# OwshenNetwork/owshen

Hardware: AMD Instinct MI355X
Metric: withdraw proofs/sec (batch=1024) (higher is better)
Workload: dtype u32 (9 x 29-bit-limb Montgomery, 254-bit modular integers)

## Files before the change

include/owshen_gpu.h:

```cpp
#ifndef OWSHEN_GPU_H
#define OWSHEN_GPU_H

#include <stddef.h>
#include <stdint.h>

#ifdef __cplusplus
extern "C" {
#endif

typedef struct og_ctx og_ctx;
typedef struct og_bases og_bases;
typedef struct og_pk og_pk;

#define OG_OK 0
#define OG_ERR_INVALID (-1)
#define OG_ERR_HIP (-2)
#define OG_ERR_NO_DEVICE (-3)
#define OG_ERR_UNSATISFIED (-4)

int og_init(int device, og_ctx** out);
void og_shutdown(og_ctx* ctx);
const char* og_last_error(void);
int og_device_count(void);
int og_sync(og_ctx* ctx);
void* og_stream(og_ctx* ctx);

int og_malloc(og_ctx* ctx, size_t bytes, void** out_d);
int og_free(og_ctx* ctx, void* ptr_d);
int og_memcpy_h2d(og_ctx* ctx, void* dst_d, const void* src, size_t bytes);
int og_memcpy_d2h(og_ctx* ctx, void* dst, const void* src_d, size_t bytes);

int og_field_op_d(og_ctx* ctx, int field, int op, const uint8_t* a_d, const uint8_t* b_d,
                  uint8_t* out_d, size_t n);
int og_field_mulchain_d(og_ctx* ctx, int field, uint8_t* x_d, const uint8_t* y_d, size_t n,
                        int iters, float* ms_out);

int og_field_mulchain_lat_d(og_ctx* ctx, int field, int form, uint8_t* x_d, const uint8_t* y_d, size_t n,
                            int iters, float* ms_out, uint64_t* wave_cycles_out);

int og_ubench(og_ctx* ctx, int kind, int iters, int blocks, float* ms_out);
int og_ubench_cycles(og_ctx* ctx, int kind, int iters, int blocks, float* ms_out, uint64_t* wave_cycles_out);
int og_ubench_coresidency(og_ctx* ctx, int wgs_per_cu, int kind, int iters, int filler_blocks, int filler_threads,
                          int filler_lds, int filler_prio, int filler_work, int delay_us, float out[3]);

int og_mimc7_constants(og_ctx* ctx, uint8_t out[91 * 32]);
int og_mimc7_hash2_d(og_ctx* ctx, const uint8_t* left_d, const uint8_t* right_d, uint8_t* out_d,
                     size_t n);
int og_mimc7_merkle_paths_d(og_ctx* ctx, const uint8_t* leaves_d, const uint64_t* indices_d,
                            const uint8_t* siblings_d, int depth, uint8_t* nodes_out_d, size_t n);
int og_mimc7_tree_build_d(og_ctx* ctx, const uint8_t* leaves_d, size_t n, uint8_t* nodes_out_d);
int og_mimc7_append_d(og_ctx* ctx, int depth, const uint8_t* frontier_in_d, uint64_t next_index, const uint8_t* leaves_d,
                      size_t k, uint8_t* frontier_out_d, uint8_t* root_out_d);

int og_eddsa_verify_batch_d(og_ctx* ctx, const uint8_t* records_d, size_t n, uint32_t* ok_out);

int og_eddsa_pubkey_batch_d(og_ctx* ctx, const uint8_t* sk_d, size_t n, uint8_t* pk_out_d, uint8_t* pkc_out_d, uint32_t* ok_out);
int og_eddsa_decompress_batch_d(og_ctx* ctx, const uint8_t* pkc_d, size_t n, uint8_t* pk_out_d, uint32_t* ok_out);
int og_eddsa_sign_batch_d(og_ctx* ctx, const uint8_t* requests_d, size_t n, uint8_t* records_out_d, uint32_t* ok_out);
int og_eddsa_verify_compressed_batch_d(og_ctx* ctx, const uint8_t* records_d, size_t n, uint32_t* ok_out);

int og_note_seal_batch_d(og_ctx* ctx, const uint8_t* requests_d, size_t n, uint8_t* memos_out_d, uint8_t* notes_out_d, uint32_t* ok_out);
int og_note_scan_batch_d(og_ctx* ctx, const uint8_t sk[32], const uint8_t* memos_d, const uint8_t* leaves_d, size_t n, uint8_t* opened_out_d, uint32_t* hit_out);

int og_ntt_fr_d(og_ctx* ctx, const uint8_t* in_d, uint8_t* out_d, int log_n, int batch, int inverse,
                int coset);
int og_h_poly_d(og_ctx* ctx, const uint8_t* a_d, const uint8_t* b_d, const uint8_t* c_d, int log_d,
                int batch, uint8_t* h_out_d);

int og_bases_create_d(og_ctx* ctx, int group, const uint8_t* points_d, size_t n, int window_bits,
                      int precompute, og_bases** out);
void og_bases_free(og_bases* bases);
int og_msm_d(og_ctx* ctx, const og_bases* bases, const uint8_t* scalars_d, size_t n, int batch,
             size_t stride_bytes, uint8_t* out);

int og_msm_partial_slots(const og_bases* bases);
int og_msm_windows_d(og_ctx* ctx, const og_bases* bases, const uint8_t* scalars_d, size_t n, int win_rank, int win_world,
                     uint8_t* partial_out_d);
int og_msm_combine_d(og_ctx* ctx, const og_bases* bases, const uint8_t* gathered_d, int world, uint8_t* out);

int og_pk_load(og_ctx* ctx, const uint8_t* blob, size_t len, og_pk** out);
void og_pk_free(og_pk* pk);
int og_pk_info(const og_pk* pk, uint64_t info[4]);
int og_pk_density(const og_pk* pk, uint64_t out[4]);
int og_pk_windows(const og_pk* pk, uint64_t out[4]);
int og_pk_load_rows(og_ctx* ctx, const uint8_t* blob, size_t len, const uint8_t* rows, size_t rows_len, og_pk** out);
int og_pk_query_form(const og_pk* pk, uint64_t out[20]);
int og_prove(og_ctx* ctx, const og_pk* pk, const uint8_t* witness, const uint8_t rs[64], uint8_t proof_out[256]);
int og_prove_batch(og_ctx* ctx, const og_pk* pk, const uint8_t* witnesses, size_t n, const uint8_t* rs,
                   uint8_t* proofs_out);
int og_prove_batch_d(og_ctx* ctx, const og_pk* pk, const uint8_t* witnesses_d, size_t n, const uint8_t* rs,
                     uint8_t* proofs_out);

typedef struct og_multi og_multi;
int og_multi_init(int n_devices, og_multi** out);
void og_multi_shutdown(og_multi* m);
int og_multi_size(const og_multi* m);
int og_multi_slice(const og_multi* m, size_t n, int rank, size_t out[2]);
og_ctx* og_multi_ctx(og_multi* m, int rank);
int og_multi_device_info(const og_multi* m, int rank, uint64_t out[4], char pci_out[32]);
int og_multi_pk_load(og_multi* m, const uint8_t* blob, size_t len, og_pk** pks_out);
void og_multi_pk_free(og_multi* m, og_pk** pks);
int og_multi_prove_batch(og_multi* m, og_pk* const* pks, const uint8_t* witnesses, size_t n, const uint8_t* rs,
                         uint8_t* proofs_out);
int og_multi_withdraw_prove_batch(og_multi* m, og_pk* const* pks, int depth, uint64_t n_pad3, uint64_t n_pad2,
                                  const uint8_t* inputs, size_t n, const uint8_t* rs, uint8_t* proofs_out,
                                  uint8_t* public_out);
int og_multi_withdraw_prove_sharded(og_multi* m, og_pk* const* pks, int depth, uint64_t n_pad3, uint64_t n_pad2,
                                    const uint8_t* inputs, size_t n, const uint8_t* rs, uint8_t* proofs_out,
                                    uint8_t* public_out);
int og_multi_prove_sharded(og_multi* m, og_pk* const* pks, const uint8_t* witnesses, size_t n, const uint8_t* rs,
                           uint8_t* proofs_out);
int og_multi_bases_create(og_multi* m, int group, const uint8_t* points, size_t n, int window_bits, int precompute,
                          og_bases** bases_out);
void og_multi_bases_free(og_multi* m, og_bases** bases);
int og_multi_msm(og_multi* m, og_bases* const* bases, const uint8_t* scalars, size_t n, uint8_t* out);

int og_verify(const uint8_t* vk, size_t vk_len, const uint8_t* public_inputs, size_t n_pub,
              const uint8_t proof[256], int* ok_out);

typedef struct og_vk og_vk;
int og_vk_load(og_ctx* ctx, const uint8_t* vk, size_t vk_len, og_vk** out);
void og_vk_free(og_vk* vk);
int og_vk_info(const og_vk* vk, uint64_t info[4]);
int og_verify_batch_d(og_ctx* ctx, const og_vk* vk, const uint8_t* public_inputs_d, const uint8_t* proofs_d, size_t n,
                      uint32_t* ok_out);

int og_withdraw_shape(int depth, uint64_t n_pad3, uint64_t n_pad2, uint64_t shape[3]);
int og_withdraw_witness_d(og_ctx* ctx, int depth, uint64_t n_pad3, uint64_t n_pad2, const uint8_t* inputs_d,
                          size_t n, uint8_t* witness_out_d);
int og_withdraw_prove_batch_d(og_ctx* ctx, const og_pk* pk, int depth, uint64_t n_pad3, uint64_t n_pad2,
                              const uint8_t* inputs_d, size_t n, const uint8_t* rs, uint8_t* proofs_out,
                              uint8_t* public_out);

int og_deposit_shape(uint64_t shape[3]);
int og_deposit_witness_d(og_ctx* ctx, const uint8_t* inputs_d, size_t n, uint8_t* witness_out_d);
int og_deposit_prove_batch_d(og_ctx* ctx, const og_pk* pk, const uint8_t* inputs_d, size_t n, const uint8_t* rs,
                             uint8_t* proofs_out, uint8_t* public_out);

int og_split_shape(int depth, uint64_t shape[3]);
int og_split_witness_d(og_ctx* ctx, int depth, const uint8_t* inputs_d, size_t n, uint8_t* witness_out_d);
int og_split_prove_batch_d(og_ctx* ctx, const og_pk* pk, int depth, const uint8_t* inputs_d, size_t n, const uint8_t* rs,
                           uint8_t* proofs_out, uint8_t* public_out);

int og_join_shape(int depth, uint64_t shape[3]);
int og_join_witness_d(og_ctx* ctx, int depth, const uint8_t* inputs_d, size_t n, uint8_t* witness_out_d);
int og_join_prove_batch_d(og_ctx* ctx, const og_pk* pk, int depth, const uint8_t* inputs_d, size_t n, const uint8_t* rs,
                          uint8_t* proofs_out, uint8_t* public_out);

int og_transfer_shape(int depth, uint64_t shape[3]);
int og_transfer_witness_d(og_ctx* ctx, int depth, const uint8_t* inputs_d, size_t n, uint8_t* witness_out_d);
int og_transfer_prove_batch_d(og_ctx* ctx, const og_pk* pk, int depth, const uint8_t* inputs_d, size_t n, const uint8_t* rs,
                              uint8_t* proofs_out, uint8_t* public_out);

typedef struct og_job og_job;
int og_withdraw_prove_batch_submit_d(og_ctx* ctx, const og_pk* pk, int depth, uint64_t n_pad3, uint64_t n_pad2,
                                     const uint8_t* inputs_d, size_t n, const uint8_t* rs, uint8_t* proofs_out,
                                     uint8_t* public_out, og_job** job_out);
int og_job_wait(og_ctx* ctx, og_job* job);
int og_job_poll(og_ctx* ctx, og_job* job, int* done_out);
int og_job_abandon(og_ctx* ctx, og_job* job);

#define OG_PARTIAL_BYTES 768
int og_withdraw_prove_partials_d(og_ctx* ctx, const og_pk* pk, int depth, uint64_t n_pad3, uint64_t n_pad2,
                                 const uint8_t* inputs_d, size_t n, int win_rank, int win_world, uint8_t* partials_d,
                                 uint8_t* public_out);
int og_prove_partials_d(og_ctx* ctx, const og_pk* pk, const uint8_t* witnesses_d, size_t n, int win_rank, int win_world,
                        uint8_t* partials_d);
int og_prove_from_partials_d(og_ctx* ctx, const og_pk* pk, const uint8_t* gathered_d, int win_world, size_t n,
                             const uint8_t* rs, uint8_t* proofs_out);

typedef struct og_r1cs og_r1cs;
int og_withdraw_r1cs(og_ctx* ctx, int depth, uint64_t n_pad3, uint64_t n_pad2, int dense, og_r1cs** out);
int og_deposit_r1cs(og_ctx* ctx, og_r1cs** out);
int og_split_r1cs(og_ctx* ctx, int depth, og_r1cs** out);
int og_join_r1cs(og_ctx* ctx, int depth, og_r1cs** out);
int og_transfer_r1cs(og_ctx* ctx, int depth, og_r1cs** out);
int og_r1cs_from_csr(uint64_t n_wires, uint64_t n_pub, uint64_t n_constraints, const uint32_t* const ptr[3],
                     const uint32_t* const col[3], const uint8_t* const val[3], og_r1cs** out);
void og_r1cs_free(og_r1cs* r1cs);
int og_r1cs_info(const og_r1cs* r1cs, uint64_t info[6]);
int og_r1cs_export(const og_r1cs* r1cs, int matrix, uint32_t* ptr_out, uint32_t* col_out, uint8_t* val_out);
int og_setup(og_ctx* ctx, const og_r1cs* r1cs, const uint8_t toxic[160], uint8_t** pk_out, size_t* pk_len, uint8_t** vk_out,
             size_t* vk_len);
int og_setup_rows(og_ctx* ctx, const og_r1cs* r1cs, const uint8_t toxic[160], uint8_t** pk_out, size_t* pk_len, uint8_t** vk_out,
                  size_t* vk_len, uint8_t** rows_out, size_t* rows_len);
void og_blob_free(uint8_t* blob);

int og_zkey_import(og_ctx* ctx, const uint8_t* zkey, size_t zkey_len, const og_r1cs* r1cs, uint8_t** pk_out, size_t* pk_len,
                   uint8_t** vk_out, size_t* vk_len);
int og_zkey_export(og_ctx* ctx, const uint8_t* pk, size_t pk_len, const uint8_t* vk, size_t vk_len, uint8_t** zkey_out,
                   size_t* zkey_len);
int og_r1cs_read(const uint8_t* r1cs_file, size_t len, og_r1cs** out);
int og_r1cs_write(const og_r1cs* r1cs, uint8_t** file_out, size_t* file_len);
int og_wtns_read(const uint8_t* wtns, size_t len, uint8_t* values_out, size_t capacity, uint64_t* n_out);
int og_wtns_write(const uint8_t* values, uint64_t n, uint8_t** wtns_out, size_t* wtns_len);

int og_ptau_info(const uint8_t* ptau, size_t len, uint64_t info[4]);
int og_setup_ptau(og_ctx* ctx, const og_r1cs* r1cs, const uint8_t* ptau, size_t len, uint8_t** pk_out, size_t* pk_len,
                  uint8_t** vk_out, size_t* vk_len);
int og_pk_contribute(og_ctx* ctx, const uint8_t* pk, size_t pk_len, const uint8_t* vk, size_t vk_len, const uint8_t d[32],
                     uint8_t** pk_out, size_t* pk_out_len, uint8_t** vk_out, size_t* vk_out_len);
int og_ptau_verify(og_ctx* ctx, const uint8_t* ptau, size_t len, uint32_t* failed_out);
int og_pk_verify(og_ctx* ctx, const og_r1cs* r1cs, const uint8_t* ptau, size_t len, const uint8_t* pk, size_t pk_len,
                 const uint8_t* vk, size_t vk_len, uint32_t* failed_out);

int og_scalar_mul_d(og_ctx* ctx, int group, const uint8_t* base, const uint8_t* scalars_d, size_t n,
                    uint8_t* out_d);
int og_lagrange_evals_d(og_ctx* ctx, int log_d, const uint8_t tau[32], uint8_t* out_d);
int og_spmv_fr_d(og_ctx* ctx, const uint32_t* row_ptr_d, const uint32_t* col_d, const uint8_t* val_d,
                 size_t n_rows, const uint8_t* x_d, uint8_t* out_d);

int og_profile(og_ctx* ctx, int enable);
int og_set_lanes(og_ctx* ctx, int n_lanes);
int og_profile_read(og_ctx* ctx, int kind, double out[3]);
int og_release_scratch(og_ctx* ctx);
int og_set_scratch_budget(og_ctx* ctx, uint64_t bytes);
int og_set_host_chains(og_ctx* ctx, int max_requests);
int og_mem_info(og_ctx* ctx, uint64_t out[4]);
int og_prove_plan(og_ctx* ctx, const og_pk* pk, size_t n, uint32_t* sizes_out, size_t cap, size_t* count_out, int* mode_out);
int og_glv_decompose(const uint8_t k[32], uint8_t out[32]);
int og_pk_bytes(const og_pk* pk, uint64_t* out);

#ifdef __cplusplus
}
#endif
#endif
```

owshen_amd/_abi.py:

```python
import ctypes as C

_vp, _sz, _i, _u8p = C.c_void_p, C.c_size_t, C.c_int, C.c_void_p
_fp = C.POINTER(C.c_float)

SIGNATURES = {
    "og_init": (_i, [_i, C.POINTER(_vp)]),
    "og_shutdown": (None, [_vp]),
    "og_last_error": (C.c_char_p, []),
    "og_device_count": (_i, []),
    "og_sync": (_i, [_vp]),
    "og_stream": (_vp, [_vp]),
    "og_malloc": (_i, [_vp, _sz, C.POINTER(_vp)]),
    "og_free": (_i, [_vp, _vp]),
    "og_memcpy_h2d": (_i, [_vp, _vp, _vp, _sz]),
    "og_memcpy_d2h": (_i, [_vp, _vp, _vp, _sz]),
    "og_field_op_d": (_i, [_vp, _i, _i, _u8p, _u8p, _u8p, _sz]),
    "og_field_mulchain_d": (_i, [_vp, _i, _u8p, _u8p, _sz, _i, _fp]),
    "og_field_mulchain_lat_d": (_i, [_vp, _i, _i, _u8p, _u8p, _sz, _i, _fp, C.POINTER(C.c_uint64)]),
    "og_ubench": (_i, [_vp, _i, _i, _i, _fp]),
    "og_ubench_cycles": (_i, [_vp, _i, _i, _i, _fp, C.POINTER(C.c_uint64)]),
    "og_ubench_coresidency": (_i, [_vp, _i, _i, _i, _i, _i, _i, _i, _i, _i, _fp]),
    "og_mimc7_constants": (_i, [_vp, _vp]),
    "og_mimc7_hash2_d": (_i, [_vp, _u8p, _u8p, _u8p, _sz]),
    "og_mimc7_merkle_paths_d": (_i, [_vp, _u8p, _vp, _u8p, _i, _u8p, _sz]),
    "og_mimc7_tree_build_d": (_i, [_vp, _u8p, _sz, _u8p]),
    "og_mimc7_append_d": (_i, [_vp, _i, _u8p, C.c_uint64, _u8p, _sz, _u8p, _u8p]),
    "og_eddsa_verify_batch_d": (_i, [_vp, _u8p, _sz, _vp]),
    "og_eddsa_pubkey_batch_d": (_i, [_vp, _u8p, _sz, _u8p, _u8p, _vp]),
    "og_eddsa_decompress_batch_d": (_i, [_vp, _u8p, _sz, _u8p, _vp]),
    "og_eddsa_sign_batch_d": (_i, [_vp, _u8p, _sz, _u8p, _vp]),
    "og_eddsa_verify_compressed_batch_d": (_i, [_vp, _u8p, _sz, _vp]),
    "og_note_seal_batch_d": (_i, [_vp, _u8p, _sz, _u8p, _u8p, _vp]),
    "og_note_scan_batch_d": (_i, [_vp, _u8p, _u8p, _u8p, _sz, _u8p, _vp]),
    "og_ntt_fr_d": (_i, [_vp, _u8p, _u8p, _i, _i, _i, _i]),
    "og_h_poly_d": (_i, [_vp, _u8p, _u8p, _u8p, _i, _i, _u8p]),
    "og_bases_create_d": (_i, [_vp, _i, _u8p, _sz, _i, _i, C.POINTER(_vp)]),
    "og_bases_free": (None, [_vp]),
    "og_msm_d": (_i, [_vp, _vp, _u8p, _sz, _i, _sz, _vp]),
    "og_msm_partial_slots": (_i, [_vp]),
    "og_msm_windows_d": (_i, [_vp, _vp, _u8p, _sz, _i, _i, _u8p]),
    "og_msm_combine_d": (_i, [_vp, _vp, _u8p, _i, _vp]),
    "og_multi_init": (_i, [_i, C.POINTER(_vp)]),
    "og_multi_shutdown": (None, [_vp]),
    "og_multi_size": (_i, [_vp]),
    "og_multi_slice": (_i, [_vp, _sz, _i, C.POINTER(_sz)]),
    "og_multi_ctx": (_vp, [_vp, _i]),
    "og_multi_pk_load": (_i, [_vp, _vp, _sz, C.POINTER(_vp)]),
    "og_multi_pk_free": (None, [_vp, C.POINTER(_vp)]),
    "og_multi_prove_batch": (_i, [_vp, C.POINTER(_vp), _vp, _sz, _vp, _vp]),
    "og_multi_withdraw_prove_batch": (_i, [_vp, C.POINTER(_vp), _i, C.c_uint64, C.c_uint64, _vp, _sz, _vp, _vp, _vp]),
    "og_multi_withdraw_prove_sharded": (_i, [_vp, C.POINTER(_vp), _i, C.c_uint64, C.c_uint64, _vp, _sz, _vp, _vp, _vp]),
    "og_multi_prove_sharded": (_i, [_vp, C.POINTER(_vp), _vp, _sz, _vp, _vp]),
    "og_withdraw_prove_partials_d": (_i, [_vp, _vp, _i, C.c_uint64, C.c_uint64, _u8p, _sz, _i, _i, _u8p, _vp]),
    "og_prove_partials_d": (_i, [_vp, _vp, _u8p, _sz, _i, _i, _u8p]),
    "og_prove_from_partials_d": (_i, [_vp, _vp, _u8p, _i, _sz, _vp, _vp]),
    "og_multi_bases_create": (_i, [_vp, _i, _vp, _sz, _i, _i, C.POINTER(_vp)]),
    "og_multi_bases_free": (None, [_vp, C.POINTER(_vp)]),
    "og_multi_msm": (_i, [_vp, C.POINTER(_vp), _vp, _sz, _vp]),
    "og_deposit_shape": (_i, [C.POINTER(C.c_uint64)]),
    "og_deposit_witness_d": (_i, [_vp, _u8p, _sz, _u8p]),
    "og_deposit_prove_batch_d": (_i, [_vp, _vp, _u8p, _sz, _vp, _vp, _vp]),
    "og_deposit_r1cs": (_i, [_vp, C.POINTER(_vp)]),
    "og_split_shape": (_i, [_i, C.POINTER(C.c_uint64)]),
    "og_split_witness_d": (_i, [_vp, _i, _u8p, _sz, _u8p]),
    "og_split_prove_batch_d": (_i, [_vp, _vp, _i, _u8p, _sz, _vp, _vp, _vp]),
    "og_split_r1cs": (_i, [_vp, _i, C.POINTER(_vp)]),
    "og_join_shape": (_i, [_i, C.POINTER(C.c_uint64)]),
    "og_join_witness_d": (_i, [_vp, _i, _u8p, _sz, _u8p]),
    "og_join_prove_batch_d": (_i, [_vp, _vp, _i, _u8p, _sz, _vp, _vp, _vp]),
    "og_join_r1cs": (_i, [_vp, _i, C.POINTER(_vp)]),
    "og_transfer_shape": (_i, [_i, C.POINTER(C.c_uint64)]),
    "og_transfer_witness_d": (_i, [_vp, _i, _u8p, _sz, _u8p]),
    "og_transfer_prove_batch_d": (_i, [_vp, _vp, _i, _u8p, _sz, _vp, _vp, _vp]),
    "og_transfer_r1cs": (_i, [_vp, _i, C.POINTER(_vp)]),
    "og_withdraw_r1cs": (_i, [_vp, _i, C.c_uint64, C.c_uint64, _i, C.POINTER(_vp)]),
    "og_r1cs_from_csr": (_i, [C.c_uint64, C.c_uint64, C.c_uint64, C.POINTER(_vp), C.POINTER(_vp), C.POINTER(_vp), C.POINTER(_vp)]),
    "og_r1cs_free": (None, [_vp]),
    "og_r1cs_info": (_i, [_vp, C.POINTER(C.c_uint64)]),
    "og_r1cs_export": (_i, [_vp, _i, _vp, _vp, _vp]),
    "og_setup": (_i, [_vp, _vp, _vp, C.POINTER(_vp), C.POINTER(_sz), C.POINTER(_vp), C.POINTER(_sz)]),
    "og_setup_rows": (_i, [_vp, _vp, _vp, C.POINTER(_vp), C.POINTER(_sz), C.POINTER(_vp), C.POINTER(_sz), C.POINTER(_vp), C.POINTER(_sz)]),
    "og_blob_free": (None, [_vp]),
    "og_zkey_import": (_i, [_vp, _vp, _sz, _vp, C.POINTER(_vp), C.POINTER(_sz), C.POINTER(_vp), C.POINTER(_sz)]),
    "og_r1cs_read": (_i, [_vp, _sz, C.POINTER(_vp)]),
    "og_r1cs_write": (_i, [_vp, C.POINTER(_vp), C.POINTER(_sz)]),
    "og_zkey_export": (_i, [_vp, _vp, _sz, _vp, _sz, C.POINTER(_vp), C.POINTER(_sz)]),
    "og_wtns_read": (_i, [_vp, _sz, _vp, _sz, C.POINTER(C.c_uint64)]),
    "og_wtns_write": (_i, [_vp, C.c_uint64, C.POINTER(_vp), C.POINTER(_sz)]),
    "og_ptau_info": (_i, [_vp, _sz, C.POINTER(C.c_uint64)]),
    "og_setup_ptau": (_i, [_vp, _vp, _vp, _sz, C.POINTER(_vp), C.POINTER(_sz), C.POINTER(_vp), C.POINTER(_sz)]),
    "og_pk_contribute": (_i, [_vp, _vp, _sz, _vp, _sz, _vp, C.POINTER(_vp), C.POINTER(_sz), C.POINTER(_vp), C.POINTER(_sz)]),
    "og_ptau_verify": (_i, [_vp, _vp, _sz, C.POINTER(C.c_uint32)]),
    "og_pk_verify": (_i, [_vp, _vp, _vp, _sz, _vp, _sz, _vp, _sz, C.POINTER(C.c_uint32)]),
    "og_pk_load": (_i, [_vp, _vp, _sz, C.POINTER(_vp)]),
    "og_pk_load_rows": (_i, [_vp, _vp, _sz, _vp, _sz, C.POINTER(_vp)]),
    "og_pk_query_form": (_i, [_vp, C.POINTER(C.c_uint64)]),
    "og_pk_free": (None, [_vp]),
    "og_pk_info": (_i, [_vp, C.POINTER(C.c_uint64)]),
    "og_pk_density": (_i, [_vp, C.POINTER(C.c_uint64)]),
    "og_pk_windows": (_i, [_vp, C.POINTER(C.c_uint64)]),
    "og_prove": (_i, [_vp, _vp, _vp, _vp, _vp]),
    "og_prove_batch": (_i, [_vp, _vp, _vp, _sz, _vp, _vp]),
    "og_prove_batch_d": (_i, [_vp, _vp, _u8p, _sz, _vp, _vp]),
    "og_verify": (_i, [_vp, _sz, _vp, _sz, _vp, C.POINTER(_i)]),
    "og_vk_load": (_i, [_vp, _vp, _sz, C.POINTER(_vp)]),
    "og_vk_free": (None, [_vp]),
    "og_vk_info": (_i, [_vp, C.POINTER(C.c_uint64)]),
    "og_verify_batch_d": (_i, [_vp, _vp, _u8p, _u8p, _sz, _vp]),
    "og_withdraw_shape": (_i, [_i, C.c_uint64, C.c_uint64, C.POINTER(C.c_uint64)]),
    "og_withdraw_witness_d": (_i, [_vp, _i, C.c_uint64, C.c_uint64, _u8p, _sz, _u8p]),
    "og_profile": (_i, [_vp, _i]),
    "og_set_lanes": (_i, [_vp, _i]),
    "og_profile_read": (_i, [_vp, _i, C.POINTER(C.c_double)]),
    "og_release_scratch": (_i, [_vp]),
    "og_set_scratch_budget": (_i, [_vp, C.c_uint64]),
    "og_set_host_chains": (_i, [_vp, _i]),
    "og_withdraw_prove_batch_d": (_i, [_vp, _vp, _i, C.c_uint64, C.c_uint64, _u8p, _sz, _vp, _vp, _vp]),
    "og_withdraw_prove_batch_submit_d": (_i, [_vp, _vp, _i, C.c_uint64, C.c_uint64, _u8p, _sz, _vp, _vp, _vp, C.POINTER(_vp)]),
    "og_job_wait": (_i, [_vp, _vp]),
    "og_job_abandon": (_i, [_vp, _vp]),
    "og_job_poll": (_i, [_vp, _vp, _vp]),
    "og_multi_device_info": (_i, [_vp, _i, _vp, _vp]),
    "og_mem_info": (_i, [_vp, C.POINTER(C.c_uint64)]),
    "og_pk_bytes": (_i, [_vp, C.POINTER(C.c_uint64)]),
    "og_glv_decompose": (_i, [_vp, _vp]),
    "og_prove_plan": (_i, [_vp, _vp, _sz, C.POINTER(C.c_uint32), _sz, C.POINTER(_sz), C.POINTER(_i)]),
    "og_scalar_mul_d": (_i, [_vp, _i, _vp, _u8p, _sz, _u8p]),
    "og_lagrange_evals_d": (_i, [_vp, _i, _vp, _u8p]),
    "og_spmv_fr_d": (_i, [_vp, _vp, _vp, _u8p, _sz, _u8p, _u8p]),
}


def bind(lib):
    for name, (res, args) in SIGNATURES.items():
        f = getattr(lib, name)
        f.restype = res
        f.argtypes = args
    return lib
```

owshen_amd/csrc/groth16.hip:

```cpp
#include "ctx.h"
#include "statements.h"
#include "msm.hip.h"
#include "prover.h"
#include "field.hip.h"
#include "glv.h"
#include "ec.hip.h"
#include "key_blob.h"
#include <string.h>
#include <algorithm>
#include <iterator>
#include <atomic>
#include <mutex>
#include <thread>

struct og_pk {
  uint64_t m = 0, n_pub = 0, log_d = 0, n_rows = 0;
  size_t d = 0;
  uint64_t nnz[3] = {0, 0, 0};
  uint32_t* ptr[3] = {nullptr, nullptr, nullptr};
  uint32_t* col[3] = {nullptr, nullptr, nullptr};
  uint8_t* val[3] = {nullptr, nullptr, nullptr};
  uint32_t* long_rows[3] = {nullptr, nullptr, nullptr};
  uint32_t n_long[3] = {0, 0, 0};
  og_bases *a = nullptr, *b1 = nullptr, *b2 = nullptr, *l = nullptr, *h = nullptr;
  uint32_t* map[3] = {nullptr, nullptr, nullptr};
  size_t n_dense[3] = {0, 0, 0};
  size_t n_real[3] = {0, 0, 0};
  int sort_src[3] = {0, 1, 2};
  bool row[3] = {false, false, false};
  og_bases *lag1 = nullptr, *lag2 = nullptr;
  uint32_t* rmap = nullptr;
  size_t n_rowpts = 0;
  size_t rows_q[2] = {0, 0};
  int c_wire[3] = {0, 0, 0};
  bool merge_lh = false;
  bool c_is_ab = false;
  uint8_t* consts1 = nullptr;
  uint8_t* consts2 = nullptr;
  uint8_t* fb_delta2 = nullptr;
  int device = 0;
  uint8_t consts1_h[192] = {}, consts2_h[256] = {};
  std::vector<uint8_t> fb_delta2_h;
  mutable std::vector<uint8_t> fb_delta1_h;
  mutable std::once_flag fb_delta1_once;
};

namespace og {

__global__ void __launch_bounds__(256) k_spmv(const uint32_t* __restrict__ ptr, const uint32_t* __restrict__ col,
                                             const uint8_t* __restrict__ val, size_t n_rows, size_t n_out,
                                             const uint8_t* __restrict__ x, size_t x_stride, uint8_t* __restrict__ out,
                                             size_t out_stride, int val_mont, int out_mont, uint32_t long_row,
                                             uint8_t* __restrict__ canon, size_t canon_stride) {
  OG_FILLER_PRIO();
  size_t row = (size_t)blockIdx.x * blockDim.x + threadIdx.x;
  if (row >= n_out) return;
  const int g = blockIdx.y;
  const uint8_t* xg = x + (size_t)g * x_stride;
  Fr acc = Fr::zero();
  if (row < n_rows) {
    if (ptr[row + 1] - ptr[row] > long_row) return;
    for (uint32_t k = ptr[row]; k < ptr[row + 1]; k++) {
      Fr v = fe_load<FrParams>(val + (size_t)k * 32);
      if (!val_mont) v = fe_to_mont(v);
      acc = fe_add(acc, fe_mul(v, fe_load<FrParams>(xg + (size_t)col[k] * 32)));
    }
    if (canon) fe_store(canon + (size_t)g * canon_stride + row * 32, fe_canon(acc));
    acc = out_mont ? fe_to_mont(acc) : fe_canon(acc);
  }
  fe_store(out + (size_t)g * out_stride + row * 32, acc);
}

constexpr uint32_t SPMV_LONG = 2048;
__global__ void __launch_bounds__(256) k_spmv_long(const uint32_t* __restrict__ rows, const uint32_t* __restrict__ ptr,
                                                  const uint32_t* __restrict__ col, const uint8_t* __restrict__ val,
                                                  const uint8_t* __restrict__ x, size_t x_stride, uint8_t* __restrict__ out,
                                                  size_t out_stride, int val_mont, int out_mont, uint8_t* __restrict__ canon,
                                                  size_t canon_stride) {
  OG_FILLER_PRIO();
  __shared__ __align__(16) uint32_t part[256 * 8];
  const uint32_t row = rows[blockIdx.x];
  const int g = blockIdx.y;
  const uint8_t* xg = x + (size_t)g * x_stride;
  Fr acc = Fr::zero();
  for (uint32_t k = ptr[row] + threadIdx.x; k < ptr[row + 1]; k += 256) {
    Fr v = fe_load<FrParams>(val + (size_t)k * 32);
    if (!val_mont) v = fe_to_mont(v);
    acc = fe_add(acc, fe_mul(v, fe_load<FrParams>(xg + (size_t)col[k] * 32)));
  }
  fe_store(&part[threadIdx.x * 8], acc);
  __syncthreads();
  for (int d = 128; d >= 1; d >>= 1) {
    if ((int)threadIdx.x < d)
      fe_store(&part[threadIdx.x * 8], fe_add(fe_load<FrParams>(&part[threadIdx.x * 8]), fe_load<FrParams>(&part[(threadIdx.x + d) * 8])));
    __syncthreads();
  }
  if (threadIdx.x == 0) {
    acc = fe_load<FrParams>(&part[0]);
    if (canon) fe_store(canon + (size_t)g * canon_stride + (size_t)row * 32, fe_canon(acc));
    fe_store(out + (size_t)g * out_stride + (size_t)row * 32, out_mont ? fe_to_mont(acc) : fe_canon(acc));
  }
}

__global__ void __launch_bounds__(256) k_fr_to_mont(const uint8_t* __restrict__ in, uint8_t* __restrict__ out, size_t n) {
  size_t i = (size_t)blockIdx.x * blockDim.x + threadIdx.x;
  if (i >= n) return;
  fe_store(out + i * 32, fe_to_mont(fe_load<FrParams>(in + i * 32)));
}

__global__ void __launch_bounds__(256) k_mul_rows(const uint8_t* __restrict__ a, const uint8_t* __restrict__ b, uint8_t* __restrict__ c, size_t d) {
  OG_FILLER_PRIO();
  const size_t row = (size_t)blockIdx.x * blockDim.x + threadIdx.x;
  if (row >= d) return;
  const size_t o = ((size_t)blockIdx.y * d + row) * 32;
  fe_store(c + o, fe_mul(fe_load<FrParams>(a + o), fe_load<FrParams>(b + o)));
}

__global__ void __launch_bounds__(256) k_check_rows(const uint8_t* __restrict__ a, const uint8_t* __restrict__ b, const uint8_t* __restrict__ c,
                                                   size_t n_rows, size_t d, const uint8_t* __restrict__ z, size_t z_stride,
                                                   uint32_t* __restrict__ flags) {
  OG_FILLER_PRIO();
  size_t row = (size_t)blockIdx.x * blockDim.x + threadIdx.x;
  const int g = blockIdx.y;
  if (row >= n_rows) return;
  const size_t o = ((size_t)g * d + row) * 32;
  bool bad = !fe_sub(fe_mul(fe_load<FrParams>(a + o), fe_load<FrParams>(b + o)), fe_load<FrParams>(c + o)).is_zero();
  if (row == 0) {
    Fr z0 = fe_load<FrParams>(z + (size_t)g * z_stride);
    z0.l[0] ^= 1u;
    uint32_t nz = 0;
#pragma unroll
    for (int i = 0; i < 9; i++) nz |= z0.l[i];
    bad = bad || nz != 0;
  }
  if (bad) atomicOr(&flags[g], 1u);
}

__global__ void __launch_bounds__(256) k_check_canonical(const uint8_t* __restrict__ x, size_t stride, size_t count, uint32_t* __restrict__ bad) {
  OG_FILLER_PRIO();
  const size_t i = (size_t)blockIdx.x * blockDim.x + threadIdx.x;
  if (i >= count) return;
  const int g = blockIdx.y;
  if (!fe_lt_modulus(fe_load<FrParams>(x + (size_t)g * stride + i * 32))) atomicMin(&bad[g], (uint32_t)i);
}

__global__ void __launch_bounds__(256) k_lagrange(const uint8_t* __restrict__ consts, const uint8_t* __restrict__ tau_c, int log_d,
                                                 uint8_t* __restrict__ out) {
  size_t k = (size_t)blockIdx.x * blockDim.x + threadIdx.x;
  const size_t d = (size_t)1 << log_d;
  if (k >= d) return;
  Fr tau = fe_to_mont(fe_load<FrParams>(tau_c));
  Fr zt = tau;
  for (int i = 0; i < log_d; i++) zt = fe_sqr(zt);
  zt = fe_sub(zt, Fr::one());
  Fr b = fe_load<FrParams>(consts + 0 * 32), wk = Fr::one();
  for (size_t e = k; e; e >>= 1) {
    if (e & 1) wk = fe_mul(wk, b);
    b = fe_sqr(b);
  }
  Fr num = fe_mul(fe_mul(zt, fe_load<FrParams>(consts + 4 * 32)), wk);
  Fr den = fe_sub(tau, wk);
  fe_store(out + k * 32, fe_from_mont(fe_mul(num, fe_inv(den))));
}

int spmv_canonical(og_ctx* ctx, const uint32_t* ptr_d, const uint32_t* col_d, const uint8_t* val_d, size_t n_rows,
                   const uint8_t* x_d, uint8_t* out_d) {
  if (n_rows == 0) return OG_OK;
  hipLaunchKernelGGL(k_spmv, dim3(grid_for(n_rows, 256), 1), dim3(256), 0, ctx->stream, ptr_d, col_d, val_d, n_rows, n_rows, x_d,
                     (size_t)0, out_d, (size_t)0, 0, 0, 0xffffffffu, (uint8_t*)nullptr, (size_t)0);
  OG_HIP(hipGetLastError());
  return OG_OK;
}

int lagrange_evals(og_ctx* ctx, int log_d, const uint8_t tau[32], uint8_t* out_d) {
  uint8_t* consts = nullptr;
  OG_TRY(ntt_domain_consts(ctx, log_d, &consts));
  uint8_t* tau_d = nullptr;
  OG_TRY(arena_get(ctx, "g16.tau", 32, (void**)&tau_d));
  OG_HIP(hipMemcpyAsync(tau_d, tau, 32, hipMemcpyHostToDevice, ctx->stream));
  const size_t d = (size_t)1 << log_d;
  hipLaunchKernelGGL(k_lagrange, dim3(grid_for(d, 256)), dim3(256), 0, ctx->stream, consts, tau_d, log_d, out_d);
  OG_HIP(hipGetLastError());
  OG_HIP(hipStreamSynchronize(ctx->stream));
  return OG_OK;
}

int scalar_mul_fixed(og_ctx* ctx, int is_g2, const uint8_t* base_host, const uint8_t* scalars_d, size_t n, uint8_t* out_d) {
  const size_t pb = is_g2 ? 128 : 64;
  const int g = is_g2 ? 1 : 0;
  uint8_t *raw = nullptr, *mont = nullptr;
  OG_TRY(arena_get(ctx, "g16.base.raw", 128, (void**)&raw));
  OG_TRY(arena_get(ctx, "g16.base.mont", 128, (void**)&mont));
  if (!ctx->fb_tab[g]) {
    OG_HIP(hipMalloc((void**)&ctx->fb_tab[g], 64 * 16 * pb));
    ctx->owned.push_back(ctx->fb_tab[g]);
  }
  uint8_t* tab = ctx->fb_tab[g];
  if (!ctx->fb_valid[g] || memcmp(ctx->fb_base[g], base_host, pb) != 0) {
    ctx->fb_valid[g] = false;
    OG_HIP(hipMemcpyAsync(raw, base_host, pb, hipMemcpyHostToDevice, ctx->stream));
    OG_TRY(is_g2 ? import_points_g2(ctx, raw, mont, 1) : import_points_g1(ctx, raw, mont, 1));
    OG_TRY(is_g2 ? fixed_table_g2(ctx, mont, tab) : fixed_table_g1(ctx, mont, tab));
    OG_HIP(hipStreamSynchronize(ctx->stream));
    memcpy(ctx->fb_base[g], base_host, pb);
    ctx->fb_valid[g] = true;
  }
  OG_TRY(is_g2 ? scalar_mul_fixed_g2(ctx, tab, scalars_d, n, out_d) : scalar_mul_fixed_g1(ctx, tab, scalars_d, n, out_d));
  OG_HIP(hipStreamSynchronize(ctx->stream));
  return OG_OK;
}

void pk_destroy(og_pk* pk) {
  if (!pk) return;
  (void)hipSetDevice(pk->device);
  (void)hipDeviceSynchronize();
  for (int k = 0; k < 3; k++) {
    if (pk->ptr[k]) (void)hipFree(pk->ptr[k]);
    if (pk->col[k]) (void)hipFree(pk->col[k]);
    if (pk->val[k]) (void)hipFree(pk->val[k]);
    if (pk->long_rows[k]) (void)hipFree(pk->long_rows[k]);
  }
  for (og_bases* q : {pk->a, pk->b1, pk->b2})
    if (q != pk->lag1 && q != pk->lag2) bases_destroy(q);
  bases_destroy(pk->lag1); bases_destroy(pk->lag2); bases_destroy(pk->l); bases_destroy(pk->h);
  for (int k = 0; k < 3; k++)
    if (pk->map[k] && pk->map[k] != pk->rmap) (void)hipFree(pk->map[k]);
  if (pk->rmap) (void)hipFree(pk->rmap);
  if (pk->consts1) (void)hipFree(pk->consts1);
  if (pk->consts2) (void)hipFree(pk->consts2);
  if (pk->fb_delta2) (void)hipFree(pk->fb_delta2);
  delete pk;
}

bool row_form_pays(size_t rows_q, size_t wires_q) {
  if (rows_q == 0 || wires_q == 0) return false;
  const double row_adds = (double)rows_q * msm_nwin((int)msm_pick_query_c(rows_q));
  const double wire_adds = (double)wires_q * msm_nwin((int)msm_pick_query_c(wires_q));
  return row_adds <= 0.8 * wire_adds;
}

static int rows_check(og_ctx* ctx, const og_pk* pk, const PkView& v, const RowsView& rv, uint8_t* stage, const std::string& who) {
  const size_t m = pk->m, nr = pk->n_rows;
  std::vector<uint8_t> rho(m * 32);
  uint64_t x = rd64(rv.digest) ^ rd64(rv.digest + 8) ^ rd64(rv.digest + 16) ^ rd64(rv.digest + 24);
  for (size_t i = 0; i < m * 4; i++) {
    x += 0x9e3779b97f4a7c15ull;
    uint64_t z = x;
    z = (z ^ (z >> 30)) * 0xbf58476d1ce4e5b9ull;
    z = (z ^ (z >> 27)) * 0x94d049bb133111ebull;
    z ^= z >> 31;
    if ((i & 3) == 3) z &= (1ull << 60) - 1;
    memcpy(&rho[i * 8], &z, 8);
  }
  uint8_t *rho_d, *ev_d, *res_d, *aff_d;
  OG_TRY(arena_get(ctx, "g16.chk.rho", m * 32, (void**)&rho_d));
  OG_TRY(arena_get(ctx, "g16.chk.ev", nr * 32, (void**)&ev_d));
  OG_TRY(arena_get(ctx, "g16.chk.res", 512, (void**)&res_d));
  OG_TRY(arena_get(ctx, "g16.chk.aff", 256, (void**)&aff_d));
  OG_HIP(hipMemcpyAsync(rho_d, rho.data(), m * 32, hipMemcpyHostToDevice, ctx->stream));
  const int cw = (int)msm_pick_c(m);
  struct Pair { int q, src, is_g2; const char* name; };
  const Pair pairs[3] = {{0, 0, 0, "A"}, {1, 1, 0, "B (G1)"}, {1, 2, 1, "B (G2)"}};
  for (const Pair& p : pairs) {
    if (!pk->row[p.q]) continue;
    const size_t pb = p.is_g2 ? 128 : 64;
    hipLaunchKernelGGL(k_spmv, dim3(grid_for(nr, 256), 1), dim3(256), 0, ctx->stream, pk->ptr[p.q], pk->col[p.q], pk->val[p.q], nr, nr, rho_d,
                       (size_t)0, ev_d, (size_t)0, 1, 0, SPMV_LONG, (uint8_t*)nullptr, (size_t)0);
    OG_HIP(hipGetLastError());
    if (pk->n_long[p.q]) {
      hipLaunchKernelGGL(k_spmv_long, dim3(pk->n_long[p.q], 1), dim3(256), 0, ctx->stream, pk->long_rows[p.q], pk->ptr[p.q], pk->col[p.q],
                         pk->val[p.q], rho_d, (size_t)0, ev_d, (size_t)0, 1, 0, (uint8_t*)nullptr, (size_t)0);
      OG_HIP(hipGetLastError());
    }
    OG_HIP(hipMemcpyAsync(stage, v.query[p.src], m * pb, hipMemcpyHostToDevice, ctx->stream));
    og_bases* wb = nullptr;
    OG_TRY(bases_create(ctx, p.is_g2, stage, m, cw, 0, &wb));
    struct Drop { og_bases* b; ~Drop() { bases_destroy(b); } } drop{wb};
    DigitSort dw, dr;
    OG_TRY(msm_digit_sort(ctx, 0, rho_d, m * 32, m, nullptr, 1, cw, 0, &dw));
    OG_TRY(msm_run(ctx, wb, dw, res_d));
    const og_bases* lag = p.is_g2 ? pk->lag2 : pk->lag1;
    OG_TRY(msm_digit_sort(ctx, 1, ev_d, nr * 32, pk->n_rowpts, pk->rmap, 1, lag->c, 1, &dr));
    OG_TRY(msm_run(ctx, lag, dr, res_d + 256));
    OG_TRY(xyzz_to_affine_bytes(ctx, p.is_g2, res_d, aff_d, 1));
    OG_TRY(xyzz_to_affine_bytes(ctx, p.is_g2, res_d + 256, aff_d + 128, 1));
    uint8_t got[256];
    OG_HIP(hipMemcpyAsync(got, aff_d, 256, hipMemcpyDeviceToHost, ctx->stream));
    OG_HIP(hipStreamSynchronize(ctx->stream));
    OG_REQUIRE(memcmp(got, got + 128, pb) == 0,
               who + ": row-basis extension: its points do not reproduce the key's " + p.name + " query (not the Lagrange basis of this key's tau)");
  }
  return OG_OK;
}

static int pk_load_impl(og_ctx* ctx, const uint8_t* blob, size_t len, const uint8_t* rows, size_t rows_len, og_pk* pk) {
  const std::string who = rows ? "og_pk_load_rows" : "og_pk_load";
  PkView v;
  OG_TRY(pk_view(blob, len, who, &v));
  RowsView rv{};
  if (rows) OG_TRY(rows_view(rows, rows_len, v, who, &rv));
  OG_REQUIRE(v.flags <= 1 && v.word9 == 0, who + ": unknown header flags");
  OG_REQUIRE(!(v.flags & 1) || v.nnz[2] == 0, who + ": a key with the C = A o B flag carries no C matrix");
  OG_TRY(pk_csr_check(v, 3, who));
  pk->m = v.m; pk->n_pub = v.l; pk->log_d = v.log_d; pk->n_rows = v.n_rows; pk->d = v.d;
  for (int k = 0; k < 3; k++) pk->nnz[k] = v.nnz[k];
  pk->c_is_ab = (v.flags & 1) != 0;
  const size_t m = pk->m, nl = v.nl, nh = v.nh;
  const uint8_t *c1 = blob + PK_CONSTS1, *c2 = blob + PK_CONSTS2;
  for (int k = 0; k < 3; k++) {
    OG_HIP(hipMalloc((void**)&pk->ptr[k], (pk->n_rows + 1) * 4));
    OG_HIP(hipMalloc((void**)&pk->col[k], pk->nnz[k] * 4 + 4));
    OG_HIP(hipMalloc((void**)&pk->val[k], pk->nnz[k] * 32 + 32));
    OG_HIP(hipMemcpyAsync(pk->ptr[k], v.ptr[k], (pk->n_rows + 1) * 4, hipMemcpyHostToDevice, ctx->stream));
    OG_HIP(hipMemcpyAsync(pk->col[k], v.col[k], pk->nnz[k] * 4, hipMemcpyHostToDevice, ctx->stream));
    OG_HIP(hipMemcpyAsync(pk->val[k], v.val[k], pk->nnz[k] * 32, hipMemcpyHostToDevice, ctx->stream));
    {
      std::vector<uint32_t> lr;
      for (size_t r = 0; r < pk->n_rows; r++)
        if (rd32(v.ptr[k] + (r + 1) * 4) - rd32(v.ptr[k] + r * 4) > SPMV_LONG) lr.push_back((uint32_t)r);
      pk->n_long[k] = (uint32_t)lr.size();
      if (!lr.empty()) {
        OG_HIP(hipMalloc((void**)&pk->long_rows[k], lr.size() * 4));
        OG_HIP(hipMemcpy(pk->long_rows[k], lr.data(), lr.size() * 4, hipMemcpyHostToDevice));
      }
    }
    if (pk->nnz[k]) {
      hipLaunchKernelGGL(k_fr_to_mont, dim3(grid_for(pk->nnz[k], 256)), dim3(256), 0, ctx->stream, pk->val[k], pk->val[k],
                         (size_t)pk->nnz[k]);
      OG_HIP(hipGetLastError());
    }
  }
  uint8_t* stage = nullptr;
  const size_t stage_bytes = std::max<size_t>(std::max<size_t>(std::max<size_t>(512, m * 128), nh * 64), rows ? pk->n_rows * 128 : 0);
  OG_HIP(hipMalloc((void**)&stage, stage_bytes));
  struct Guard { uint8_t* p; ~Guard() { if (p) (void)hipFree(p); } } guard{stage};
  OG_HIP(hipMalloc((void**)&pk->consts1, 256));
  OG_HIP(hipMalloc((void**)&pk->consts2, 256));
  OG_HIP(hipMemcpyAsync(stage, c1, 256, hipMemcpyHostToDevice, ctx->stream));
  OG_TRY(import_points_g1(ctx, stage, pk->consts1, 3));
  OG_HIP(hipStreamSynchronize(ctx->stream));
  OG_HIP(hipMemcpyAsync(stage, c2, 256, hipMemcpyHostToDevice, ctx->stream));
  OG_TRY(import_points_g2(ctx, stage, pk->consts2, 2));
  OG_HIP(hipMalloc((void**)&pk->fb_delta2, 64 * 16 * 128));
  OG_TRY(fixed_table_g2(ctx, pk->consts2 + 128, pk->fb_delta2));
  OG_HIP(hipStreamSynchronize(ctx->stream));
  pk->fb_delta2_h.resize(64 * 16 * 128);
  OG_HIP(hipMemcpy(pk->consts1_h, pk->consts1, 192, hipMemcpyDeviceToHost));
  OG_HIP(hipMemcpy(pk->consts2_h, pk->consts2, 256, hipMemcpyDeviceToHost));
  OG_HIP(hipMemcpy(pk->fb_delta2_h.data(), pk->fb_delta2, pk->fb_delta2_h.size(), hipMemcpyDeviceToHost));
  int ch = (int)msm_pick_query_c(nh);
  std::vector<uint32_t> wire[3];
  for (size_t i = 0; i < m; i++) {
    if (!all_zero(v.query[0] + i * 64, 64)) wire[0].push_back((uint32_t)i);
    if (!all_zero(v.query[1] + i * 64, 64) || !all_zero(v.query[2] + i * 128, 128)) wire[1].push_back((uint32_t)i);
  }
  for (size_t i = 0; i < nl; i++)
    if (!all_zero(v.query[3] + i * 64, 64)) wire[2].push_back((uint32_t)(i + pk->n_pub + 1));
  for (int k = 0; k < 3; k++) pk->n_real[k] = wire[k].size();
  std::vector<uint32_t> rlist;
  if (rows) {
    const long long force = OG_HOOK_INT("OG_ROW_FORM", -1);
    for (int q = 0; q < 2; q++) {
      for (size_t r = 0; r < pk->n_rows; r++) pk->rows_q[q] += rd32(v.ptr[q] + (r + 1) * 4) > rd32(v.ptr[q] + r * 4);
      pk->row[q] = pk->rows_q[q] > 0 && !wire[q].empty() && force != 0 && (force == 1 || row_form_pays(pk->rows_q[q], wire[q].size()));
    }
    for (size_t r = 0; r < pk->n_rows; r++)
      if ((pk->row[0] && rd32(v.ptr[0] + (r + 1) * 4) > rd32(v.ptr[0] + r * 4)) || (pk->row[1] && rd32(v.ptr[1] + (r + 1) * 4) > rd32(v.ptr[1] + r * 4)))
        rlist.push_back((uint32_t)r);
  }
  for (int q = 1; q < 3; q++)
    for (int p0 = 0; p0 < q; p0++) {
      if (pk->row[q] || pk->row[p0]) continue;
      if (pk->sort_src[p0] != p0) continue;
      std::vector<uint32_t> u;
      std::set_union(wire[p0].begin(), wire[p0].end(), wire[q].begin(), wire[q].end(), std::back_inserter(u));
      const size_t least = std::min(wire[p0].size(), wire[q].size());
      if (u.size() - least > 64 || msm_pick_query_c(u.size()) != msm_pick_query_c(least)) continue;
      for (int k = 0; k < q; k++)
        if (pk->sort_src[k] == p0) wire[k] = u;
      wire[q] = u;
      pk->sort_src[q] = p0;
      break;
    }
  pk->n_rowpts = rlist.size();
  if (!rlist.empty()) {
    OG_HIP(hipMalloc((void**)&pk->rmap, rlist.size() * 4 + 4));
    OG_HIP(hipMemcpyAsync(pk->rmap, rlist.data(), rlist.size() * 4, hipMemcpyHostToDevice, ctx->stream));
  }
  for (int k = 0; k < 3; k++) {
    pk->c_wire[k] = (int)msm_pick_query_c(wire[k].size());
    if (pk->row[k]) {
      pk->n_dense[k] = rlist.size();
      pk->map[k] = pk->rmap;
      continue;
    }
    pk->n_dense[k] = wire[k].size();
    OG_HIP(hipMalloc((void**)&pk->map[k], wire[k].size() * 4 + 4));
    OG_HIP(hipMemcpyAsync(pk->map[k], wire[k].data(), wire[k].size() * 4, hipMemcpyHostToDevice, ctx->stream));
  }
  OG_HIP(hipStreamSynchronize(ctx->stream));
  std::vector<uint8_t> host(std::max<size_t>(std::max<size_t>(std::max<size_t>(1, m * 128), nh * 64), rlist.size() * 128));
  if (!rlist.empty()) {
    for (int g2 = 0; g2 < (pk->row[1] ? 2 : 1); g2++) {
      const size_t pb = g2 ? 128 : 64;
      uint32_t flags = 0;
      OG_TRY(points_on_curve(ctx, g2, g2 ? rv.g2 : rv.g1, pk->n_rows, &flags));
      OG_REQUIRE(!(flags & 1), who + ": row-basis extension: a coordinate of a " + (g2 ? "G2" : "G1") + " point is not below the base-field modulus");
      OG_REQUIRE(!(flags & 2), who + ": row-basis extension: a " + (g2 ? "G2" : "G1") + " point is not on its curve");
      for (size_t k = 0; k < rlist.size(); k++) memcpy(host.data() + k * pb, (g2 ? rv.g2 : rv.g1) + (size_t)rlist[k] * pb, pb);
      OG_HIP(hipMemcpyAsync(stage, host.data(), rlist.size() * pb, hipMemcpyHostToDevice, ctx->stream));
      OG_TRY(bases_create(ctx, g2, stage, rlist.size(), (int)msm_pick_query_c(rlist.size()), 1, g2 ? &pk->lag2 : &pk->lag1));
    }
    if (pk->row[0]) pk->a = pk->lag1;
    if (pk->row[1]) { pk->b1 = pk->lag1; pk->b2 = pk->lag2; }
    OG_TRY(rows_check(ctx, pk, v, rv, stage, who));
  }
  struct QSpec { int src, mapk, is_g2; og_bases** dst; };
  const QSpec qs[4] = {{0, 0, 0, &pk->a}, {1, 1, 0, &pk->b1}, {2, 1, 1, &pk->b2}, {3, 2, 0, &pk->l}};
  for (const QSpec& q : qs) {
    if (pk->row[q.mapk]) continue;
    const size_t pb = q.is_g2 ? 128 : 64;
    const std::vector<uint32_t>& w = wire[q.mapk];
    const size_t shift = q.src == 3 ? pk->n_pub + 1 : 0;
    const size_t q_len = q.src == 3 ? nl : m;
    for (size_t k = 0; k < w.size(); k++) {
      if (w[k] >= shift && w[k] - shift < q_len) memcpy(host.data() + k * pb, v.query[q.src] + (w[k] - shift) * pb, pb);
      else memset(host.data() + k * pb, 0, pb);
    }
    OG_HIP(hipMemcpyAsync(stage, host.data(), w.size() * pb, hipMemcpyHostToDevice, ctx->stream));
    OG_TRY(bases_create(ctx, q.is_g2, stage, w.size(), (int)msm_pick_query_c(w.size()), 1, q.dst));
  }
  for (size_t k = 0; k < nh; k++) {
    size_t r = 0;
    for (uint64_t bit = 0; bit < pk->log_d; bit++) r |= ((k >> bit) & 1) << (pk->log_d - 1 - bit);
    memcpy(host.data() + k * 64, v.query[4] + r * 64, 64);
  }
  OG_HIP(hipMemcpyAsync(stage, host.data(), nh * 64, hipMemcpyHostToDevice, ctx->stream));
  const int cl = pk->l->c;
  const bool h_takes_cl = cl == ch || (cl == 17 && (double)nh * 15 < (double)(1u << 23) && nh >= 512) || (cl == 16 && nh >= 512);
  if (OG_HOOK_INT("OG_MERGE_LH", 1) && h_takes_cl && (cl == 16 || cl == 17 || cl == ch)) {
    ch = cl;
    pk->merge_lh = true;
  }
  OG_TRY(bases_create(ctx, 0, stage, nh, ch, 1, &pk->h));
  return OG_OK;
}

void pk_info(const og_pk* pk, uint64_t out[4]) {
  out[0] = pk->m; out[1] = pk->n_pub; out[2] = pk->log_d; out[3] = pk->n_rows;
}

void pk_windows(const og_pk* pk, uint64_t out[4]) {
  for (int k = 0; k < 3; k++) out[k] = (uint64_t)pk->c_wire[k];
  out[3] = pk->h->c;
}

void pk_query_form(const og_pk* pk, uint64_t out[20]) {
  const og_bases* q[5] = {pk->a, pk->b1, pk->b2, pk->l, pk->h};
  const int mapk[5] = {0, 1, 1, 2, -1};
  for (int k = 0; k < 5; k++) {
    out[4 * k + 0] = mapk[k] >= 0 && pk->row[mapk[k]] ? 1 : 0;
    out[4 * k + 1] = q[k]->n;
    out[4 * k + 2] = (uint64_t)q[k]->c;
    int first = k;
    for (int j = k - 1; j >= 0; j--)
      if (q[j] == q[k]) first = j;
    out[4 * k + 3] = (uint64_t)first;
  }
}

void pk_density(const og_pk* pk, uint64_t out[4]) {
  for (int k = 0; k < 3; k++) out[k] = pk->n_real[k];
  out[3] = pk->d - 1;
}

uint64_t pk_bytes(const og_pk* pk) {
  uint64_t b = 0;
  for (int k = 0; k < 3; k++)
    b += (pk->n_rows + 1) * 4 + pk->nnz[k] * 36 + 36 + (uint64_t)pk->n_long[k] * 4 + (pk->row[k] ? 0 : pk->n_dense[k] * 4 + 4);
  if (pk->rmap) b += pk->n_rowpts * 4 + 4;
  const og_bases* qs[5] = {pk->a, pk->b1, pk->b2, pk->l, pk->h};
  for (int k = 0; k < 5; k++) {
    const og_bases* q = qs[k];
    if (!q || std::find(qs, qs + k, q) != qs + k) continue;
    b += (uint64_t)(q->n ? q->n : 1) * (q->precomp ? q->nwin : 1) * (q->is_g2 ? 128 : 64);
  }
  return b + 256 + 256 + 64 * 16 * 128;
}

int pk_load(og_ctx* ctx, const uint8_t* blob, size_t len, const uint8_t* rows, size_t rows_len, og_pk** out) {
  og_pk* pk = new og_pk();
  pk->device = ctx->device;
  int r = pk_load_impl(ctx, blob, len, rows, rows_len, pk);
  if (r != OG_OK) {
    (void)hipStreamSynchronize(ctx->stream);
    pk_destroy(pk);
    return r;
  }
  *out = pk;
  return OG_OK;
}

bool glv_pair_ok() {
  static const bool ok = [] {
    const Fq one = Fq::one();
    const Fq two = fe_add(one, one);
    const Affine<Fq> g{one, two};
    XYZZ<Fq> acc = XYZZ<Fq>::inf();
    for (int bit = 255; bit >= 0; bit--) {
      acc = xyzz_dbl(acc);
      if ((glv::LAMBDA[bit >> 6] >> (bit & 63)) & 1) acc = xyzz_madd(acc, g);
    }
    const Affine<Fq> got = xyzz_to_affine(acc);
    uint32_t bw[8];
    for (int i = 0; i < 4; i++) { bw[2 * i] = (uint32_t)glv::BETA[i]; bw[2 * i + 1] = (uint32_t)(glv::BETA[i] >> 32); }
    const Fq want_x = fe_mul(one, fe_to_mont(fe_from_words<FqParams>(bw)));
    return fe_canon(got.x) == fe_canon(want_x) && fe_canon(got.y) == fe_canon(two);
  }();
  return ok;
}

static int choose_sub_batch(og_ctx* ctx, const og_pk* pk, size_t n) {
  size_t pts = pk->d, row_entries = 0, evc = 0;
  const og_bases* wq[3] = {pk->a, pk->b1, pk->l};
  int c_max = pk->l->c;
  for (int q = 0; q < 3; q++) {
    if (pk->row[q]) {
      row_entries += (size_t)wq[q]->nwin * pk->n_dense[q];
      evc += pk->n_rows * 32;
      c_max = std::max(c_max, wq[q]->c);
    } else if (pk->sort_src[q] == q) {
      pts += pk->n_dense[q];
    }
  }
  const size_t entries = (size_t)pk->l->nwin * pts + row_entries;
  const size_t per = entries * 4 * 2 + pk->d * 32 * 5 + pk->m * 32 + evc + ((size_t)1 << (c_max - 1)) * (4 * 128 + 256) * 2;
  size_t budget = (size_t)64 << 30, free_b = 0, total_b = 0;
  if (hipMemGetInfo(&free_b, &total_b) == hipSuccess && total_b) {
    size_t mine = 0;
    for (const auto& kv : ctx->arena) mine += kv.second.second;
    budget = std::min(budget, std::max<size_t>((size_t)1 << 30, (size_t)((double)(free_b + mine) * 0.85) / og_ctx::PIPE_SLOTS));
  }
  if (ctx->scratch_budget) budget = std::min(budget, std::max<size_t>(per, ctx->scratch_budget / og_ctx::PIPE_SLOTS));
  size_t sb = budget / (per ? per : 1);
  if (const char* e = getenv("OG_SUB_BATCH")) sb = (size_t)atoi(e);
  const size_t cap_by_size = std::max<size_t>(256, std::min<size_t>(1024, ((size_t)40 << 30) / (per ? per : 1)));
  sb = std::max<size_t>(1, std::min<size_t>(sb, (size_t)OG_HOOK_INT("OG_SUB_CAP", (long long)cap_by_size)));
  return (int)std::min(sb, n);
}

struct StatementGen {
  const Statement* st;
  StatementArgs args;
  const uint8_t* inputs_d;
};

struct WinShard {
  int rank = 0, world = 1;
  uint8_t* partials_d = nullptr;
};
constexpr size_t PARTIAL_BYTES = 4 * 128 + 256;

struct ProvePlan {
  int sb_max = 1;
  bool split = false, sym = false, pipe = false;
  std::vector<int> plan;
};

static int make_plan(og_ctx* ctx, const og_pk* pk, size_t n, ProvePlan* out) {
  const bool two_lanes = ctx->n_lanes >= 2;
  int sb_max = choose_sub_batch(ctx, pk, n);
  const size_t split_max = (size_t)OG_HOOK_INT("OG_SPLIT_MAX", 1024);
  if (two_lanes && (size_t)sb_max * 2 > n && n >= 2 && n > split_max) sb_max = (int)((n + 1) / 2);
  const bool split = two_lanes && n <= (size_t)sb_max && n <= std::max<size_t>(split_max, 1);
  const int pipe_min = (int)OG_HOOK_INT("OG_PIPE_MIN", 64);
  const bool sym = two_lanes && !split && sb_max < pipe_min;
  const bool pipe = two_lanes && !split && !sym;
  std::vector<int>& plan = out->plan;
  plan.clear();
  {
    size_t left = n;
    if (const char* e = pipe ? OG_HOOK_STR("OG_SUB_PLAN") : nullptr) {
      int last = sb_max;
      for (const char* q = e; *q && left;) {
        OG_REQUIRE(atoi(q) >= 1, "OG_SUB_PLAN: every sub-batch size must be >= 1 (empty or non-numeric entry)");
        last = std::min(sb_max, atoi(q));
        plan.push_back((int)std::min<size_t>(last, left));
        left -= plan.back();
        while (*q && *q != ',') q++;
        if (*q == ',') q++;
      }
      while (left) {
        plan.push_back((int)std::min<size_t>(last, left));
        left -= plan.back();
      }
    } else if (pipe && n > (size_t)sb_max) {
      const int first = std::max(1, std::max(pipe_min, sb_max / 4));
      plan.push_back(first);
      left -= first;
      const size_t parts = (left + sb_max - 1) / sb_max;
      for (size_t k = 0; k < parts; k++) {
        const size_t sz = (left + (parts - k) - 1) / (parts - k);
        plan.push_back((int)sz);
        left -= sz;
      }
    } else {
      while (left) {
        plan.push_back((int)std::min<size_t>(sb_max, left));
        left -= plan.back();
      }
    }
  }
  out->sb_max = sb_max; out->split = split; out->sym = sym; out->pipe = pipe;
  return OG_OK;
// ... 9 lines not shown
}

template <class T>
static XYZZ<T> host_mul_window4(const XYZZ<T>& p, const uint32_t k[8]) {
  XYZZ<T> tab[16];
  tab[1] = p;
  for (int d = 2; d < 16; d++) tab[d] = d == 2 ? xyzz_dbl(p) : xyzz_add(tab[d - 1], p);
  XYZZ<T> acc = XYZZ<T>::inf();
  for (int w = 63; w >= 0; w--) {
    if (w != 63) for (int e = 0; e < 4; e++) acc = xyzz_dbl(acc);
    const uint32_t dgt = (k[w >> 3] >> ((w & 7) * 4)) & 15u;
    if (dgt) acc = xyzz_add(acc, tab[dgt]);
  }
  return acc;
}
static const std::vector<uint8_t>& host_fb_delta1(const og_pk* pk) {
  std::call_once(pk->fb_delta1_once, [&]() {
    pk->fb_delta1_h.resize(64 * 16 * G1XYZZ::BYTES);
    G1XYZZ pw = G1XYZZ::from_affine(G1Affine::load(pk->consts1_h + 128));
    for (int w = 0; w < 64; w++) {
      G1XYZZ q = pw;
      for (int d = 1; d < 16; d++) {
        q.store(pk->fb_delta1_h.data() + (size_t)(w * 16 + d) * G1XYZZ::BYTES);
        q = xyzz_add(q, pw);
      }
      pw = q;
    }
  });
  return pk->fb_delta1_h;
}
constexpr size_t HOST_FIXED_BYTES = 2 * G1XYZZ::BYTES + G2XYZZ::BYTES;
static void host_assemble_fixed(const og_pk* pk, const uint8_t* rs, uint8_t* out) {
  uint32_t r[8], s[8], p[8];
  memcpy(r, rs, 32);
  memcpy(s, rs + 32, 32);
  fe_to_words(p, fe_from_mont(fe_mul(fe_to_mont(fe_from_words<FrParams>(r)), fe_to_mont(fe_from_words<FrParams>(s)))));
  const uint8_t* fb1 = host_fb_delta1(pk).data();
  auto fixed1 = [&](const uint32_t k[8]) {
    G1XYZZ acc = G1XYZZ::inf();
    for (int w = 0; w < 64; w++) {
      const uint32_t d = (k[w >> 3] >> ((w & 7) * 4)) & 15u;
      if (d) acc = xyzz_add(acc, G1XYZZ::load(fb1 + (size_t)(w * 16 + d) * G1XYZZ::BYTES));
    }
    return acc;
  };
  fixed1(r).store(out);
  fixed1(p).store(out + G1XYZZ::BYTES);
  G2XYZZ B = G2XYZZ::from_affine(G2Affine::load(pk->consts2_h));
  for (int w = 0; w < 64; w++) {
    const uint32_t d = (s[w >> 3] >> ((w & 7) * 4)) & 15u;
    if (d) B = xyzz_madd(B, G2Affine::load(pk->fb_delta2_h.data() + (size_t)(w * 16 + d) * G2Affine::BYTES));
  }
  B.store(out + 2 * G1XYZZ::BYTES);
}
static void host_assemble_one(const og_pk* pk, const uint8_t* rs, const uint8_t* fixed, const uint8_t* ra, const uint8_t* rb1,
                              const uint8_t* rb2, const uint8_t* rl, const uint8_t* rh, uint8_t* proof, bool helper_thread) {
  uint32_t r[8], s[8];
  memcpy(r, rs, 32);
  memcpy(s, rs + 32, 32);
  const G1Affine alpha = G1Affine::load(pk->consts1_h), beta1 = G1Affine::load(pk->consts1_h + 64);
  const G1XYZZ a_full = xyzz_madd(G1XYZZ::load(ra), alpha), b1_full = xyzz_madd(G1XYZZ::load(rb1), beta1);
  const G1XYZZ A = xyzz_add(a_full, G1XYZZ::load(fixed));
  G1XYZZ C = xyzz_add(G1XYZZ::load(rl), G1XYZZ::load(rh));
  G1XYZZ prod[2];
  auto mul = [&](size_t k) { prod[k] = k == 0 ? host_mul_window4(a_full, s) : host_mul_window4(b1_full, r); };
  if (helper_thread) host_parallel_for(2, mul);
  else { mul(0); mul(1); }
  C = xyzz_add(xyzz_add(C, prod[0]), prod[1]);
  C = xyzz_add(C, G1XYZZ::load(fixed + G1XYZZ::BYTES));
  const G2XYZZ B = xyzz_add(G2XYZZ::load(rb2), G2XYZZ::load(fixed + 2 * G1XYZZ::BYTES));
  G1Affine a = xyzz_to_affine(A), c = xyzz_to_affine(C);
  a.x = fe_from_mont(a.x); a.y = fe_from_mont(a.y);
  c.x = fe_from_mont(c.x); c.y = fe_from_mont(c.y);
  G2Affine b = xyzz_to_affine(B);
  b.x = FieldIO<Fq2>::from_mont(b.x); b.y = FieldIO<Fq2>::from_mont(b.y);
  a.store(proof);
  b.store(proof + 64);
  c.store(proof + 192);
}
static void assemble_fixed_on_host(const og_pk* pk, const uint8_t* rs, size_t n, std::vector<uint8_t>& fixed) {
  fixed.resize(n * HOST_FIXED_BYTES);
  (void)host_fb_delta1(pk);
  host_parallel_for(n, [&](size_t g) { host_assemble_fixed(pk, rs + g * 64, fixed.data() + g * HOST_FIXED_BYTES); });
}
static void assemble_on_host(const og_pk* pk, const uint8_t* rs, const uint8_t* fixed, const uint8_t* res, size_t n, uint8_t* proofs) {
  const uint8_t *ra = res, *rb1 = ra + n * 128, *rb2 = rb1 + n * 128, *rl = rb2 + n * 256, *rh = rl + n * 128;
  host_parallel_for(n, [&](size_t g) {
    host_assemble_one(pk, rs + g * 64, fixed + g * HOST_FIXED_BYTES, ra + g * 128, rb1 + g * 128, rb2 + g * 256, rl + g * 128, rh + g * 128,
                      proofs + g * 256, n == 1);
  });
}

static uint64_t next_job_id() {
  static std::atomic<uint64_t> n{1};
  return n.fetch_add(1);
}

static void glv_halves(const uint8_t* rs, size_t n, std::vector<uint8_t>& out) {
  out.clear();
  const size_t glv_max = !glv_pair_ok() ? 0 : OG_HOOK_SET("OG_GLV") ? (OG_HOOK_INT("OG_GLV", 1) ? (size_t)1 << 30 : 0) : 64;
  if (n > glv_max) return;
  out.resize(n * 128);
  for (size_t g = 0; g < n && !out.empty(); g++) {
    const uint8_t *rb = rs + g * 64, *sb = rs + g * 64 + 32;
    uint32_t rw[8], sw[8], pw[8];
    memcpy(rw, rb, 32);
    memcpy(sw, sb, 32);
    fe_to_words(pw, fe_from_mont(fe_mul(fe_to_mont(fe_from_words<FrParams>(rw)), fe_to_mont(fe_from_words<FrParams>(sw)))));
    uint8_t* o = out.data() + g * 128;
    if (!glv::decompose(rb, o) || !glv::decompose(reinterpret_cast<const uint8_t*>(pw), o + 32) || !glv::decompose(sb, o + 64)) out.clear();
    else memcpy(o + 96, o, 32);
  }
}

static int prove_finish(og_job* job, size_t* first_bad);

struct ProveCall {
  og_ctx* ctx;
  const og_pk* pk;
  size_t n;
  ProvePlan plan;
  int call_slot;
  const StatementGen* gen;
  const uint8_t *z_host, *z_d;
  bool trusted_z;
  const WinShard* sh;
  bool host_asm;
  const uint8_t* rs;
  uint8_t *proofs, *pub_out;
  uint8_t *res[5], *rs_d, *proofs_d, *asm_tmp, *glv_d, *pub_d;
  size_t asm_lanes;
  uint32_t *flags, *bad;
  bool assembles() const { return !sh && !host_asm; }
};
struct SubBatch {
  size_t g0;
  int sb, slot;
  const uint8_t* zs;
  uint8_t *ev[3], *tmp, *h;
  uint8_t* evc[2];
  uint8_t* res(const ProveCall& c, int k) const { return c.res[k] + g0 * (k == 2 ? 256 : 128); }
  uint8_t* asm_tmp(const ProveCall& c) const { return c.asm_tmp + g0 * c.asm_lanes * 128 * 17; }
  const uint8_t* glv(const ProveCall& c) const { return c.glv_d ? c.glv_d + g0 * 128 : nullptr; }
};

static int sub_sort(const ProveCall& c, const SubBatch& s, int slot, int q, DigitSort* out) {
  const og_pk* pk = c.pk;
  const uint8_t* scalars = q < 2 && pk->row[q] ? s.evc[q] : s.zs;
  const size_t stride = q < 2 && pk->row[q] ? (size_t)pk->n_rows * 32 : pk->m * 32;
  return msm_digit_sort_windows(c.ctx, slot, scalars, stride, pk->n_dense[q], pk->map[q], s.sb, (q == 0 ? pk->a : q == 1 ? pk->b1 : pk->l)->c,
                                1, c.sh ? c.sh->rank : 0, c.sh ? c.sh->world : 1, out);
}
static int sub_sort_h(const ProveCall& c, const SubBatch& s, DigitSort* out) {
  return msm_digit_sort_windows(c.ctx, 2, s.h, c.pk->d * 32, c.pk->d - 1, nullptr, s.sb, c.pk->h->c, 1, c.sh ? c.sh->rank : 0,
                                c.sh ? c.sh->world : 1, out);
}

static int call_begin(ProveCall& c) {
  og_ctx* ctx = c.ctx;
  const og_pk* pk = c.pk;
  const size_t n = c.n;
  const std::string cs = "#" + std::to_string(c.call_slot);
  const char* resn[5] = {"g16.res.a", "g16.res.b1", "g16.res.b2", "g16.res.l", "g16.res.h"};
  uint8_t** res = c.res;
  if (c.sh) {
    res[0] = c.sh->partials_d; res[1] = res[0] + n * 128; res[3] = res[1] + n * 128; res[4] = res[3] + n * 128; res[2] = res[4] + n * 128;
  } else {
    for (int k = 0; k < 5; k++) OG_TRY(arena_get(ctx, (resn[k] + cs).c_str(), n * (k == 2 ? 256 : 128), (void**)&res[k]));
  }
  OG_TRY(arena_get(ctx, ("g16.rs" + cs).c_str(), n * 64, (void**)&c.rs_d));
  OG_TRY(arena_get(ctx, ("g16.proofs" + cs).c_str(), n * 256, (void**)&c.proofs_d));
  c.host_asm = !c.sh && ctx->host_chains_max > 0 && n <= (size_t)ctx->host_chains_max;
  std::vector<uint8_t> glv_h;
  if (c.assembles()) glv_halves(c.rs, n, glv_h);
  c.asm_lanes = glv_h.empty() ? 4 : 8;
  OG_TRY(arena_get(ctx, ("g16.asm" + cs).c_str(), n * c.asm_lanes * 128 * 17, (void**)&c.asm_tmp));
  c.glv_d = nullptr;
  if (!glv_h.empty()) OG_TRY(arena_get(ctx, ("g16.glv" + cs).c_str(), n * 128, (void**)&c.glv_d));
  OG_TRY(arena_get(ctx, ("g16.flags" + cs).c_str(), n * 8, (void**)&c.flags));
  c.bad = c.flags + n;
  c.pub_d = nullptr;
  if (c.pub_out && pk->n_pub) OG_TRY(arena_get(ctx, ("g16.pub" + cs).c_str(), n * pk->n_pub * 32, (void**)&c.pub_d));
  if (!c.sh) OG_HIP(hipMemcpyAsync(c.rs_d, c.rs, n * 64, hipMemcpyHostToDevice, ctx->copy_lane));
  if (c.glv_d) OG_HIP(hipMemcpyAsync(c.glv_d, glv_h.data(), n * 128, hipMemcpyHostToDevice, ctx->copy_lane));
  OG_HIP(hipStreamSynchronize(ctx->copy_lane));
  if (ctx->pipe_ev[0][0] == nullptr)
    for (int p = 0; p < og_ctx::PIPE_SLOTS; p++)
      for (int e = 0; e < og_ctx::PIPE_EVENTS; e++) OG_HIP(hipEventCreateWithFlags(&ctx->pipe_ev[p][e], hipEventDisableTiming));
  ctx->sort_beside_acc = c.plan.pipe;
  if (!(c.plan.pipe && ctx->last_call_piped)) OG_HIP(drain_streams(ctx));
  ctx->last_call_piped = c.plan.pipe;
  return OG_OK;
}

static int sub_front(const ProveCall& c, SubBatch& s) {
  og_ctx* ctx = c.ctx;
  const og_pk* pk = c.pk;
  const size_t m = pk->m, d = pk->d, g0 = s.g0, sb_max = (size_t)c.plan.sb_max;
  const char* evn[3] = {"g16.eva", "g16.evb", "g16.evc"};
  for (int k = 0; k < 3; k++) OG_TRY(arena_get(ctx, evn[k], sb_max * d * 32, (void**)&s.ev[k]));
  const char* evcn[2] = {"g16.eva.c", "g16.evb.c"};
  for (int k = 0; k < 2; k++) {
    s.evc[k] = nullptr;
    if (pk->row[k]) OG_TRY(arena_get(ctx, evcn[k], sb_max * pk->n_rows * 32, (void**)&s.evc[k]));
  }
  OG_TRY(arena_get(ctx, "g16.tmp", 32, (void**)&s.tmp));
  OG_TRY(arena_get(ctx, "g16.h", sb_max * d * 32, (void**)&s.h));
  s.zs = c.z_d ? c.z_d + g0 * m * 32 : nullptr;
  OG_HIP(hipMemsetAsync(c.bad + g0, 0xff, (size_t)s.sb * 4, ctx->stream));
  if (const StatementGen* gen = c.gen) {
    const uint8_t* records = gen->inputs_d + g0 * record_bytes(*gen->st, gen->args.depth);
    uint8_t* zbuf = nullptr;
    OG_TRY(records_check_enqueue(*gen->st, ctx, gen->args, records, (size_t)s.sb, c.bad + g0));
    OG_TRY(arena_get(ctx, "g16.zgen", sb_max * m * 32, (void**)&zbuf));
    OG_TRY(gen->st->witness(*gen->st, ctx, gen->args, records, (size_t)s.sb, zbuf));
    s.zs = zbuf;
  } else if (c.z_host) {
    uint8_t* zbuf = nullptr;
    OG_TRY(arena_get(ctx, "g16.zgen", sb_max * m * 32, (void**)&zbuf));
    OG_HIP(hipMemcpyAsync(zbuf, c.z_host + g0 * m * 32, (size_t)s.sb * m * 32, hipMemcpyHostToDevice, ctx->stream));
    s.zs = zbuf;
  }
  if (!c.gen && !c.trusted_z) {
    hipLaunchKernelGGL(k_check_canonical, dim3(grid_for(m, 256), s.sb), dim3(256), 0, ctx->stream, s.zs, m * 32, m, c.bad + g0);
    OG_HIP(hipGetLastError());
  }
  if (c.pub_d)
    OG_HIP(hipMemcpy2DAsync(c.pub_d + g0 * pk->n_pub * 32, pk->n_pub * 32, s.zs + 32, m * 32, pk->n_pub * 32, (size_t)s.sb,
                            hipMemcpyDeviceToDevice, ctx->stream));
  return OG_OK;
}

static int sub_rows(const ProveCall& c, const SubBatch& s) {
  og_ctx* ctx = c.ctx;
  const og_pk* pk = c.pk;
  const size_t m = pk->m, d = pk->d;
  const int sb = s.sb;
  for (int k = 0; k < 3; k++) {
    ProfScope ps(ctx, PROF_SPMV, (double)pk->nnz[k] * sb);
    if (k == 2 && pk->c_is_ab) {
      hipLaunchKernelGGL(k_mul_rows, dim3(grid_for(d, 256), sb), dim3(256), 0, ctx->stream, s.ev[0], s.ev[1], s.ev[2], d);
      OG_HIP(hipGetLastError());
      continue;
    }
    uint8_t* canon = k < 2 && pk->row[k] ? s.evc[k] : nullptr;
    hipLaunchKernelGGL(k_spmv, dim3(grid_for(d, 256), sb), dim3(256), 0, ctx->stream, pk->ptr[k], pk->col[k], pk->val[k],
                       (size_t)pk->n_rows, d, s.zs, m * 32, s.ev[k], d * 32, 1, 1, SPMV_LONG, canon, (size_t)pk->n_rows * 32);
    OG_HIP(hipGetLastError());
    if (pk->n_long[k]) {
      hipLaunchKernelGGL(k_spmv_long, dim3(pk->n_long[k], sb), dim3(256), 0, ctx->stream, pk->long_rows[k], pk->ptr[k], pk->col[k],
                         pk->val[k], s.zs, m * 32, s.ev[k], d * 32, 1, 1, canon, (size_t)pk->n_rows * 32);
      OG_HIP(hipGetLastError());
    }
  }
  OG_HIP(hipMemsetAsync(c.flags + s.g0, 0, (size_t)sb * 4, ctx->stream));
  if (pk->n_rows) {
    hipLaunchKernelGGL(k_check_rows, dim3(grid_for(pk->n_rows, 256), sb), dim3(256), 0, ctx->stream, s.ev[0], s.ev[1], s.ev[2],
                       (size_t)pk->n_rows, d, s.zs, m * 32, c.flags + s.g0);
    OG_HIP(hipGetLastError());
  }
  OG_STEP(ctx, "g16.spmv");
  return OG_OK;
}

static int sub_quotient(const ProveCall& c, const SubBatch& s) {
  ProfScope ps(c.ctx, PROF_HPOLY, (double)c.pk->d * s.sb);
  OG_TRY(h_poly_device(c.ctx, s.ev[0], s.ev[1], s.ev[2], s.tmp, s.h, (int)c.pk->log_d, s.sb));
  OG_STEP(c.ctx, "g16.hpoly");
  return OG_OK;
}

static int msm_l(const ProveCall& c, const SubBatch& s, const DigitSort& ds_l) {
  if (!c.pk->merge_lh) return msm_run(c.ctx, c.pk->l, ds_l, s.res(c, 3));
  OG_HIP(hipMemsetAsync(s.res(c, 3), 0, (size_t)s.sb * 128, c.ctx->stream));
  return msm_run_phase(c.ctx, c.pk->l, ds_l, nullptr, MSM_FIRST);
}
static int msm_h(const ProveCall& c, const SubBatch& s, const DigitSort& dh) {
  return msm_run_phase(c.ctx, c.pk->h, dh, s.res(c, 4), c.pk->merge_lh ? MSM_SECOND : MSM_FULL);
}

static int sub_assemble(const ProveCall& c, const SubBatch& s) {
  if (!c.assembles()) return OG_OK;
  og_ctx* ctx = c.ctx;
  const og_pk* pk = c.pk;
  ProfScope ps_asm(ctx, PROF_ASSEMBLE, (double)s.sb);
  OG_TRY(assemble_g1(ctx, pk->consts1, c.rs_d + s.g0 * 64, s.res(c, 0), s.res(c, 1), s.res(c, 3), s.res(c, 4), (size_t)s.sb, s.asm_tmp(c),
                     c.proofs_d + s.g0 * 256, s.glv(c)));
  OG_TRY(assemble_g2(ctx, pk->consts2, pk->fb_delta2, c.rs_d + s.g0 * 64, s.res(c, 2), (size_t)s.sb, c.proofs_d + s.g0 * 256));
  OG_STEP(ctx, "g16.assemble");
  return OG_OK;
}

static int issue_fan_out(const ProveCall& c, SubBatch& s) {
  og_ctx* ctx = c.ctx;
  const og_pk* pk = c.pk;
  hipEvent_t* fan = ctx->pipe_ev[0];
  hipStream_t s0 = ctx->lanes[0], s_b2 = ctx->lanes[1], s_b1 = ctx->copy_lane, s_a = ctx->tail_lane, s_l = ctx->aux_lane;
  const bool asm_early = c.assembles() && OG_HOOK_INT("OG_ASM_EARLY", 1) != 0;
  const uint8_t* rs_sub = c.rs_d + s.g0 * 64;
  uint8_t* proofs_sub = c.proofs_d + s.g0 * 256;
  auto side = [&](int lane_id, hipStream_t st, hipEvent_t after) -> int {
    ctx->lane = lane_id;
    ctx->stream = st;
    OG_HIP(hipStreamWaitEvent(st, after, 0));
    return OG_OK;
  };
  ctx->lane = s.slot;
  ctx->stream = s0;
  OG_TRY(sub_front(c, s));
  const bool rows_first = pk->row[0] || pk->row[1];
  if (rows_first) OG_TRY(sub_rows(c, s));
  OG_HIP(hipEventRecord(ctx->ev0, s0));
  DigitSort dsb, dsa, dsl, dh;
  OG_TRY(side(1, s_b2, ctx->ev0));
  OG_TRY(sub_sort(c, s, 1, 1, &dsb));
  OG_HIP(hipEventRecord(fan[FAN_B_SORTED], s_b2));
  OG_TRY(msm_run(ctx, pk->b2, dsb, s.res(c, 2)));
  {
    ProfScope ps_asm(ctx, PROF_ASSEMBLE, 0.0);
    if (c.assembles())
      OG_TRY(assemble_g2(ctx, pk->consts2, pk->fb_delta2, rs_sub, s.res(c, 2), (size_t)s.sb, proofs_sub, OG_HOOK_INT("OG_ASM_G2_TREE", 1) != 0));
  }
  OG_HIP(hipEventRecord(ctx->ev1, s_b2));
  OG_TRY(side(4, s_b1, fan[FAN_B_SORTED]));
  OG_TRY(msm_run(ctx, pk->b1, dsb, s.res(c, 1)));
  OG_HIP(hipEventRecord(fan[FAN_B1_DONE], s_b1));
  OG_TRY(side(2, s_a, ctx->ev0));
  OG_TRY(sub_sort(c, s, 1, 0, &dsa));
  OG_TRY(msm_run(ctx, pk->a, dsa, s.res(c, 0)));
  if (asm_early) {
    ProfScope ps_asm(ctx, PROF_ASSEMBLE, 0.0);
    OG_HIP(hipStreamWaitEvent(s_a, fan[FAN_B1_DONE], 0));
    OG_TRY(assemble_g1_early(ctx, pk->consts1, rs_sub, s.res(c, 0), s.res(c, 1), (size_t)s.sb, s.asm_tmp(c), proofs_sub, s.glv(c),
                             fan[FAN_PRODUCTS]));
  }
  OG_HIP(hipEventRecord(fan[FAN_A_DONE], s_a));
  OG_TRY(side(3, s_l, ctx->ev0));
  OG_TRY(sub_sort(c, s, 1, 2, &dsl));
  OG_TRY(msm_run(ctx, pk->l, dsl, s.res(c, 3)));
  OG_HIP(hipEventRecord(fan[FAN_L_DONE], s_l));
  ctx->lane = s.slot;
  ctx->stream = s0;
  if (!rows_first) OG_TRY(sub_rows(c, s));
  OG_TRY(sub_quotient(c, s));
  OG_TRY(sub_sort_h(c, s, &dh));
  OG_TRY(msm_run_phase(ctx, pk->h, dh, s.res(c, 4), MSM_FULL));
  OG_STEP(ctx, "g16.msm");
  if (asm_early) {
    OG_HIP(hipStreamWaitEvent(s0, fan[FAN_L_DONE], 0));
    OG_HIP(hipStreamWaitEvent(s0, fan[FAN_PRODUCTS], 0));
    ProfScope ps_asm(ctx, PROF_ASSEMBLE, (double)s.sb);
    OG_TRY(assemble_g1_late(ctx, s.res(c, 3), s.res(c, 4), (size_t)s.sb, s.asm_tmp(c), proofs_sub, c.glv_d != nullptr));
    OG_STEP(ctx, "g16.assemble");
  } else {
    for (int e : {FAN_B1_DONE, FAN_A_DONE, FAN_L_DONE}) OG_HIP(hipStreamWaitEvent(s0, fan[e], 0));
    if (c.assembles()) {
      ProfScope ps_asm(ctx, PROF_ASSEMBLE, (double)s.sb);
      OG_TRY(assemble_g1(ctx, pk->consts1, rs_sub, s.res(c, 0), s.res(c, 1), s.res(c, 3), s.res(c, 4), (size_t)s.sb, s.asm_tmp(c), proofs_sub,
                         s.glv(c)));
      OG_STEP(ctx, "g16.assemble");
    }
  }
  if (asm_early) OG_HIP(hipStreamWaitEvent(s0, fan[FAN_A_DONE], 0));
  OG_HIP(hipStreamWaitEvent(s0, ctx->ev1, 0));
  return OG_OK;
}

static int issue_pipeline(const ProveCall& c, SubBatch& s) {
  og_ctx* ctx = c.ctx;
  const og_pk* pk = c.pk;
  hipStream_t math = ctx->lanes[0], prep = ctx->lanes[1], aux = ctx->aux_lane, tail = ctx->tail_lane;
  s.slot = (int)(ctx->pipe_counter++ % og_ctx::PIPE_SLOTS);
  hipEvent_t* ev = ctx->pipe_ev[s.slot];
  auto on = [&](hipStream_t st) { ctx->stream = st; };
  auto rec = [&](int e) -> int { OG_HIP(hipEventRecord(ev[e], ctx->stream)); return OG_OK; };
  auto wait = [&](int e) -> int { OG_HIP(hipStreamWaitEvent(ctx->stream, ev[e], 0)); return OG_OK; };
  ctx->lane = s.slot;
  on(prep);
  OG_TRY(wait(EV_PREP_FREE));
  OG_TRY(sub_front(c, s));
  OG_TRY(sub_rows(c, s));
  OG_TRY(rec(EV_ROWS));
  DigitSort ds_a, ds_b, ds_l, dh;
  OG_TRY(sub_sort(c, s, 1, 0, &ds_a));
  OG_TRY(rec(EV_SORT_A));
  if (pk->sort_src[1] == 0) ds_b = ds_a;
  else OG_TRY(sub_sort(c, s, 3, 1, &ds_b));
  OG_TRY(rec(EV_SORT_B));
  if (pk->sort_src[2] == 0) ds_l = ds_a;
  else if (pk->sort_src[2] == 1) ds_l = ds_b;
  else OG_TRY(sub_sort(c, s, 4, 2, &ds_l));
  OG_TRY(rec(EV_SORT_L));
  on(math);
  OG_TRY(wait(EV_ROWS));
  OG_TRY(sub_quotient(c, s));
  OG_TRY(rec(EV_QUOT));
  on(aux);
  OG_TRY(wait(EV_QUOT));
  OG_TRY(sub_sort_h(c, s, &dh));
  OG_TRY(rec(EV_SORT_H));
  on(math);
  {
    struct TailGuard {
      og_ctx* c;
      ~TailGuard() { c->tail_stream = nullptr; c->msm_tag = 0; c->after_heavy_ev = nullptr; }
    } tail_guard{ctx};
    ctx->tail_stream = tail;
    OG_TRY(wait(EV_ASSEMBLED));
    OG_TRY(wait(EV_SORT_A));
    ctx->msm_tag = 0;
    OG_TRY(msm_run(ctx, pk->a, ds_a, s.res(c, 0)));
    OG_TRY(wait(EV_SORT_B));
    ctx->msm_tag = 1;
    OG_TRY(msm_run(ctx, pk->b1, ds_b, s.res(c, 1)));
    ctx->msm_tag = 2;
    OG_TRY(msm_run(ctx, pk->b2, ds_b, s.res(c, 2)));
    OG_TRY(wait(EV_SORT_L));
    ctx->msm_tag = 3;
    OG_TRY(msm_l(c, s, ds_l));
    OG_TRY(wait(EV_SORT_H));
// ... 392 lines not shown
```

owshen_amd/csrc/ntt.hip:

```cpp
#include "ctx.h"
#include "field.hip.h"
#include "msm.hip.h"
#include "prover.h"

namespace og {

constexpr int NTT_TILE_LOG = 10;
constexpr int NTT_TILE = 1 << NTT_TILE_LOG;

struct NttPlan {
  int log_n = 0;
  uint8_t* consts = nullptr;
  uint8_t* tw_fwd = nullptr;
  uint8_t* tw_inv = nullptr;
  uint8_t* cs_fwd = nullptr;
  uint8_t* cs_fwd_ninv = nullptr;
  uint8_t* cs_inv_ninv = nullptr;
  uint8_t* cs_fwd_ninv_br = nullptr;
  uint8_t* cs_inv_ninv_br = nullptr;
};

__global__ void k_ntt_consts(int log_n, uint8_t* __restrict__ out) {
  if (threadIdx.x != 0 || blockIdx.x != 0) return;
  const uint32_t T[8] = {0x3e1f593fu, 0x9b970914u, 0x833e8487u, 0x181585d2u, 0x85045b68u, 0x131a029bu, 0x0644e72eu, 0x00000003u};
  Fr seven = fe_to_mont(fe_from_u32<FrParams>(7));
  Fr w = Fr::one();
  for (int i = 255; i >= 0; i--) {
    w = fe_sqr(w);
    if ((T[i >> 5] >> (i & 31)) & 1) w = fe_mul(w, seven);
  }
  for (int i = 28; i > log_n; i--) w = fe_sqr(w);
  Fr nn = fe_to_mont(fe_from_u32<FrParams>(1u << log_n));
  Fr gn = seven;
  for (int i = 0; i < log_n; i++) gn = fe_sqr(gn);
  Fr zc = fe_sub(gn, Fr::one());
  fe_store(out + 0 * 32, w);
  fe_store(out + 1 * 32, fe_inv(w));
  fe_store(out + 2 * 32, seven);
  fe_store(out + 3 * 32, fe_inv(seven));
  fe_store(out + 4 * 32, fe_inv(nn));
  fe_store(out + 5 * 32, fe_inv(zc));
  fe_store(out + 6 * 32, Fr::one());
}

__global__ void __launch_bounds__(256) k_pow_table(const uint8_t* __restrict__ consts, int ib, int ic, uint8_t* __restrict__ out, size_t n,
                                                  int rev_log) {
  size_t i = (size_t)blockIdx.x * blockDim.x + threadIdx.x;
  if (i >= n) return;
  Fr b = fe_load<FrParams>(consts + ib * 32);
  Fr acc = fe_load<FrParams>(consts + ic * 32);
  for (size_t e = rev_log ? (size_t)(__brevll((unsigned long long)i) >> (64 - rev_log)) : i; e; e >>= 1) {
    if (e & 1) acc = fe_mul(acc, b);
    b = fe_sqr(b);
  }
  fe_store(out + i * 32, acc);
}

__global__ void __launch_bounds__(256) k_ntt_prep(const uint8_t* __restrict__ in, size_t in_stride, uint8_t* __restrict__ out,
                                                 size_t out_stride, int log_n, const uint8_t* __restrict__ table, int to_mont) {
  size_t i = (size_t)blockIdx.x * blockDim.x + threadIdx.x;
  const size_t n = (size_t)1 << log_n;
  if (i >= n) return;
  const int g = blockIdx.y;
  Fr v = fe_load<FrParams>(in + (size_t)g * in_stride + i * 32);
  if (to_mont) v = fe_to_mont(v);
  if (table) v = fe_mul(v, fe_load<FrParams>(table + i * 32));
  size_t j = log_n ? (size_t)(__brevll((unsigned long long)i) >> (64 - log_n)) : 0;
  fe_store(out + (size_t)g * out_stride + j * 32, v);
}

__global__ void __launch_bounds__(256) k_ntt_post(uint8_t* __restrict__ data, size_t stride, size_t n,
                                                 const uint8_t* __restrict__ table, int from_mont) {
  size_t i = (size_t)blockIdx.x * blockDim.x + threadIdx.x;
  if (i >= n) return;
  const int g = blockIdx.y;
  uint8_t* p = data + (size_t)g * stride + i * 32;
  Fr v = fe_load<FrParams>(p);
  if (table) v = fe_mul(v, fe_load<FrParams>(table + i * 32));
  if (from_mont) v = fe_from_mont(v);
  fe_store(p, v);
}

__global__ void __launch_bounds__(256) k_ntt_stages(uint8_t* __restrict__ data, size_t stride, int log_n, int s0, int ns,
                                                   const uint8_t* __restrict__ tw) {
  __shared__ __align__(16) uint32_t lds[NTT_TILE * 8];
  const int g = blockIdx.y;
  uint8_t* base = data + (size_t)g * stride;
  const int tile_log = log_n < NTT_TILE_LOG ? log_n : NTT_TILE_LOG;
  const int tile = 1 << tile_log;
  const int lo_t_log = tile_log - ns;
  const int lo_t = 1 << lo_t_log;
  const size_t chunks_lo = ((size_t)1 << s0) >> lo_t_log;
  const size_t blk = blockIdx.x;
  const size_t hi = blk / chunks_lo, lo_base = (blk % chunks_lo) << lo_t_log;
  const size_t gbase = (hi << (s0 + ns)) | lo_base;
  for (int e = threadIdx.x; e < tile; e += 256) {
    int m = e >> lo_t_log, t = e & (lo_t - 1);
    const uint4* src = reinterpret_cast<const uint4*>(base + (gbase + ((size_t)m << s0) + t) * 32);
    uint4* dst = reinterpret_cast<uint4*>(&lds[e * 8]);
    dst[0] = src[0];
    dst[1] = src[1];
  }
  __syncthreads();
  for (int q = 0; q < ns; q++) {
    const int s = s0 + q;
    for (int b = threadIdx.x; b < tile / 2; b += 256) {
      int t = b & (lo_t - 1), mm = b >> lo_t_log;
      int m0 = ((mm >> q) << (q + 1)) | (mm & ((1 << q) - 1));
      int m1 = m0 | (1 << q);
      size_t j = ((size_t)(m0 & ((1 << q) - 1)) << s0) | (lo_base + t);
      size_t te = j << (log_n - s - 1);
      uint32_t* p0 = &lds[(m0 * lo_t + t) * 8];
      uint32_t* p1 = &lds[(m1 * lo_t + t) * 8];
      Fr u = fe_load<FrParams>(p0);
      Fr v = fe_mul(fe_load<FrParams>(p1), fe_load<FrParams>(tw + te * 32));
      fe_store(p0, fe_add(u, v));
      fe_store(p1, fe_sub(u, v));
    }
    __syncthreads();
  }
  for (int e = threadIdx.x; e < tile; e += 256) {
    int m = e >> lo_t_log, t = e & (lo_t - 1);
    uint4* dst = reinterpret_cast<uint4*>(base + (gbase + ((size_t)m << s0) + t) * 32);
    const uint4* src = reinterpret_cast<const uint4*>(&lds[e * 8]);
    dst[0] = src[0];
    dst[1] = src[1];
  }
}


struct NttBlock {
  const uint8_t* in;
  uint8_t* out;
  size_t stride;
  int log_n, s0, ns;
  const uint8_t* tw_dif;
  const uint8_t* mid;
  const uint8_t* tw_dit;
  const uint8_t* pw_a;
  const uint8_t* pw_b;
  const uint8_t* consts;
  int to_mont, from_mont;
};

constexpr int NTT_LIMBS = 9;

__device__ __forceinline__ Fr lds_get(const uint32_t* p) {
  Fr r;
#pragma unroll
  for (int i = 0; i < NTT_LIMBS; i++) r.l[i] = p[i];
  return r;
}
__device__ __forceinline__ void lds_put(uint32_t* p, const Fr& v) {
#pragma unroll
  for (int i = 0; i < NTT_LIMBS; i++) p[i] = v.l[i];
}

__global__ void __launch_bounds__(256) k_ntt_block(NttBlock a) {
  OG_FILLER_PRIO();
  __shared__ uint32_t lds[NTT_TILE * NTT_LIMBS];
  const int g = blockIdx.y;
  const int log_n = a.log_n, s0 = a.s0, ns = a.ns;
  const uint8_t* src = a.in + (size_t)g * a.stride;
  uint8_t* dst = a.out + (size_t)g * a.stride;
  const int tile_log = log_n < NTT_TILE_LOG ? log_n : NTT_TILE_LOG;
  const int tile = 1 << tile_log;
  const int lo_t_log = tile_log - ns;
  const int lo_t = 1 << lo_t_log;
  const size_t chunks_lo = ((size_t)1 << s0) >> lo_t_log;
  const size_t blk = blockIdx.x;
  const size_t hi = blk / chunks_lo, lo_base = (blk % chunks_lo) << lo_t_log;
  const size_t gbase = (hi << (s0 + ns)) | lo_base;
  for (int e = threadIdx.x; e < tile; e += 256) {
    const int m = e >> lo_t_log, t = e & (lo_t - 1);
    Fr v = fe_load<FrParams>(src + (gbase + ((size_t)m << s0) + t) * 32);
    if (a.to_mont) v = fe_to_mont(v);
    lds_put(&lds[e * NTT_LIMBS], v);
  }
  __syncthreads();
#pragma unroll 1
  for (int sweep = 0; sweep < 2; sweep++) {
    const uint8_t* tw = sweep == 0 ? a.tw_dif : a.tw_dit;
    if (sweep == 1 && a.mid && a.tw_dit) {
      for (int e = threadIdx.x; e < tile; e += 256) {
        const int m = e >> lo_t_log, t = e & (lo_t - 1);
        const size_t p = gbase + ((size_t)m << s0) + t;
        lds_put(&lds[e * NTT_LIMBS], fe_mul(lds_get(&lds[e * NTT_LIMBS]), fe_load<FrParams>(a.mid + p * 32)));
      }
      __syncthreads();
    }
    if (!tw) continue;
#pragma unroll 1
    for (int qq = 0; qq < ns; qq++) {
      const int q = sweep == 0 ? ns - 1 - qq : qq;
      const int s = s0 + q;
      for (int b = threadIdx.x; b < tile / 2; b += 256) {
        const int t = b & (lo_t - 1), mm = b >> lo_t_log;
        const int m0 = ((mm >> q) << (q + 1)) | (mm & ((1 << q) - 1));
        const int m1 = m0 | (1 << q);
        const size_t j = ((size_t)(m0 & ((1 << q) - 1)) << s0) | (lo_base + t);
        uint32_t* p0 = &lds[(m0 * lo_t + t) * NTT_LIMBS];
        uint32_t* p1 = &lds[(m1 * lo_t + t) * NTT_LIMBS];
        const Fr u = lds_get(p0), x = lds_get(p1);
        if (s == 0) {
          lds_put(p0, fe_add(u, x));
          lds_put(p1, fe_sub(u, x));
          continue;
        }
        const Fr w = fe_load<FrParams>(tw + (j << (log_n - s - 1)) * 32);
        if (sweep == 0) {
          lds_put(p0, fe_add(u, x));
          lds_put(p1, fe_mul(fe_sub_weak(u, x), w));
        } else {
          const Fr v = fe_mul(x, w);
          lds_put(p0, fe_add(u, v));
          lds_put(p1, fe_sub(u, v));
        }
      }
      __syncthreads();
    }
  }
  const uint8_t* pa = a.pw_a ? a.pw_a + (size_t)g * a.stride : nullptr;
  const uint8_t* pb = a.pw_b ? a.pw_b + (size_t)g * a.stride : nullptr;
  for (int e = threadIdx.x; e < tile; e += 256) {
    const int m = e >> lo_t_log, t = e & (lo_t - 1);
    const size_t p = gbase + ((size_t)m << s0) + t;
    Fr v = lds_get(&lds[e * NTT_LIMBS]);
    if (a.mid && !a.tw_dit) v = fe_mul(v, fe_load<FrParams>(a.mid + p * 32));
    if (pa) v = fe_mul(fe_sub(fe_mul(fe_load<FrParams>(pa + p * 32), fe_load<FrParams>(pb + p * 32)), v), fe_load<FrParams>(a.consts + 5 * 32));
    if (a.from_mont) v = fe_from_mont(v);
    fe_store(dst + p * 32, v);
  }
}

template <class M>
__host__ __device__ constexpr uint32_t kn_limb(uint32_t k, int i) {
  uint64_t c = 0;
  uint32_t out = 0;
  for (int j = 0; j <= i; j++) {
    const uint64_t v = (uint64_t)M::N[j] * k + c;
    out = j == 8 ? (uint32_t)v : (uint32_t)(v & MASK29);
    c = v >> 29;
  }
  return out;
}
template <class M>
__host__ __device__ constexpr uint32_t kn_neg_limb(uint32_t k, int i) {
  return kn_limb<M>(k, i) + (i < 8 ? (1u << 29) : 0u) - (i > 0 ? 1u : 0u);
}
static_assert(kn_neg_limb<FrParams>(4, 0) == FrParams::NEG4[0] && kn_neg_limb<FrParams>(4, 5) == FrParams::NEG4[5] &&
                  kn_neg_limb<FrParams>(4, 8) == FrParams::NEG4[8] && kn_limb<FrParams>(3, 2) == FrParams::N3[2] &&
                  kn_limb<FrParams>(5, 8) == FrParams::N5[8],
              "k N limbs");

template <uint32_t K>
struct KN {
  static constexpr uint32_t L[9] = {kn_limb<FrParams>(K, 0), kn_limb<FrParams>(K, 1), kn_limb<FrParams>(K, 2), kn_limb<FrParams>(K, 3),
                                    kn_limb<FrParams>(K, 4), kn_limb<FrParams>(K, 5), kn_limb<FrParams>(K, 6), kn_limb<FrParams>(K, 7),
                                    kn_limb<FrParams>(K, 8)};
  static constexpr uint32_t NEG[9] = {kn_neg_limb<FrParams>(K, 0), kn_neg_limb<FrParams>(K, 1), kn_neg_limb<FrParams>(K, 2),
                                      kn_neg_limb<FrParams>(K, 3), kn_neg_limb<FrParams>(K, 4), kn_neg_limb<FrParams>(K, 5),
                                      kn_neg_limb<FrParams>(K, 6), kn_neg_limb<FrParams>(K, 7), kn_neg_limb<FrParams>(K, 8)};
};

__device__ __forceinline__ Fr nt_add(const Fr& a, const Fr& b) {
  Fr r;
#pragma unroll
  for (int i = 0; i < 9; i++) r.l[i] = a.l[i] + b.l[i];
  return r;
}
template <uint32_t K>
__device__ __forceinline__ Fr nt_sub(const Fr& a, const Fr& b) {
  Fr r;
#pragma unroll
  for (int i = 0; i < 9; i++) r.l[i] = a.l[i] + (KN<K>::NEG[i] - b.l[i]);
  return r;
}
__device__ __forceinline__ Fr nt_norm(const Fr& a) {
  Fr r;
  normalize29u(r.l, a.l);
  return r;
}
template <uint32_t K>
__device__ __forceinline__ Fr nt_csub(const Fr& a) {
  uint32_t u[9];
  int32_t c = 0;
#pragma unroll
  for (int i = 0; i < 9; i++) {
    const int32_t v = (int32_t)a.l[i] - (int32_t)KN<K>::L[i] + c;
    u[i] = i < 8 ? ((uint32_t)v & MASK29) : (uint32_t)v;
    c = i < 8 ? (v >> 29) : (v < 0 ? -1 : 0);
  }
  Fr r;
#pragma unroll
  for (int i = 0; i < 9; i++) r.l[i] = c ? a.l[i] : u[i];
  return r;
}
__device__ __forceinline__ Fr nt_reduce_8n(const Fr& a) { return nt_csub<2>(nt_csub<4>(nt_norm(a))); }
__device__ __forceinline__ Fr nt_reduce_64n(const Fr& a) { return nt_csub<4>(nt_csub<8>(nt_csub<16>(nt_csub<32>(a)))); }

__global__ void __launch_bounds__(256) k_ntt_block4(NttBlock a) {
  OG_FILLER_PRIO();
  __shared__ uint32_t lds[NTT_TILE * NTT_LIMBS];
  const int g = blockIdx.y;
  const int log_n = a.log_n, s0 = a.s0, ns = a.ns;
  const uint8_t* src = a.in + (size_t)g * a.stride;
  uint8_t* dst = a.out + (size_t)g * a.stride;
  const int tile_log = log_n < NTT_TILE_LOG ? log_n : NTT_TILE_LOG;
  const int tile = 1 << tile_log;
  const int lo_t_log = tile_log - ns;
  const int lo_t = 1 << lo_t_log;
  const size_t chunks_lo = ((size_t)1 << s0) >> lo_t_log;
  const size_t blk = blockIdx.x;
  const size_t hi = blk / chunks_lo, lo_base = (blk % chunks_lo) << lo_t_log;
  const size_t gbase = (hi << (s0 + ns)) | lo_base;
  const size_t quarter = ((size_t)1 << log_n) >> 2;
  for (int e = threadIdx.x; e < tile; e += 256) {
    const int m = e >> lo_t_log, t = e & (lo_t - 1);
    Fr v = fe_load<FrParams>(src + (gbase + ((size_t)m << s0) + t) * 32);
    if (a.to_mont) v = fe_to_mont(v);
    lds_put(&lds[e * NTT_LIMBS], v);
  }
  __syncthreads();
  auto elem = [&](int m, int t) -> uint32_t* { return &lds[(m * lo_t + t) * NTT_LIMBS]; };
  if (a.tw_dif) {
    const uint8_t* tw = a.tw_dif;
    int q = ns - 2;
#pragma unroll 1
    for (; q >= 0; q -= 2) {
      const int s = s0 + q;
      for (int gi = threadIdx.x; gi < tile / 4; gi += 256) {
        const int t = gi & (lo_t - 1), mm = gi >> lo_t_log;
        const int base = ((mm >> q) << (q + 2)) | (mm & ((1 << q) - 1));
        uint32_t *p00 = elem(base, t), *p01 = elem(base | (1 << q), t), *p10 = elem(base | (2 << q), t), *p11 = elem(base | (3 << q), t);
        const size_t j1 = ((size_t)(base & ((1 << q) - 1)) << s0) | (lo_base + t);
        const size_t te2 = j1 << (log_n - s - 2);
        Fr x0 = lds_get(p00), x1 = lds_get(p01), x2 = lds_get(p10), x3 = lds_get(p11);
        const Fr w2 = fe_load<FrParams>(tw + te2 * 32), w3 = fe_load<FrParams>(tw + (te2 + quarter) * 32);
        const Fr a1 = nt_add(x0, x2), b1 = nt_add(x1, x3);
        const Fr c1 = fe_mul(nt_sub<4>(x0, x2), w2), d1 = fe_mul(nt_sub<4>(x1, x3), w3);
        const Fr b1n = nt_norm(b1);
        Fr y0 = nt_reduce_8n(nt_add(a1, b1)), y2 = nt_csub<2>(nt_norm(nt_add(c1, d1))), y1, y3;
        if (s == 0) {
          y1 = nt_csub<2>(nt_csub<4>(nt_csub<8>(nt_norm(nt_sub<5>(a1, b1n)))));
          y3 = fe_sub(c1, d1);
        } else {
          const Fr w1 = fe_load<FrParams>(tw + (j1 << (log_n - s - 1)) * 32);
          y1 = fe_mul(nt_sub<5>(a1, b1n), w1);
          y3 = fe_mul(nt_sub<4>(c1, d1), w1);
        }
        lds_put(p00, y0); lds_put(p01, y1); lds_put(p10, y2); lds_put(p11, y3);
      }
      __syncthreads();
    }
    if (q == -1) {
      const int s = s0;
      for (int b = threadIdx.x; b < tile / 2; b += 256) {
        const int t = b & (lo_t - 1), mm = b >> lo_t_log;
        uint32_t *p0 = elem(mm << 1, t), *p1 = elem((mm << 1) | 1, t);
        const Fr u = lds_get(p0), x = lds_get(p1);
        lds_put(p0, fe_add(u, x));
        if (s == 0) lds_put(p1, fe_sub(u, x));
        else lds_put(p1, fe_mul(nt_sub<4>(u, x), fe_load<FrParams>(tw + ((size_t)(lo_base + t) << (log_n - s - 1)) * 32)));
      }
      __syncthreads();
    }
  }
  if (a.mid && a.tw_dit) {
    for (int e = threadIdx.x; e < tile; e += 256) {
      const int m = e >> lo_t_log, t = e & (lo_t - 1);
      const size_t p = gbase + ((size_t)m << s0) + t;
      lds_put(&lds[e * NTT_LIMBS], fe_mul(lds_get(&lds[e * NTT_LIMBS]), fe_load<FrParams>(a.mid + p * 32)));
    }
    __syncthreads();
  }
  if (a.tw_dit) {
    const uint8_t* tw = a.tw_dit;
    int q = 0;
#pragma unroll 1
    for (; q + 1 < ns; q += 2) {
      const int s = s0 + q;
      for (int gi = threadIdx.x; gi < tile / 4; gi += 256) {
        const int t = gi & (lo_t - 1), mm = gi >> lo_t_log;
        const int base = ((mm >> q) << (q + 2)) | (mm & ((1 << q) - 1));
        uint32_t *p00 = elem(base, t), *p01 = elem(base | (1 << q), t), *p10 = elem(base | (2 << q), t), *p11 = elem(base | (3 << q), t);
        const size_t j1 = ((size_t)(base & ((1 << q) - 1)) << s0) | (lo_base + t);
        const size_t te2 = j1 << (log_n - s - 2);
        const Fr x0 = lds_get(p00), x1 = lds_get(p01), x2 = lds_get(p10), x3 = lds_get(p11);
        Fr v1 = x1, v3 = x3;
        if (s != 0) {
          const Fr w1 = fe_load<FrParams>(tw + (j1 << (log_n - s - 1)) * 32);
          v1 = fe_mul(x1, w1);
          v3 = fe_mul(x3, w1);
        }
        const Fr a1 = nt_add(x0, v1), c1 = nt_add(x2, v3);
        const Fr b1 = s != 0 ? nt_sub<3>(x0, v1) : nt_sub<5>(x0, v1), d1 = s != 0 ? nt_sub<3>(x2, v3) : nt_sub<5>(x2, v3);
        const Fr w2 = fe_load<FrParams>(tw + te2 * 32), w3 = fe_load<FrParams>(tw + (te2 + quarter) * 32);
        const Fr v2 = fe_mul(c1, w2), v4 = fe_mul(d1, w3);
        lds_put(p00, nt_norm(nt_add(a1, v2)));
        lds_put(p10, nt_norm(nt_sub<3>(a1, v2)));
        lds_put(p01, nt_norm(nt_add(b1, v4)));
        lds_put(p11, nt_norm(nt_sub<3>(b1, v4)));
      }
      __syncthreads();
    }
    if (q < ns) {
      const int s = s0 + q;
      for (int b = threadIdx.x; b < tile / 2; b += 256) {
        const int t = b & (lo_t - 1), mm = b >> lo_t_log;
        const int m0 = ((mm >> q) << (q + 1)) | (mm & ((1 << q) - 1));
        uint32_t *p0 = elem(m0, t), *p1 = elem(m0 | (1 << q), t);
        const size_t j = ((size_t)(m0 & ((1 << q) - 1)) << s0) | (lo_base + t);
        const Fr u = lds_get(p0), x = lds_get(p1);
        if (s == 0) {
          lds_put(p0, nt_norm(nt_add(u, x)));
          lds_put(p1, nt_norm(nt_sub<5>(u, x)));
        } else {
          const Fr v = fe_mul(x, fe_load<FrParams>(tw + (j << (log_n - s - 1)) * 32));
          lds_put(p0, nt_norm(nt_add(u, v)));
          lds_put(p1, nt_norm(nt_sub<3>(u, v)));
        }
      }
      __syncthreads();
    }
  }
  const uint8_t* pa = a.pw_a ? a.pw_a + (size_t)g * a.stride : nullptr;
  const uint8_t* pb = a.pw_b ? a.pw_b + (size_t)g * a.stride : nullptr;
  const bool lazy = a.tw_dit != nullptr;
  for (int e = threadIdx.x; e < tile; e += 256) {
    const int m = e >> lo_t_log, t = e & (lo_t - 1);
    const size_t p = gbase + ((size_t)m << s0) + t;
    Fr v = lds_get(&lds[e * NTT_LIMBS]);
    if (a.mid && !a.tw_dit) v = fe_mul(v, fe_load<FrParams>(a.mid + p * 32));
    if (pa) {
      const Fr ab = fe_mul(fe_load<FrParams>(pa + p * 32), fe_load<FrParams>(pb + p * 32));
      v = fe_mul(lazy ? nt_sub<40>(ab, v) : nt_sub<4>(ab, v), fe_load<FrParams>(a.consts + 5 * 32));
    } else if (lazy) {
      v = nt_reduce_64n(v);
    }
    if (a.from_mont) v = fe_from_mont(v);
    fe_store(dst + p * 32, v);
  }
}

__global__ void __launch_bounds__(256) k_bitrev_copy(const uint8_t* __restrict__ in, uint8_t* __restrict__ out, size_t stride, int log_n) {
  size_t i = (size_t)blockIdx.x * blockDim.x + threadIdx.x;
  if (i >= ((size_t)1 << log_n)) return;
  const size_t j = log_n ? (size_t)(__brevll((unsigned long long)i) >> (64 - log_n)) : 0;
  const uint4* s4 = reinterpret_cast<const uint4*>(in + (size_t)blockIdx.y * stride + i * 32);
  uint4* d4 = reinterpret_cast<uint4*>(out + (size_t)blockIdx.y * stride + j * 32);
  d4[0] = s4[0];
  d4[1] = s4[1];
}

static int ntt_plan(og_ctx* ctx, int log_n, NttPlan* out) {
  OG_REQUIRE(log_n >= 0 && log_n <= 28, "ntt: log_n must be 0..28 (Fr 2-adicity)");
  const size_t n = (size_t)1 << log_n;
  std::string key = "ntt" + std::to_string(log_n);
  NttPlan p;
  p.log_n = log_n;
  bool fresh = !arena_has(ctx, (key + ".consts").c_str());
  OG_TRY(arena_get(ctx, (key + ".consts").c_str(), 8 * 32, (void**)&p.consts));
  OG_TRY(arena_get(ctx, (key + ".twf").c_str(), (n / 2 + 1) * 32, (void**)&p.tw_fwd));
  OG_TRY(arena_get(ctx, (key + ".twi").c_str(), (n / 2 + 1) * 32, (void**)&p.tw_inv));
  OG_TRY(arena_get(ctx, (key + ".csf").c_str(), n * 32, (void**)&p.cs_fwd));
  OG_TRY(arena_get(ctx, (key + ".csfn").c_str(), n * 32, (void**)&p.cs_fwd_ninv));
  OG_TRY(arena_get(ctx, (key + ".csin").c_str(), n * 32, (void**)&p.cs_inv_ninv));
  OG_TRY(arena_get(ctx, (key + ".csfnb").c_str(), n * 32, (void**)&p.cs_fwd_ninv_br));
  OG_TRY(arena_get(ctx, (key + ".csinb").c_str(), n * 32, (void**)&p.cs_inv_ninv_br));
  if (fresh) {
    hipLaunchKernelGGL(k_ntt_consts, dim3(1), dim3(64), 0, ctx->stream, log_n, p.consts);
    size_t h = n / 2 ? n / 2 : 1;
    hipLaunchKernelGGL(k_pow_table, dim3(grid_for(h, 256)), dim3(256), 0, ctx->stream, p.consts, 0, 6, p.tw_fwd, h, 0);
    hipLaunchKernelGGL(k_pow_table, dim3(grid_for(h, 256)), dim3(256), 0, ctx->stream, p.consts, 1, 6, p.tw_inv, h, 0);
    hipLaunchKernelGGL(k_pow_table, dim3(grid_for(n, 256)), dim3(256), 0, ctx->stream, p.consts, 2, 6, p.cs_fwd, n, 0);
    hipLaunchKernelGGL(k_pow_table, dim3(grid_for(n, 256)), dim3(256), 0, ctx->stream, p.consts, 2, 4, p.cs_fwd_ninv, n, 0);
    hipLaunchKernelGGL(k_pow_table, dim3(grid_for(n, 256)), dim3(256), 0, ctx->stream, p.consts, 2, 4, p.cs_fwd_ninv_br, n, log_n);
    hipLaunchKernelGGL(k_pow_table, dim3(grid_for(n, 256)), dim3(256), 0, ctx->stream, p.consts, 3, 4, p.cs_inv_ninv_br, n, log_n);
    hipLaunchKernelGGL(k_pow_table, dim3(grid_for(n, 256)), dim3(256), 0, ctx->stream, p.consts, 3, 4, p.cs_inv_ninv, n, 0);
    OG_HIP(hipGetLastError());
  }
  *out = p;
  return OG_OK;
}

int ntt_domain_consts(og_ctx* ctx, int log_n, uint8_t** consts_d) {
  NttPlan p;
  OG_TRY(ntt_plan(ctx, log_n, &p));
  *consts_d = p.consts;
  return OG_OK;
}

static int ntt_core(og_ctx* ctx, const NttPlan& p, const uint8_t* in, size_t in_stride, uint8_t* out, size_t out_stride,
                    int batch, bool inverse, const uint8_t* prep_table, int to_mont) {
  const int log_n = p.log_n;
  const size_t n = (size_t)1 << log_n;
  hipLaunchKernelGGL(k_ntt_prep, dim3(grid_for(n, 256), batch), dim3(256), 0, ctx->stream, in, in_stride, out, out_stride,
                     log_n, prep_table, to_mont);
  OG_HIP(hipGetLastError());
  const uint8_t* tw = inverse ? p.tw_inv : p.tw_fwd;
  const int tile_log = log_n < NTT_TILE_LOG ? log_n : NTT_TILE_LOG;
  for (int s0 = 0; s0 < log_n;) {
    int ns = log_n - s0 < tile_log ? log_n - s0 : tile_log;
    size_t nblocks = n >> tile_log;
    hipLaunchKernelGGL(k_ntt_stages, dim3((unsigned)nblocks, batch), dim3(256), 0, ctx->stream, out, out_stride, log_n, s0, ns, tw);
    OG_HIP(hipGetLastError());
    s0 += ns;
  }
  return OG_OK;
}

static int ntt_post(og_ctx* ctx, uint8_t* data, size_t stride, size_t n, int batch, const uint8_t* table, int from_mont) {
  hipLaunchKernelGGL(k_ntt_post, dim3(grid_for(n, 256), batch), dim3(256), 0, ctx->stream, data, stride, n, table, from_mont);
  OG_HIP(hipGetLastError());
  return OG_OK;
}

int ntt_canonical(og_ctx* ctx, const uint8_t* in_d, uint8_t* out_d, int log_n, int batch, int inverse, int coset) {
  NttPlan p;
  OG_TRY(ntt_plan(ctx, log_n, &p));
  const size_t n = (size_t)1 << log_n, stride = n * 32;
  if (!inverse) {
    OG_TRY(ntt_core(ctx, p, in_d, stride, out_d, stride, batch, false, coset ? p.cs_fwd : nullptr, 1));
    OG_TRY(ntt_post(ctx, out_d, stride, n, batch, nullptr, 1));
  } else {
    OG_TRY(ntt_core(ctx, p, in_d, stride, out_d, stride, batch, true, nullptr, 1));
    uint8_t* ninv_tab = nullptr;
    if (!coset) {
      OG_TRY(arena_get(ctx, ("ntt" + std::to_string(log_n) + ".ninv").c_str(), n * 32, (void**)&ninv_tab));
      hipLaunchKernelGGL(k_pow_table, dim3(grid_for(n, 256)), dim3(256), 0, ctx->stream, p.consts, 6, 4, ninv_tab, n, 0);
      OG_HIP(hipGetLastError());
    }
    OG_TRY(ntt_post(ctx, out_d, stride, n, batch, coset ? p.cs_inv_ninv : ninv_tab, 1));
  }
  return OG_OK;
}

int h_poly_device(og_ctx* ctx, uint8_t* a, uint8_t* b, uint8_t* c, uint8_t* tmp, uint8_t* h_out, int log_d, int batch) {
  (void)tmp;
  NttPlan p;
  OG_TRY(ntt_plan(ctx, log_d, &p));
  const size_t d = (size_t)1 << log_d, stride = d * 32;
  const int tile_log = log_d < NTT_TILE_LOG ? log_d : NTT_TILE_LOG;
  const unsigned nblocks = (unsigned)(d >> tile_log);
  int bs[8], bn[8], nb = 0;
  for (int s0 = 0; s0 < log_d || nb == 0;) {
    const int ns = log_d - s0 < tile_log ? log_d - s0 : tile_log;
    bs[nb] = s0; bn[nb] = ns; nb++;
    s0 += ns;
    if (ns == 0) break;
  }
  const bool radix4 = OG_HOOK_INT("OG_NTT_RADIX4", 1) != 0;
  auto launch = [&](const NttBlock& blk) -> int {
    if (radix4)
      hipLaunchKernelGGL(k_ntt_block4, dim3(nblocks, batch), dim3(256), 0, ctx->stream, blk);
    else
      hipLaunchKernelGGL(k_ntt_block, dim3(nblocks, batch), dim3(256), 0, ctx->stream, blk);
    OG_HIP(hipGetLastError());
    return OG_OK;
  };
  auto block = [&](uint8_t* data, int k) {
    NttBlock x;
    x.in = data; x.out = data; x.stride = stride; x.log_n = log_d; x.s0 = bs[k]; x.ns = bn[k];
    x.tw_dif = nullptr; x.mid = nullptr; x.tw_dit = nullptr; x.pw_a = nullptr; x.pw_b = nullptr; x.consts = p.consts;
    x.to_mont = 0; x.from_mont = 0;
    return x;
  };
  uint8_t* arr[3] = {a, b, c};
  for (int k = 0; k < 3; k++) {
    for (int j = nb - 1; j >= 1; j--) {
      NttBlock x = block(arr[k], j);
      x.tw_dif = p.tw_inv;
      OG_TRY(launch(x));
    }
    NttBlock m = block(arr[k], 0);
    m.tw_dif = p.tw_inv; m.mid = p.cs_fwd_ninv_br; m.tw_dit = p.tw_fwd;
    if (k == 2 && nb == 1) { m.pw_a = a; m.pw_b = b; }
    OG_TRY(launch(m));
    for (int j = 1; j < nb; j++) {
      NttBlock x = block(arr[k], j);
      x.tw_dit = p.tw_fwd;
      if (k == 2 && j == nb - 1) { x.pw_a = a; x.pw_b = b; }
      OG_TRY(launch(x));
    }
  }
  for (int j = nb - 1; j >= 1; j--) {
    NttBlock x = block(c, j);
    x.tw_dif = p.tw_inv;
    OG_TRY(launch(x));
  }
  NttBlock f = block(c, 0);
  f.tw_dif = p.tw_inv; f.mid = p.cs_inv_ninv_br; f.from_mont = 1; f.out = h_out;
  OG_TRY(launch(f));
  return OG_OK;
}


__global__ void __launch_bounds__(256) k_to_mont_copy(const uint8_t* __restrict__ in, uint8_t* __restrict__ out, size_t n) {
  size_t i = (size_t)blockIdx.x * blockDim.x + threadIdx.x;
  if (i >= n) return;
  fe_store(out + i * 32, fe_to_mont(fe_load<FrParams>(in + i * 32)));
}

int h_poly_canonical(og_ctx* ctx, const uint8_t* a, const uint8_t* b, const uint8_t* c, int log_d, int batch, uint8_t* h_out) {
  const size_t d = (size_t)1 << log_d, tot = d * (size_t)batch;
  uint8_t* buf[4];
  const char* names[4] = {"hpoly.a", "hpoly.b", "hpoly.c", "hpoly.t"};
  for (int k = 0; k < 4; k++) OG_TRY(arena_get(ctx, names[k], tot * 32, (void**)&buf[k]));
  const uint8_t* src[3] = {a, b, c};
  for (int k = 0; k < 3; k++) {
    hipLaunchKernelGGL(k_to_mont_copy, dim3(grid_for(tot, 256)), dim3(256), 0, ctx->stream, src[k], buf[k], tot);
    OG_HIP(hipGetLastError());
  }
  OG_TRY(h_poly_device(ctx, buf[0], buf[1], buf[2], buf[3], buf[3], log_d, batch));
  hipLaunchKernelGGL(k_bitrev_copy, dim3(grid_for(d, 256), batch), dim3(256), 0, ctx->stream, buf[3], h_out, d * 32, log_d);
  OG_HIP(hipGetLastError());
  return OG_OK;
}

}
```

owshen_amd/csrc/prover.h:

```cpp
#pragma once
#include "ctx.h"

namespace og {

int ntt_domain_consts(og_ctx* ctx, int log_n, uint8_t** consts_d);
int ntt_canonical(og_ctx* ctx, const uint8_t* in_d, uint8_t* out_d, int log_n, int batch, int inverse, int coset);
int h_poly_device(og_ctx* ctx, uint8_t* a, uint8_t* b, uint8_t* c, uint8_t* tmp, uint8_t* h_out, int log_d, int batch);
int h_poly_canonical(og_ctx* ctx, const uint8_t* a, const uint8_t* b, const uint8_t* c, int log_d, int batch, uint8_t* h_out);

int spmv_canonical(og_ctx* ctx, const uint32_t* ptr_d, const uint32_t* col_d, const uint8_t* val_d, size_t n_rows,
                   const uint8_t* x_d, uint8_t* out_d);
int lagrange_evals(og_ctx* ctx, int log_d, const uint8_t tau[32], uint8_t* out_d);
int scalar_mul_fixed(og_ctx* ctx, int is_g2, const uint8_t* base_host, const uint8_t* scalars_d, size_t n, uint8_t* out_d);

int points_on_curve(og_ctx* ctx, int is_g2, const uint8_t* points, size_t n, uint32_t* flags);

int pk_load(og_ctx* ctx, const uint8_t* blob, size_t len, const uint8_t* rows, size_t rows_len, og_pk** out);
void pk_destroy(og_pk* pk);
bool row_form_pays(size_t rows_q, size_t wires_q);
void pk_query_form(const og_pk* pk, uint64_t out[20]);
void pk_info(const og_pk* pk, uint64_t out[4]);
void pk_windows(const og_pk* pk, uint64_t out[4]);
void pk_density(const og_pk* pk, uint64_t out[4]);
uint64_t pk_bytes(const og_pk* pk);

bool glv_pair_ok();
int prove_plan(og_ctx* ctx, const og_pk* pk, size_t n, uint32_t* sizes_out, size_t cap, size_t* count_out, int* mode_out);
int prove_batch_device(og_ctx* ctx, const og_pk* pk, const uint8_t* z_d, size_t n, const uint8_t* rs, uint8_t* proofs,
                       size_t* first_bad);
int prove_batch_host(og_ctx* ctx, const og_pk* pk, const uint8_t* z, size_t n, const uint8_t* rs, uint8_t* proofs);
int prove_partials_enqueue(og_ctx* ctx, const og_pk* pk, const uint8_t* z_d, size_t n, int win_rank, int win_world, uint8_t* partials_d,
                           og_job** job_out);
int prove_from_partials(og_ctx* ctx, const og_pk* pk, const uint8_t* gathered_d, int world, size_t n, const uint8_t* rs, uint8_t* proofs);

int job_wait(og_job* job);
int job_done_events(og_job* job, hipEvent_t* out);
bool job_is_live(og_ctx* ctx, og_job* job);
bool job_mark_waiting(og_job* job, bool on, uint64_t* id_out);
bool job_same(og_job* job, uint64_t id);
bool job_is_waited_for(og_job* job);
bool ctx_has_waiters(og_ctx* ctx);
int job_abandon(og_job* job);
int job_join_stream(og_job* job, hipStream_t st);

}
```

owshen_amd/csrc/ptau.hip:

```cpp
#include "ctx.h"
#include "field.hip.h"
#include "ec.hip.h"
#include "snarkfile.hip.h"
#include "keygen.h"
#include "key_blob.h"
#include "mimc7.hip.h"
#include "msm.hip.h"
#include "prover.h"
#include "verify_tower.h"
#include <string.h>
#include <stdlib.h>
#include <algorithm>
#include <vector>

namespace og {

__global__ void __launch_bounds__(64) k_g2_subgroup(const uint8_t* __restrict__ aff, size_t n, K256 order, uint32_t* __restrict__ flags) {
  const size_t i = (size_t)blockIdx.x * blockDim.x + threadIdx.x;
  if (i >= n) return;
  const G2XYZZ p = G2XYZZ::from_affine(G2Affine::load(aff + i * 128));
  const G2XYZZ q = ecntt_smul(p, order);
  if (!q.is_inf()) atomicOr(flags, 4u);
}

template <class T>
__global__ void __launch_bounds__(64) k_spmv_terms(const uint8_t* __restrict__ lag, const uint32_t* __restrict__ idx, const uint8_t* __restrict__ val,
                                                  size_t nnz, K256 m1, uint8_t* __restrict__ terms) {
  const size_t e = (size_t)blockIdx.x * blockDim.x + threadIdx.x;
  if (e >= nnz) return;
  XYZZ<T> p = XYZZ<T>::from_affine(Affine<T>::load(lag + (size_t)idx[e] * Affine<T>::BYTES));
  const K256 k = k256_load(val + e * 32);
  uint32_t hi = 0, dm = 0;
  int top = -1;
#pragma unroll
  for (int w = 0; w < 8; w++) {
    if (w) hi |= k.l[w];
    dm |= k.l[w] ^ m1.l[w];
    if (k.l[w]) top = 32 * w + 31 - __clz((int)k.l[w]);
  }
  if (dm == 0)
    p = xyzz_neg(p);
  else if (!(hi == 0 && k.l[0] == 1))
    p = ecntt_smul(p, k, top);
  p.store(terms + e * XYZZ<T>::BYTES);
}

template <class T>
__global__ void __launch_bounds__(64) k_seg_sum(const uint8_t* __restrict__ in, const uint32_t* __restrict__ ptr, size_t n, uint8_t* __restrict__ out,
                                               int affine) {
  const size_t c = (size_t)blockIdx.x * blockDim.x + threadIdx.x;
  if (c >= n) return;
  const uint32_t b = ptr[c], e = ptr[c + 1];
  XYZZ<T> acc = XYZZ<T>::inf();
#pragma unroll 1
  for (uint32_t i = b; i < e; i++) acc = xyzz_add(acc, XYZZ<T>::load(in + (size_t)i * XYZZ<T>::BYTES));
  if (!affine) {
    acc.store(out + c * XYZZ<T>::BYTES);
    return;
  }
  Affine<T> a = xyzz_to_affine(acc);
  a.x = FieldIO<T>::from_mont(a.x);
  a.y = FieldIO<T>::from_mont(a.y);
  a.store(out + c * Affine<T>::BYTES);
}

__global__ void __launch_bounds__(64) k_ptau_h(const uint8_t* __restrict__ tau, size_t d, uint8_t* __restrict__ out) {
  const size_t j = (size_t)blockIdx.x * blockDim.x + threadIdx.x;
  if (j + 1 >= d) return;
  const G1XYZZ hi = G1XYZZ::from_affine(G1Affine::load(tau + (j + d) * 64));
  G1Affine a = xyzz_to_affine(xyzz_madd_signed(hi, G1Affine::load(tau + j * 64), true));
  a.x = fe_from_mont(a.x);
  a.y = fe_from_mont(a.y);
  a.store(out + j * 64);
}

template <class T>
__global__ void __launch_bounds__(64) k_smul_uniform(const uint8_t* __restrict__ in, size_t n, K256 k, const uint8_t* __restrict__ b_mont,
                                                    uint8_t* __restrict__ out, uint32_t* __restrict__ flags) {
  const size_t i = (size_t)blockIdx.x * blockDim.x + threadIdx.x;
  if (i >= n) return;
  const Affine<T> c = Affine<T>::load(in + i * Affine<T>::BYTES);
  Affine<T> r = Affine<T>::inf();
  if (lem_or(c.x) | lem_or(c.y)) {
    if (!lem_lt(c.x) || !lem_lt(c.y)) {
      atomicOr(flags, 1u);
    } else {
      const Affine<T> m = {FieldIO<T>::to_mont(c.x), FieldIO<T>::to_mont(c.y)};
      const T b = FieldIO<T>::load(b_mont);
      if (!(f_sqr(m.y) == f_add(f_mul(f_sqr(m.x), m.x), b))) atomicOr(flags, 2u);
      r = xyzz_to_affine(ecntt_smul(XYZZ<T>::from_affine(m), k));
      r.x = FieldIO<T>::from_mont(r.x);
      r.y = FieldIO<T>::from_mont(r.y);
    }
  }
  r.store(out + i * Affine<T>::BYTES);
}

__global__ void __launch_bounds__(128) k_challenge_scalars(const uint32_t* __restrict__ consts, const uint8_t* __restrict__ seed, uint32_t section,
                                                          size_t n, uint8_t* __restrict__ out) {
  const size_t i = (size_t)blockIdx.x * blockDim.x + threadIdx.x;
  if (i >= n) return;
  const uint32_t idx[8] = {(uint32_t)i, section, 0, 0, 0, 0, 0, 0};
  const Fr h = fe_from_mont(mimc7_hash2<false>(consts, fe_to_mont(fe_load<FrParams>(seed)), fe_to_mont(fe_from_words<FrParams>(idx))));
  uint32_t w[8];
  fe_to_words(w, h);
  uint4* q = reinterpret_cast<uint4*>(out + i * 32);
  q[0] = make_uint4(w[0], w[1], w[2], w[3]);
  q[1] = make_uint4(0, 0, 0, 0);
}

template <class T>
__global__ void __launch_bounds__(256) k_canon_to_mont(const uint8_t* __restrict__ in, size_t n, const uint8_t* __restrict__ b_mont,
                                                      uint8_t* __restrict__ out_mont, uint32_t* __restrict__ flags) {
  const size_t i = (size_t)blockIdx.x * blockDim.x + threadIdx.x;
  if (i >= n) return;
  const Affine<T> c = Affine<T>::load(in + i * Affine<T>::BYTES);
  Affine<T> m = Affine<T>::inf();
  if (lem_or(c.x) | lem_or(c.y)) {
    if (!lem_lt(c.x) || !lem_lt(c.y)) {
      atomicOr(flags, 1u);
    } else {
      m = {FieldIO<T>::to_mont(c.x), FieldIO<T>::to_mont(c.y)};
      const T b = FieldIO<T>::load(b_mont);
      if (!(f_sqr(m.y) == f_add(f_mul(f_sqr(m.x), m.x), b))) {
        atomicOr(flags, 2u);
        m = Affine<T>::inf();
      }
    }
  }
  m.store(out_mont + i * Affine<T>::BYTES);
}

static const uint32_t FR_WORDS[8] = {0xf0000001u, 0x43e1f593u, 0x79b97091u, 0x2833e848u, 0x8181585du, 0xb85045b6u, 0xe131a029u, 0x30644e72u};
static K256 fr_order(uint32_t minus) {
  K256 k;
  memcpy(k.l, FR_WORDS, 32);
  k.l[0] -= minus;
  return k;
}

static const char* const PTAU_SEC[7] = {"", "section 1 (header)", "section 2 (tauG1)", "section 3 (tauG2)", "section 4 (alphaTauG1)", "section 5 (betaTauG1)",
                                        "section 6 (betaG2)"};

struct PtauHeader {
  uint32_t power = 0, ceremony_power = 0;
};

static int ptau_parse(const uint8_t* data, size_t len, const std::string& who, BinFile* bf, PtauHeader* hd) {
  OG_TRY(binfile_parse(data, len, "ptau", 1, who, bf));
  OG_REQUIRE(bf->sec.count(1), who + ": " + PTAU_SEC[1] + " missing");
  const uint8_t* h = bf->sec[1].first;
  OG_REQUIRE(bf->sec[1].second == 4 + 32 + 8 && rd32(h) == 32, who + ": " + PTAU_SEC[1] + " has the wrong length for a 32-byte base field");
  OG_REQUIRE(memcmp(h + 4, FQ_BYTES, 32) == 0, who + ": " + PTAU_SEC[1] + ": the base field is not BN254's");
  hd->power = rd32(h + 36);
  hd->ceremony_power = rd32(h + 40);
  OG_REQUIRE(hd->power <= 28 && hd->ceremony_power <= 28 && hd->power <= hd->ceremony_power, who + ": " + PTAU_SEC[1] + ": bad power " +
                                                                                               std::to_string(hd->power) + " / " + std::to_string(hd->ceremony_power));
  return OG_OK;
}

static int ptau_decode(og_ctx* ctx, ZDev& dev, BinFile& bf, int sec, bool g2, size_t n, size_t n_dev, std::vector<uint8_t>& canon, uint8_t** mont_d,
                       const std::string& who) {
  const size_t pb = g2 ? 128 : 64;
  std::vector<uint8_t> in(n_dev * pb, 0);
  memcpy(in.data(), bf.sec[sec].first, n * pb);
  canon.resize(n_dev * pb);
  OG_TRY(dev.get(n_dev * pb, mont_d));
  return lem_convert(ctx, dev, g2, false, in.data(), n_dev, canon.data(), *mont_d, who + ": " + PTAU_SEC[sec]);
}

static int g2_subgroup_flags(og_ctx* ctx, ZDev& dev, const uint8_t* mont_d, size_t n, bool* outside) {
  uint8_t* f_d;
  OG_TRY(dev.get(4, &f_d));
  OG_HIP(hipMemsetAsync(f_d, 0, 4, ctx->stream));
  hipLaunchKernelGGL(k_g2_subgroup, dim3(grid_for(n, 64)), dim3(64), 0, ctx->stream, mont_d, n, fr_order(0), (uint32_t*)f_d);
  OG_HIP(hipGetLastError());
  uint32_t flags = 0;
  OG_HIP(hipMemcpyAsync(&flags, f_d, 4, hipMemcpyDeviceToHost, ctx->stream));
  OG_HIP(hipStreamSynchronize(ctx->stream));
  *outside = flags != 0;
  return OG_OK;
}

static int g2_subgroup_check(og_ctx* ctx, ZDev& dev, const uint8_t* mont_d, size_t n, const std::string& who_sec) {
  bool outside = false;
  OG_TRY(g2_subgroup_flags(ctx, dev, mont_d, n, &outside));
  OG_REQUIRE(!outside, who_sec + ": a point is not in the order-r subgroup");
  return OG_OK;
}

constexpr uint32_t SEG = 32;

template <class T>
static int point_spmv(og_ctx* ctx, const uint8_t* lag_d, const std::vector<uint32_t>& tptr, const std::vector<uint32_t>& tidx,
                      const std::vector<uint8_t>& tval, size_t m, uint8_t* out_d) {
  const size_t nnz = tidx.size();
  ZDev dev;
  uint8_t *idx_d, *val_d, *cur_d;
  OG_TRY(dev.get(nnz * 4, &idx_d));
  OG_TRY(dev.get(nnz * 32, &val_d));
  OG_TRY(dev.get(nnz * XYZZ<T>::BYTES, &cur_d));
  if (nnz) {
    OG_HIP(hipMemcpyAsync(idx_d, tidx.data(), nnz * 4, hipMemcpyHostToDevice, ctx->stream));
    OG_HIP(hipMemcpyAsync(val_d, tval.data(), nnz * 32, hipMemcpyHostToDevice, ctx->stream));
    hipLaunchKernelGGL(k_spmv_terms<T>, dim3(grid_for(nnz, 64)), dim3(64), 0, ctx->stream, lag_d, (const uint32_t*)idx_d, val_d, nnz, fr_order(1), cur_d);
    OG_HIP(hipGetLastError());
  }
  std::vector<std::vector<uint32_t>> keep;
  std::vector<uint32_t> cp = tptr;
  for (;;) {
    uint32_t longest = 0;
    for (size_t i = 0; i < m; i++) longest = std::max(longest, cp[i + 1] - cp[i]);
    if (longest <= SEG) break;
    std::vector<uint32_t> chunk, next(m + 1, 0);
    for (size_t i = 0; i < m; i++) {
      for (uint32_t s = cp[i]; s < cp[i + 1]; s += SEG) chunk.push_back(s);
      next[i + 1] = (uint32_t)chunk.size();
    }
    const size_t n_chunks = chunk.size();
    chunk.push_back(cp[m]);
    uint8_t *p_d, *nxt_d;
    OG_TRY(dev.get((n_chunks + 1) * 4, &p_d));
    OG_TRY(dev.get(n_chunks * XYZZ<T>::BYTES, &nxt_d));
    keep.push_back(std::move(chunk));
    OG_HIP(hipMemcpyAsync(p_d, keep.back().data(), (n_chunks + 1) * 4, hipMemcpyHostToDevice, ctx->stream));
    hipLaunchKernelGGL(k_seg_sum<T>, dim3(grid_for(n_chunks, 64)), dim3(64), 0, ctx->stream, cur_d, (const uint32_t*)p_d, n_chunks, nxt_d, 0);
    OG_HIP(hipGetLastError());
    cur_d = nxt_d;
    cp.swap(next);
  }
  uint8_t* p_d;
  OG_TRY(dev.get((m + 1) * 4, &p_d));
  OG_HIP(hipMemcpyAsync(p_d, cp.data(), (m + 1) * 4, hipMemcpyHostToDevice, ctx->stream));
  hipLaunchKernelGGL(k_seg_sum<T>, dim3(grid_for(m, 64)), dim3(64), 0, ctx->stream, cur_d, (const uint32_t*)p_d, m, out_d, 1);
  OG_HIP(hipGetLastError());
  OG_HIP(hipStreamSynchronize(ctx->stream));
  return OG_OK;
}

static int ptau_sections(BinFile& bf, const PtauHeader& hd, const std::string& who) {
  const uint64_t np = 1ull << hd.power;
  const uint64_t want[7] = {0, 0, (2 * np - 1) * 64, np * 128, np * 64, np * 64, 128};
  for (uint32_t id = 2; id <= 6; id++) {
    OG_REQUIRE(bf.sec.count(id), who + ": " + PTAU_SEC[id] + " missing");
    OG_REQUIRE(bf.sec[id].second == want[id], who + ": " + PTAU_SEC[id] + " has " + std::to_string(bf.sec[id].second) + " bytes, power " +
                                                  std::to_string(hd.power) + " asks for " + std::to_string(want[id]));
  }
  return OG_OK;
}

static int ptau_setup(og_ctx* ctx, const og_r1cs* r, const uint8_t* data, size_t len, std::vector<uint8_t>& pk, std::vector<uint8_t>& vk,
               const std::string& who = "og_setup_ptau") {
  BinFile bf;
  PtauHeader hd;
  OG_TRY(ptau_parse(data, len, who, &bf, &hd));
  OG_TRY(ptau_sections(bf, hd, who));
  QapRows rows;
  OG_TRY(r1cs_qap_rows(r, who, &rows));
  const size_t m = r->n_wires, l = r->n_pub, n_rows = r->n_constraints + l + 1;
  int log_d = 1;
  while (((size_t)1 << log_d) < n_rows) log_d++;
  OG_REQUIRE(log_d <= 28, who + ": too many constraints for the 2^28 domain");
  OG_REQUIRE((uint32_t)log_d <= hd.power, who + ": " + PTAU_SEC[1] + ": power " + std::to_string(hd.power) + " is below the circuit's domain 2^" +
                                              std::to_string(log_d));
  const size_t d = (size_t)1 << log_d, nh = d - 1;
  std::vector<uint32_t> tptr[3], trow[3];
  std::vector<uint8_t> tval[3];
  for (int k = 0; k < 3; k++) csr_transpose(rows.ptr[k], rows.col[k], rows.val[k], n_rows, m, tptr[k], trow[k], tval[k]);

  std::lock_guard<std::mutex> lk(ctx->mu);
  OG_HIP(hipSetDevice(ctx->device));
  ctx->lane = 0;
  ctx->stream = ctx->lanes[0];
  ZDev dev;
  std::vector<uint8_t> tau_c, alpha_c, beta_c, tau2_c, beta2_c;
  uint8_t *tau_m, *alpha_m, *beta_m, *tau2_m, *beta2_m;
  OG_TRY(ptau_decode(ctx, dev, bf, 2, false, 2 * d - 1, 2 * d, tau_c, &tau_m, who));
  OG_REQUIRE(memcmp(tau_c.data(), G1_GEN_BYTES, 64) == 0, who + ": " + PTAU_SEC[2] + ": the first point is not the G1 generator");
  OG_TRY(ptau_decode(ctx, dev, bf, 3, true, d, d, tau2_c, &tau2_m, who));
  OG_REQUIRE(memcmp(tau2_c.data(), G2_GEN_BYTES, 128) == 0, who + ": " + PTAU_SEC[3] + ": the first point is not the G2 generator");
  OG_TRY(ptau_decode(ctx, dev, bf, 4, false, d, d, alpha_c, &alpha_m, who));
  OG_TRY(ptau_decode(ctx, dev, bf, 5, false, d, d, beta_c, &beta_m, who));
  OG_TRY(ptau_decode(ctx, dev, bf, 6, true, 1, 1, beta2_c, &beta2_m, who));
  OG_TRY(g2_subgroup_check(ctx, dev, tau2_m, d, who + ": " + PTAU_SEC[3]));
  OG_TRY(g2_subgroup_check(ctx, dev, beta2_m, 1, who + ": " + PTAU_SEC[6]));
  const FfRoots& f = ff_roots();
  OG_REQUIRE(f.ok, who + ": internal: the roots of unity are not what the field layer expects");
  std::vector<uint8_t> tw, post(32);
  pow_table(fe_inv(zfr_pow2k(f.w28_own, 28 - log_d)), Fr::one(), d / 2, tw);
  Fr nn = Fr::one();
  for (int i = 0; i < log_d; i++) nn = fe_dbl(nn);
  zfr_store(post.data(), fe_from_mont(fe_inv(nn)));
  uint8_t *lag1_d, *lag2_d;
  OG_TRY(dev.get(3 * d * 64, &lag1_d));
  OG_TRY(dev.get(d * 128, &lag2_d));
  OG_TRY(ecntt_run<Fq>(ctx, dev, tau_m, log_d, tw, nullptr, &post, true, d, lag1_d, true));
  OG_TRY(ecntt_run<Fq>(ctx, dev, alpha_m, log_d, tw, nullptr, &post, true, d, lag1_d + d * 64, true));
  OG_TRY(ecntt_run<Fq>(ctx, dev, beta_m, log_d, tw, nullptr, &post, true, d, lag1_d + 2 * d * 64, true));
  OG_TRY(ecntt_run<Fq2>(ctx, dev, tau2_m, log_d, tw, nullptr, &post, true, d, lag2_d, true));
  uint8_t *a_d, *b1_d, *b2_d, *kk_d, *h_d;
  OG_TRY(dev.get(m * 64, &a_d));
  OG_TRY(dev.get(m * 64, &b1_d));
  OG_TRY(dev.get(m * 128, &b2_d));
  OG_TRY(dev.get(m * 64, &kk_d));
  OG_TRY(dev.get(nh * 64, &h_d));
  OG_TRY(point_spmv<Fq>(ctx, lag1_d, tptr[0], trow[0], tval[0], m, a_d));
  OG_TRY(point_spmv<Fq>(ctx, lag1_d, tptr[1], trow[1], tval[1], m, b1_d));
  OG_TRY(point_spmv<Fq2>(ctx, lag2_d, tptr[1], trow[1], tval[1], m, b2_d));
  {
    const size_t nnz = trow[0].size() + trow[1].size() + trow[2].size();
    OG_REQUIRE(3 * (uint64_t)d < (1ull << 32) && nnz < (1ull << 32), who + ": circuit too large");
    std::vector<uint32_t> kptr(m + 1, 0), kidx;
    std::vector<uint8_t> kval;
    kidx.reserve(nnz);
    kval.reserve(nnz * 32);
    const uint32_t base[3] = {(uint32_t)(2 * d), (uint32_t)d, 0};
    for (size_t i = 0; i < m; i++) {
      for (int k = 0; k < 3; k++) {
        for (uint32_t e = tptr[k][i]; e < tptr[k][i + 1]; e++) kidx.push_back(base[k] + trow[k][e]);
        kval.insert(kval.end(), tval[k].begin() + (size_t)tptr[k][i] * 32, tval[k].begin() + (size_t)tptr[k][i + 1] * 32);
      }
      kptr[i + 1] = (uint32_t)kidx.size();
    }
    OG_TRY(point_spmv<Fq>(ctx, lag1_d, kptr, kidx, kval, m, kk_d));
  }
  hipLaunchKernelGGL(k_ptau_h, dim3(grid_for(d, 64)), dim3(64), 0, ctx->stream, tau_m, d, h_d);
  OG_HIP(hipGetLastError());
  std::vector<uint8_t> a_q(m * 64), b1_q(m * 64), b2_q(m * 128), kk(m * 64), h_q(nh * 64);
  OG_HIP(hipMemcpyAsync(a_q.data(), a_d, m * 64, hipMemcpyDeviceToHost, ctx->stream));
  OG_HIP(hipMemcpyAsync(b1_q.data(), b1_d, m * 64, hipMemcpyDeviceToHost, ctx->stream));
  OG_HIP(hipMemcpyAsync(b2_q.data(), b2_d, m * 128, hipMemcpyDeviceToHost, ctx->stream));
  OG_HIP(hipMemcpyAsync(kk.data(), kk_d, m * 64, hipMemcpyDeviceToHost, ctx->stream));
  OG_HIP(hipMemcpyAsync(h_q.data(), h_d, nh * 64, hipMemcpyDeviceToHost, ctx->stream));
  OG_HIP(hipStreamSynchronize(ctx->stream));
  KeyParts parts;
  parts.m = m; parts.l = l; parts.log_d = log_d; parts.n_rows = n_rows;
  parts.alpha1 = alpha_c.data(); parts.beta1 = beta_c.data(); parts.delta1 = G1_GEN_BYTES;
  parts.beta2 = beta2_c.data(); parts.gamma2 = G2_GEN_BYTES; parts.delta2 = G2_GEN_BYTES;
  parts.query[0] = a_q.data(); parts.query[1] = b1_q.data(); parts.query[2] = b2_q.data();
  parts.query[3] = kk.data() + (l + 1) * 64; parts.query[4] = h_q.data();
  parts.ic = kk.data();
  key_blobs(parts, rows, pk, vk);
  return OG_OK;
}

template <class T>
static int smul_uniform(og_ctx* ctx, ZDev& dev, const uint8_t* in, size_t n, const K256& k, uint8_t* out, const std::string& who) {
  if (n == 0) return OG_OK;
  uint32_t flags = 0;
  OG_TRY(lem_run(ctx, dev, Affine<T>::BYTES == 128, false, in, n, out, nullptr, &flags, [&](uint8_t* in_d, uint8_t* c_d, uint8_t* out_d, uint32_t* f_d) {
    hipLaunchKernelGGL(k_smul_uniform<T>, dim3(grid_for(n, 64)), dim3(64), 0, ctx->stream, in_d, n, k, c_d + 32, out_d, f_d);
  }));
  OG_REQUIRE(!(flags & 1), who + ": a point coordinate of the key is not below the base-field modulus");
  OG_REQUIRE(!(flags & 2), who + ": a point of the key is not on its curve");
  return OG_OK;
}

static int pk_contribute(og_ctx* ctx, const uint8_t* pkb, size_t pk_len, const uint8_t* vkb, size_t vk_len, const uint8_t dd[32], std::vector<uint8_t>& pk,
                  std::vector<uint8_t>& vk) {
  const std::string who = "og_pk_contribute";
  const Fr dv = zfr_load(dd);
  OG_REQUIRE(fe_lt_modulus(dv) && !dv.is_zero(), who + ": the contribution must be canonical (below the group order) and non-zero");
  PkView pv;
  VkView vv;
  OG_TRY(pk_view(pkb, pk_len, who, &pv));
  OG_REQUIRE(pv.flags <= 1 && pv.word9 == 0, who + ": bad key header");
  OG_TRY(vk_view(vkb, vk_len, who, &vv));
  OG_REQUIRE(vk_is_of_pk(vv, pv), who + ": the verifying key does not belong to this proving key (n_pub, alpha, beta or delta differ)");
  const size_t nl = pv.nl, nh = pv.nh, l_off = pv.off(pv.query[3]), h_off = pv.off(pv.query[4]);
  K256 kd, kinv;
  memcpy(kd.l, dd, 32);
  uint8_t inv_b[32];
  zfr_store(inv_b, fe_from_mont(fe_inv(fe_to_mont(dv))));
  memcpy(kinv.l, inv_b, 32);

  std::lock_guard<std::mutex> lk(ctx->mu);
  OG_HIP(hipSetDevice(ctx->device));
  ctx->lane = 0;
  ctx->stream = ctx->lanes[0];
  ZDev dev;
  pk.assign(pkb, pkb + pk_len);
  vk.assign(vkb, vkb + vk_len);
  std::vector<uint8_t> lh((nl + nh) * 64), lh_out((nl + nh) * 64);
  memcpy(lh.data(), pkb + l_off, nl * 64);
  memcpy(lh.data() + nl * 64, pkb + h_off, nh * 64);
  OG_TRY(smul_uniform<Fq>(ctx, dev, lh.data(), nl + nh, kinv, lh_out.data(), who));
  memcpy(&pk[l_off], lh_out.data(), nl * 64);
  memcpy(&pk[h_off], lh_out.data() + nl * 64, nh * 64);
  OG_TRY(smul_uniform<Fq>(ctx, dev, pv.delta1, 1, kd, &pk[PK_DELTA1], who));
// ... 315 lines not shown
```

owshen_amd/groth16.py:

```python
import ctypes as C
import struct

import numpy as np

from . import api
from .api import FR, FR_MODULUS as R

G1_GEN = (1, 2)
G2_GEN = ((10857046999023057135944570762232829481370756359578518086990519993285655852781,
           11559732032986387107991004021392285783925812861821192530917403151452391805634),
          (8495653923123431417604973247489272438418190587263600148770280649306958101930,
           4082367875863433681332203403145435568316851327593401208105741076214120093531))
PK_MAGIC = b"OWPK0001"
VK_MAGIC = b"OWVK0001"


def _le(v):
    return int(v).to_bytes(32, "little")


G1_GEN_BYTES = _le(G1_GEN[0]) + _le(G1_GEN[1])
G2_GEN_BYTES = _le(G2_GEN[0][0]) + _le(G2_GEN[0][1]) + _le(G2_GEN[1][0]) + _le(G2_GEN[1][1])


def _pad32(b):
    return b + b"\0" * (-len(b) % 32)


class SparseMatrix:

    def __init__(self, ptr, col, val, n_cols):
        self.ptr = np.ascontiguousarray(ptr, dtype=np.uint32)
        self.col = np.ascontiguousarray(col, dtype=np.uint32)
        self.val = np.ascontiguousarray(val, dtype=np.uint8).reshape(-1, 32)
        self.n_cols = n_cols
        assert self.ptr[0] == 0 and self.ptr[-1] == self.col.shape[0] == self.val.shape[0]

    @property
    def n_rows(self):
        return self.ptr.shape[0] - 1

    @property
    def nnz(self):
        return self.col.shape[0]

    @classmethod
    def from_rows(cls, rows, n_cols):
        ptr = np.zeros(len(rows) + 1, dtype=np.uint32)
        cols, vals = [], []
        for i, r in enumerate(rows):
            for c in sorted(r):
                v = r[c] % R
                if v:
                    cols.append(c)
                    vals.append(_le(v))
            ptr[i + 1] = len(cols)
        val = np.frombuffer(b"".join(vals), dtype=np.uint8).reshape(-1, 32) if vals else np.zeros((0, 32), np.uint8)
        return cls(ptr, np.array(cols, dtype=np.uint32), val, n_cols)

    def transpose(self):
        rows = np.repeat(np.arange(self.n_rows, dtype=np.uint32), np.diff(self.ptr.astype(np.int64)))
        order = np.argsort(self.col, kind="stable")
        ptr = np.zeros(self.n_cols + 1, dtype=np.int64)
        np.add.at(ptr, self.col.astype(np.int64) + 1, 1)
        ptr = np.cumsum(ptr).astype(np.uint32)
        return SparseMatrix(ptr, rows[order], self.val[order], self.n_rows)


class R1CS:

    def __init__(self, n_wires, n_pub, a, b, c):
        assert a.n_rows == b.n_rows == c.n_rows
        self.n_wires, self.n_pub, self.n_constraints = n_wires, n_pub, a.n_rows
        self.a, self.b, self.c = self._with_consistency(a, True), self._with_consistency(b, False), self._with_consistency(c, False)
        need = self.n_rows
        self.log_d = max(1, (need - 1).bit_length())

    def _with_consistency(self, mat, identity):
        extra = self.n_pub + 1
        if identity:
            one = np.frombuffer(_le(1), dtype=np.uint8)
            ptr = np.concatenate([mat.ptr, mat.ptr[-1] + np.arange(1, extra + 1, dtype=np.uint32)])
            col = np.concatenate([mat.col, np.arange(extra, dtype=np.uint32)])
            val = np.concatenate([mat.val, np.tile(one, (extra, 1))])
        else:
            ptr = np.concatenate([mat.ptr, np.full(extra, mat.ptr[-1], dtype=np.uint32)])
            col, val = mat.col, mat.val
        return SparseMatrix(ptr, col, val, self.n_wires)

    @property
    def n_rows(self):
        return self.n_constraints + self.n_pub + 1

    @property
    def domain_size(self):
        return 1 << self.log_d

    @classmethod
    def from_constraints(cls, n_wires, n_pub, constraints):
        return cls(n_wires, n_pub,
                   SparseMatrix.from_rows([x[0] for x in constraints], n_wires),
                   SparseMatrix.from_rows([x[1] for x in constraints], n_wires),
                   SparseMatrix.from_rows([x[2] for x in constraints], n_wires))


def _r1cs_handle(lib, r1cs):
    nc = r1cs.n_constraints
    keep = []
    ptrs, cols, vals = (C.c_void_p * 3)(), (C.c_void_p * 3)(), (C.c_void_p * 3)()
    for k, mat in enumerate((r1cs.a, r1cs.b, r1cs.c)):
        ptr = np.ascontiguousarray(mat.ptr[: nc + 1])
        nnz = int(ptr[nc])
        col = np.ascontiguousarray(mat.col[:nnz])
        val = np.ascontiguousarray(mat.val[:nnz])
        keep += [ptr, col, val]
        ptrs[k], cols[k], vals[k] = ptr.ctypes.data, col.ctypes.data, val.ctypes.data
    h = C.c_void_p()
    rc = lib.og_r1cs_from_csr(r1cs.n_wires, r1cs.n_pub, nc, ptrs, cols, vals, C.byref(h))
    return rc, h, keep


def vk_from_bytes(blob):
    assert blob[:8] == VK_MAGIC
    n_pub = struct.unpack("<Q", blob[8:16])[0]
    o = 16
    out = {"alpha_g1": blob[o:o + 64], "beta_g2": blob[o + 64:o + 192], "gamma_g2": blob[o + 192:o + 320], "delta_g2": blob[o + 320:o + 448]}
    out["ic"] = np.frombuffer(blob[o + 448:], dtype=np.uint8).reshape(n_pub + 1, 64).copy()
    return out


class ProvingKeyBlob(bytes):
    rows = None


def setup(ctx, r1cs, tau, alpha, beta, gamma, delta):
    for v in (tau, alpha, beta, gamma, delta):
        assert 0 < v < R
    lib = ctx._lib
    rc, h, _keep = _r1cs_handle(lib, r1cs)
    ctx._check(rc)
    try:
        toxic = (C.c_uint8 * 160).from_buffer_copy(b"".join(_le(v) for v in (tau, alpha, beta, gamma, delta)))
        pk_p, vk_p, pk_n, vk_n = C.c_void_p(), C.c_void_p(), C.c_size_t(), C.c_size_t()
        ext_p, ext_n = C.c_void_p(), C.c_size_t()
        ctx._pre()
        ctx._check(lib.og_setup_rows(ctx._h, h, toxic, C.byref(pk_p), C.byref(pk_n), C.byref(vk_p), C.byref(vk_n), C.byref(ext_p), C.byref(ext_n)))
        try:
            pk = ProvingKeyBlob(C.string_at(pk_p, pk_n.value))
            vk = C.string_at(vk_p, vk_n.value)
            if ext_p.value and ext_n.value:
                pk.rows = C.string_at(ext_p, ext_n.value)
        finally:
            lib.og_blob_free(pk_p)
            lib.og_blob_free(vk_p)
            lib.og_blob_free(ext_p)
    finally:
        lib.og_r1cs_free(h)
    return pk, vk_from_bytes(vk)


class ProvingKey:

    def __init__(self, ctx, blob):
        self.ctx = ctx
        h = C.c_void_p()
        buf = (C.c_uint8 * len(blob)).from_buffer_copy(blob)
        rows = getattr(blob, "rows", None)
        if rows:
            ext = (C.c_uint8 * len(rows)).from_buffer_copy(rows)
            ctx._pre()
            ctx._check(ctx._lib.og_pk_load_rows(ctx._h, buf, len(blob), ext, len(rows), C.byref(h)))
        else:
            ctx._check(ctx._lib.og_pk_load(ctx._h, buf, len(blob), C.byref(h)))
        self._h = h
        info = (C.c_uint64 * 4)()
        ctx._check(ctx._lib.og_pk_info(h, info))
        self.n_wires, self.n_pub, self.log_d, self.n_rows = (int(x) for x in info)

    def density(self):
        d = (C.c_uint64 * 4)()
        self.ctx._check(self.ctx._lib.og_pk_density(self._h, d))
        return dict(zip(("a", "b", "l", "h"), (int(x) for x in d)))

    def hbm_bytes(self):
        out = C.c_uint64()
        self.ctx._check(self.ctx._lib.og_pk_bytes(self._h, C.byref(out)))
        return int(out.value)

    def plan(self, n):
        sizes, cnt, mode = (C.c_uint32 * 4096)(), C.c_size_t(), C.c_int()
        self.ctx._check(self.ctx._lib.og_prove_plan(self.ctx._h, self._h, n, sizes, 4096, C.byref(cnt), C.byref(mode)))
        return ("serial", "query fan-out", "symmetric lanes", "stage pipeline")[mode.value], [int(sizes[k]) for k in range(min(cnt.value, 4096))]

    def windows(self):
        d = (C.c_uint64 * 4)()
        self.ctx._check(self.ctx._lib.og_pk_windows(self._h, d))
        return dict(zip(("a", "b", "l", "h"), (int(x) for x in d)))

    def query_forms(self):
        d = (C.c_uint64 * 20)()
        self.ctx._check(self.ctx._lib.og_pk_query_form(self._h, d))
        names = ("a", "b1", "b2", "l", "h")
        return {q: {"form": "row" if d[4 * k] else "wire", "points": int(d[4 * k + 1]), "bits": int(d[4 * k + 2]), "table": names[int(d[4 * k + 3])]}
                for k, q in enumerate(names)}

    @staticmethod
    def _rs_bytes(rs):
        if isinstance(rs, np.ndarray):
            return np.ascontiguousarray(rs, dtype=np.uint8).reshape(-1, 64)
        return np.frombuffer(b"".join(_le(r) + _le(s) for r, s in rs), dtype=np.uint8).reshape(-1, 64).copy()

    def prove(self, witness, r, s):
        return self.prove_batch(np.ascontiguousarray(witness, dtype=np.uint8)[None], [(r, s)])[0].tobytes()

    def prove_batch(self, witnesses, rs):
        w = np.ascontiguousarray(witnesses, dtype=np.uint8)
        n = w.shape[0]
        assert w.shape[1:] == (self.n_wires, 32)
        rsb = self._rs_bytes(rs)
        assert rsb.shape[0] == n
        out = np.zeros((n, 256), dtype=np.uint8)
        ctx = self.ctx
        ctx._check(ctx._lib.og_prove_batch(ctx._h, self._h, w.ctypes.data_as(C.c_void_p), n,
                                           rsb.ctypes.data_as(C.c_void_p), out.ctypes.data_as(C.c_void_p)))
        return out

    def prove_batch_device(self, witnesses_d, rs):
        n = witnesses_d.shape[0]
        assert tuple(witnesses_d.shape[1:]) == (self.n_wires, 32)
        rsb = self._rs_bytes(rs)
        assert rsb.shape[0] == n
        out = np.zeros((n, 256), dtype=np.uint8)
        ctx = self.ctx
        ctx._pre()
        ctx._check(ctx._lib.og_prove_batch_d(ctx._h, self._h, ctx.ptr(witnesses_d), n, rsb.ctypes.data_as(C.c_void_p),
                                             out.ctypes.data_as(C.c_void_p)))
        return out

    PARTIAL_BYTES = 768

    def prove_partials_device(self, witnesses_d, win_rank, win_world):
        n = witnesses_d.shape[0]
        assert tuple(witnesses_d.shape[1:]) == (self.n_wires, 32)
        ctx = self.ctx
        part = ctx.empty(n * self.PARTIAL_BYTES)
        ctx._pre()
        ctx._check(ctx._lib.og_prove_partials_d(ctx._h, self._h, ctx.ptr(witnesses_d), n, win_rank, win_world, ctx.ptr(part)))
        return part

    def prove_from_partials(self, gathered_d, world, rs):
        rsb = self._rs_bytes(rs)
        n = rsb.shape[0]
        assert int(np.prod(gathered_d.shape)) == world * n * self.PARTIAL_BYTES
        out = np.zeros((n, 256), dtype=np.uint8)
        ctx = self.ctx
        ctx._pre()
        ctx._check(ctx._lib.og_prove_from_partials_d(ctx._h, self._h, ctx.ptr(gathered_d), world, n, rsb.ctypes.data_as(C.c_void_p),
                                                     out.ctypes.data_as(C.c_void_p)))
        return out

    def close(self):
        if getattr(self, "_h", None):
            self.ctx._lib.og_pk_free(self._h)
            self._h = None

    def __del__(self):
        try:
            self.close()
        except Exception:
            pass



def vk_to_bytes(vk):
    ic = np.ascontiguousarray(vk["ic"], dtype=np.uint8).reshape(-1, 64)
    return (VK_MAGIC + struct.pack("<Q", ic.shape[0] - 1) + bytes(vk["alpha_g1"]) + bytes(vk["beta_g2"]) + bytes(vk["gamma_g2"]) +
            bytes(vk["delta_g2"]) + ic.tobytes())


def verify(vk_blob, public_inputs, proof, lib=None):
    if lib is None:
        from ._lib import lib
    if isinstance(public_inputs, np.ndarray):
        pub = np.ascontiguousarray(public_inputs, dtype=np.uint8).reshape(-1, 32)
    else:
        pub = np.frombuffer(b"".join(int(x).to_bytes(32, "little") for x in public_inputs), dtype=np.uint8).reshape(-1, 32).copy()
    ok = C.c_int(0)
    vkb = (C.c_uint8 * len(vk_blob)).from_buffer_copy(bytes(vk_blob))
    pf = (C.c_uint8 * 256).from_buffer_copy(bytes(proof))
    rc = lib.og_verify(vkb, len(vk_blob), pub.ctypes.data_as(C.c_void_p), pub.shape[0], pf, C.byref(ok))
    if rc != 0:
        raise api.OwshenGpuError(rc, lib.og_last_error().decode("utf-8", "replace"))
    return bool(ok.value)


class VerifyingKey:

    def __init__(self, ctx, vk_blob):
        self.ctx = ctx
        self._h = None
        blob = bytes(vk_blob)
        buf = (C.c_uint8 * max(len(blob), 1)).from_buffer_copy(blob or b"\0")
        h = C.c_void_p()
        ctx._check(ctx._lib.og_vk_load(ctx._h, buf, len(blob), C.byref(h)))
        self._h = h
        info = (C.c_uint64 * 4)()
        ctx._check(ctx._lib.og_vk_info(self._h, info))
        self.n_pub, self.walk_steps, self.table_bytes, self.device_bytes = (int(x) for x in info)

    def verify_batch(self, public_inputs, proofs):
        ctx = self.ctx
        if isinstance(proofs, np.ndarray):
            proofs = ctx.to_device(np.ascontiguousarray(proofs, dtype=np.uint8).reshape(-1, 256))
        n = int(proofs.shape[0]) if len(proofs.shape) > 1 else int(proofs.shape[0]) // 256
        if isinstance(public_inputs, np.ndarray):
            public_inputs = ctx.to_device(np.ascontiguousarray(public_inputs, dtype=np.uint8).reshape(n, self.n_pub, 32)) if self.n_pub and n else None
        if public_inputs is not None:
            assert int(np.prod(public_inputs.shape)) == n * self.n_pub * 32, "public_inputs must be [n, n_pub, 32]"
        ok = np.zeros(n, dtype=np.uint32)
        ctx._pre()
        ctx._check(ctx._lib.og_verify_batch_d(ctx._h, self._h, ctx.ptr(public_inputs) if n and self.n_pub else None, ctx.ptr(proofs) if n else None, n,
                                              ok.ctypes.data_as(C.c_void_p)))
        return ok.astype(bool)

    def close(self):
        if getattr(self, "_h", None):
            self.ctx._lib.og_vk_free(self._h)
            self._h = None

    def __enter__(self):
        return self

    def __exit__(self, *exc):
        self.close()

    def __del__(self):
        try:
            self.close()
        except Exception:
            pass


from .evm import proof_to_evm_calldata
```

Before: 865.7.

## Add evaluation-form H query that skips the coset iNTT in the quotient

At key load, derives a new H basis by running EC-NTTs over the key's H query, so the prover can MSM the quotient's coset evaluations directly instead of converting back to coefficients. It also folds the C contribution into the L table through a point-SpMV, letting the C polynomial's handling be absorbed into the precomputed bases. The point-SpMV helpers move out of ptau into a shared header, and a load-time randomized check confirms the derived tables match the original queries. This cuts per-proof NTT work in h_poly at the cost of heavier key loading and a different MSM size for H (d instead of d-1).

```diff
diff --git a/include/owshen_gpu.h b/include/owshen_gpu.h
--- a/include/owshen_gpu.h
+++ b/include/owshen_gpu.h
@@ -83,6 +83,9 @@
 int og_pk_info(const og_pk* pk, uint64_t info[4]);
 int og_pk_density(const og_pk* pk, uint64_t out[4]);
 int og_pk_windows(const og_pk* pk, uint64_t out[4]);
+#define OG_QUERY_FORM_WIRE 0
+#define OG_QUERY_FORM_ROW 1
+#define OG_QUERY_FORM_EVAL 2
 int og_pk_load_rows(og_ctx* ctx, const uint8_t* blob, size_t len, const uint8_t* rows, size_t rows_len, og_pk** out);
 int og_pk_query_form(const og_pk* pk, uint64_t out[20]);
 int og_prove(og_ctx* ctx, const og_pk* pk, const uint8_t* witness, const uint8_t rs[64], uint8_t proof_out[256]);
diff --git a/owshen_amd/_abi.py b/owshen_amd/_abi.py
--- a/owshen_amd/_abi.py
+++ b/owshen_amd/_abi.py
@@ -131,6 +131,9 @@
 }
 
 
+QUERY_FORMS = ("wire", "row", "eval")
+
+
 def bind(lib):
     for name, (res, args) in SIGNATURES.items():
         f = getattr(lib, name)
diff --git a/owshen_amd/csrc/groth16.hip b/owshen_amd/csrc/groth16.hip
--- a/owshen_amd/csrc/groth16.hip
+++ b/owshen_amd/csrc/groth16.hip
@@ -6,6 +6,8 @@
 #include "glv.h"
 #include "ec.hip.h"
 #include "key_blob.h"
+#include "keygen.h"
+#include "point_spmv.hip.h"
 #include <string.h>
 #include <algorithm>
 #include <iterator>
@@ -34,6 +36,7 @@
   size_t rows_q[2] = {0, 0};
   int c_wire[3] = {0, 0, 0};
   bool merge_lh = false;
+  bool h_form = false;
   bool c_is_ab = false;
   uint8_t* consts1 = nullptr;
   uint8_t* consts2 = nullptr;
@@ -290,6 +293,158 @@
     OG_REQUIRE(memcmp(got, got + 128, pb) == 0,
                who + ": row-basis extension: its points do not reproduce the key's " + p.name + " query (not the Lagrange basis of this key's tau)");
   }
+  return OG_OK;
+}
+
+static bool h_form_pays(bool has_c, int log_d) { return has_c && log_d >= 14; }
+
+struct HFormTables {
+  std::vector<uint8_t> e;
+  std::vector<uint8_t> lg;
+};
+static int h_form_derive(og_ctx* ctx, const og_pk* pk, const PkView& v, const std::string& who, HFormTables* out) {
+  const size_t m = pk->m, d = pk->d, nl = v.nl, nh = v.nh, npub1 = pk->n_pub + 1, n_rows = pk->n_rows, nnz = pk->nnz[2];
+  const int log_d = (int)pk->log_d;
+  const FfRoots& f = ff_roots();
+  OG_REQUIRE(f.ok, who + ": internal: the roots of unity are not what the field layer expects");
+  OG_REQUIRE((uint64_t)d + nl < (1ull << 32) && (uint64_t)nnz + nl < (1ull << 32), who + ": key too large for the evaluation form");
+  const Fr seven = fe_to_mont(fe_from_u32<FrParams>(7));
+  Fr nn = Fr::one();
+  for (int i = 0; i < log_d; i++) nn = fe_dbl(nn);
+  const Fr scale = fe_mul(fe_inv(fe_sub(zfr_pow2k(seven, log_d), Fr::one())), fe_inv(nn));
+  std::vector<uint8_t> tw, pre, post_e(32), post_f(32);
+  pow_table(fe_inv(zfr_pow2k(f.w28_own, 28 - log_d)), Fr::one(), d / 2, tw);
+  pow_table(fe_inv(seven), Fr::one(), d, pre);
+  zfr_store(post_e.data(), fe_from_mont(scale));
+  zfr_store(post_f.data(), fe_from_mont(fe_neg(scale)));
+  ZDev dev;
+  uint8_t *raw_d, *hm_d, *base_d, *e_d, *lg_d;
+  OG_TRY(dev.get(std::max(d, nl) * 64, &raw_d));
+  OG_TRY(dev.get(d * 64, &hm_d));
+  OG_TRY(dev.get((d + nl) * 64, &base_d));
+  OG_TRY(dev.get(d * 64, &e_d));
+  OG_TRY(dev.get(m * 64, &lg_d));
+  OG_HIP(hipMemsetAsync(raw_d, 0, d * 64, ctx->stream));
+  OG_HIP(hipMemcpyAsync(raw_d, v.query[4], nh * 64, hipMemcpyHostToDevice, ctx->stream));
+  OG_TRY(import_points_g1(ctx, raw_d, hm_d, d));
+  OG_TRY(ecntt_run<Fq>(ctx, dev, hm_d, log_d, tw, &pre, &post_e, true, d, e_d, false));
+  OG_TRY(ecntt_run<Fq>(ctx, dev, hm_d, log_d, tw, nullptr, &post_f, true, d, base_d, true));
+  OG_HIP(hipStreamSynchronize(ctx->stream));
+  if (nl) {
+    OG_HIP(hipMemcpyAsync(raw_d, v.query[3], nl * 64, hipMemcpyHostToDevice, ctx->stream));
+    OG_TRY(import_points_g1(ctx, raw_d, base_d + d * 64, nl));
+  }
+  std::vector<uint32_t> cptr(n_rows + 1), ccol(nnz), tptr, trow, kptr(m + 1, 0), kidx;
+  std::vector<uint8_t> cval(v.val[2], v.val[2] + nnz * 32), tval, kval;
+  for (size_t r = 0; r <= n_rows; r++) cptr[r] = rd32(v.ptr[2] + r * 4);
+  for (size_t e = 0; e < nnz; e++) ccol[e] = rd32(v.col[2] + e * 4);
+  csr_transpose(cptr, ccol, cval, n_rows, m, tptr, trow, tval);
+  kidx.reserve(nnz + nl);
+  kval.reserve((nnz + nl) * 32);
+  uint8_t one[32] = {1};
+  for (size_t i = 0; i < m; i++) {
+    kidx.insert(kidx.end(), trow.begin() + tptr[i], trow.begin() + tptr[i + 1]);
+    kval.insert(kval.end(), tval.begin() + (size_t)tptr[i] * 32, tval.begin() + (size_t)tptr[i + 1] * 32);
+    if (i >= npub1 && !all_zero(v.query[3] + (i - npub1) * 64, 64)) {
+      kidx.push_back((uint32_t)(d + (i - npub1)));
+      kval.insert(kval.end(), one, one + 32);
+    }
+    kptr[i + 1] = (uint32_t)kidx.size();
+  }
+  OG_TRY(point_spmv<Fq>(ctx, base_d, kptr, kidx, kval, m, lg_d));
+  out->e.resize(d * 64);
+  out->lg.resize(m * 64);
+  OG_HIP(hipMemcpyAsync(out->e.data(), e_d, d * 64, hipMemcpyDeviceToHost, ctx->stream));
+  OG_HIP(hipMemcpyAsync(out->lg.data(), lg_d, m * 64, hipMemcpyDeviceToHost, ctx->stream));
+  OG_HIP(hipStreamSynchronize(ctx->stream));
+  const long long corrupt = OG_HOOK_INT("OG_H_FORM_CORRUPT", 0);
+  if (corrupt == 1 && d >= 2) memcpy(&out->e[64], &out->e[0], 64);
+  for (size_t i = 0; i < m && corrupt == 2; i++) {
+    if (all_zero(&out->lg[i * 64], 64)) continue;
+    memcpy(&out->lg[i * 64], &out->e[0], 64);
+    break;
+  }
+  return OG_OK;
+}
+
+static int h_form_check(og_ctx* ctx, const og_pk* pk, const PkView& v, uint8_t* stage, const std::string& who) {
+  const size_t m = pk->m, d = pk->d, nl = v.nl, nh = v.nh, npub1 = pk->n_pub + 1;
+  const int log_d = (int)pk->log_d;
+  std::vector<uint8_t> sc((m + d) * 32);
+  uint64_t x = rd64(v.query[4]) ^ rd64(v.query[4] + 32) ^ ((uint64_t)m << 32) ^ d;
+  for (size_t i = 0; i < (m + d) * 4; i++) {
+    x += 0x9e3779b97f4a7c15ull;
+    uint64_t z = x;
+    z = (z ^ (z >> 30)) * 0xbf58476d1ce4e5b9ull;
+    z = (z ^ (z >> 27)) * 0x94d049bb133111ebull;
+    z ^= z >> 31;
+    if ((i & 3) == 3) z &= (1ull << 60) - 1;
+    memcpy(&sc[i * 8], &z, 8);
+  }
+  memset(&sc[(m + d - 1) * 32], 0, 32);
+  std::vector<uint8_t> bh(2 * d * 32);
+  const Fr zc = fe_sub(zfr_pow2k(fe_to_mont(fe_from_u32<FrParams>(7)), log_d), Fr::one());
+  for (size_t i = 0; i < d; i++) {
+    fe_store(&bh[i * 32], zc);
+    fe_store(&bh[(d + i) * 32], Fr::one());
+  }
+  ZDev dev;
+  uint8_t *sc_d, *ue_d, *a_d, *b_d, *h_d, *res_d;
+  OG_TRY(dev.get((m + d) * 32, &sc_d));
+  OG_TRY(dev.get(d * 32, &ue_d));
+  OG_TRY(dev.get(2 * d * 32, &a_d));
+  OG_TRY(dev.get(2 * d * 32, &b_d));
+  OG_TRY(dev.get(2 * d * 32, &h_d));
+  OG_TRY(dev.get(5 * 128, &res_d));
+  const uint8_t *rho_d = sc_d, *u_d = sc_d + m * 32;
+  OG_HIP(hipMemcpyAsync(sc_d, sc.data(), sc.size(), hipMemcpyHostToDevice, ctx->stream));
+  OG_HIP(hipMemcpyAsync(b_d, bh.data(), bh.size(), hipMemcpyHostToDevice, ctx->stream));
+  OG_HIP(hipMemsetAsync(res_d, 0, 5 * 128, ctx->stream));
+  OG_TRY(ntt_canonical(ctx, u_d, ue_d, log_d, 1, 0, 0));
+  hipLaunchKernelGGL(k_fr_to_mont, dim3(grid_for(d, 256)), dim3(256), 0, ctx->stream, ue_d, a_d, d);
+  OG_HIP(hipGetLastError());
+  hipLaunchKernelGGL(k_spmv, dim3(grid_for(d, 256), 1), dim3(256), 0, ctx->stream, pk->ptr[2], pk->col[2], pk->val[2], (size_t)pk->n_rows, d, rho_d,
+                     (size_t)0, a_d + d * 32, (size_t)0, 1, 1, SPMV_LONG, (uint8_t*)nullptr, (size_t)0);
+  OG_HIP(hipGetLastError());
+  if (pk->n_long[2]) {
+    hipLaunchKernelGGL(k_spmv_long, dim3(pk->n_long[2], 1), dim3(256), 0, ctx->stream, pk->long_rows[2], pk->ptr[2], pk->col[2], pk->val[2], rho_d,
+                       (size_t)0, a_d + d * 32, (size_t)0, 1, 1, (uint8_t*)nullptr, (size_t)0);
+    OG_HIP(hipGetLastError());
+  }
+  OG_TRY(h_poly_device(ctx, a_d, b_d, nullptr, nullptr, h_d, log_d, 2, 1));
+  DigitSort ds;
+  OG_TRY(msm_digit_sort(ctx, 0, h_d, d * 32, d, nullptr, 2, pk->h->c, 1, &ds));
+  OG_TRY(msm_run(ctx, pk->h, ds, res_d));
+  if (pk->n_dense[2]) {
+    OG_TRY(msm_digit_sort(ctx, 0, rho_d, m * 32, pk->n_dense[2], pk->map[2], 1, pk->l->c, 1, &ds));
+    OG_TRY(msm_run(ctx, pk->l, ds, res_d + 256));
+  }
+  const int cw = (int)msm_pick_c(std::max(nh, nl));
+  og_bases *hb = nullptr, *lb = nullptr;
+  struct Drop { og_bases*& b; ~Drop() { bases_destroy(b); } } drop_h{hb}, drop_l{lb};
+  OG_HIP(hipMemcpyAsync(stage, v.query[4], nh * 64, hipMemcpyHostToDevice, ctx->stream));
+  OG_TRY(bases_create(ctx, 0, stage, nh, cw, 0, &hb));
+  OG_TRY(msm_digit_sort(ctx, 0, u_d, d * 32, nh, nullptr, 1, cw, 0, &ds));
+  OG_TRY(msm_run(ctx, hb, ds, res_d + 384));
+  if (nl) {
+    OG_HIP(hipStreamSynchronize(ctx->stream));
+    OG_HIP(hipMemcpyAsync(stage, v.query[3], nl * 64, hipMemcpyHostToDevice, ctx->stream));
+    OG_TRY(bases_create(ctx, 0, stage, nl, cw, 0, &lb));
+    OG_TRY(msm_digit_sort(ctx, 0, rho_d + npub1 * 32, m * 32, nl, nullptr, 1, cw, 0, &ds));
+    OG_TRY(msm_run(ctx, lb, ds, res_d + 512));
+  }
+  uint8_t res[5 * 128];
+  OG_HIP(hipMemcpyAsync(res, res_d, sizeof res, hipMemcpyDeviceToHost, ctx->stream));
+  OG_HIP(hipStreamSynchronize(ctx->stream));
+  const G1XYZZ h1 = G1XYZZ::load(res), h2 = G1XYZZ::load(res + 128), ln = G1XYZZ::load(res + 256), ho = G1XYZZ::load(res + 384),
+               lo = G1XYZZ::load(res + 512);
+  auto same = [](const G1XYZZ& p, const G1XYZZ& q) {
+    const G1Affine a = xyzz_to_affine(p), b = xyzz_to_affine(q);
+    return fe_canon(a.x) == fe_canon(b.x) && fe_canon(a.y) == fe_canon(b.y);
+  };
+  OG_REQUIRE(same(h1, ho), who + ": evaluation form: the derived H tables do not reproduce the key's H query");
+  OG_REQUIRE(same(xyzz_add(xyzz_add(ln, h1), h2), xyzz_add(lo, ho)),
+             who + ": evaluation form: the C fold in the derived L tables does not reproduce the key's L and H queries");
   return OG_OK;
 }
 
@@ -331,7 +486,7 @@
     }
   }
   uint8_t* stage = nullptr;
-  const size_t stage_bytes = std::max<size_t>(std::max<size_t>(std::max<size_t>(512, m * 128), nh * 64), rows ? pk->n_rows * 128 : 0);
+  const size_t stage_bytes = std::max<size_t>(std::max<size_t>(std::max<size_t>(512, m * 128), pk->d * 64), rows ? pk->n_rows * 128 : 0);
   OG_HIP(hipMalloc((void**)&stage, stage_bytes));
   struct Guard { uint8_t* p; ~Guard() { if (p) (void)hipFree(p); } } guard{stage};
   OG_HIP(hipMalloc((void**)&pk->consts1, 256));
@@ -349,6 +504,18 @@
   OG_HIP(hipMemcpy(pk->consts2_h, pk->consts2, 256, hipMemcpyDeviceToHost));
   OG_HIP(hipMemcpy(pk->fb_delta2_h.data(), pk->fb_delta2, pk->fb_delta2_h.size(), hipMemcpyDeviceToHost));
   int ch = (int)msm_pick_query_c(nh);
+  HFormTables hf;
+  {
+    const long long force = OG_HOOK_INT("OG_H_FORM", -1);
+    pk->h_form = !pk->c_is_ab && pk->log_d >= 1 && force != 0 && (force == 1 || h_form_pays(true, (int)pk->log_d));
+  }
+  if (pk->h_form) {
+    OG_REQUIRE(ctx->jobs[0] == nullptr && ctx->jobs[1] == nullptr,
+               who + ": a submitted prove call has not been waited for (og_job_wait) -- this key takes the evaluation form, and its load-time check uses the call's scratch");
+    ctx->lane = 0;
+    ctx->stream = ctx->lanes[0];
+    OG_TRY(h_form_derive(ctx, pk, v, who, &hf));
+  }
   std::vector<uint32_t> wire[3];
   for (size_t i = 0; i < m; i++) {
     if (!all_zero(v.query[0] + i * 64, 64)) wire[0].push_back((uint32_t)i);
@@ -357,6 +524,11 @@
   for (size_t i = 0; i < nl; i++)
     if (!all_zero(v.query[3] + i * 64, 64)) wire[2].push_back((uint32_t)(i + pk->n_pub + 1));
   for (int k = 0; k < 3; k++) pk->n_real[k] = wire[k].size();
+  if (pk->h_form) {
+    wire[2].clear();
+    for (size_t i = 0; i < m; i++)
+      if (!all_zero(&hf.lg[i * 64], 64)) wire[2].push_back((uint32_t)i);
+  }
   std::vector<uint32_t> rlist;
   if (rows) {
     const long long force = OG_HOOK_INT("OG_ROW_FORM", -1);
@@ -399,7 +571,7 @@
     OG_HIP(hipMemcpyAsync(pk->map[k], wire[k].data(), wire[k].size() * 4, hipMemcpyHostToDevice, ctx->stream));
   }
   OG_HIP(hipStreamSynchronize(ctx->stream));
-  std::vector<uint8_t> host(std::max<size_t>(std::max<size_t>(std::max<size_t>(1, m * 128), nh * 64), rlist.size() * 128));
+  std::vector<uint8_t> host(std::max<size_t>(std::max<size_t>(std::max<size_t>(1, m * 128), pk->d * 64), rlist.size() * 128));
   if (!rlist.empty()) {
     for (int g2 = 0; g2 < (pk->row[1] ? 2 : 1); g2++) {
       const size_t pb = g2 ? 128 : 64;
@@ -421,28 +593,33 @@
     if (pk->row[q.mapk]) continue;
     const size_t pb = q.is_g2 ? 128 : 64;
     const std::vector<uint32_t>& w = wire[q.mapk];
-    const size_t shift = q.src == 3 ? pk->n_pub + 1 : 0;
-    const size_t q_len = q.src == 3 ? nl : m;
+    const bool folded = q.src == 3 && pk->h_form;
+    const uint8_t* src = folded ? hf.lg.data() : v.query[q.src];
+    const size_t shift = q.src == 3 && !folded ? pk->n_pub + 1 : 0;
+    const size_t q_len = q.src == 3 && !folded ? nl : m;
     for (size_t k = 0; k < w.size(); k++) {
-      if (w[k] >= shift && w[k] - shift < q_len) memcpy(host.data() + k * pb, v.query[q.src] + (w[k] - shift) * pb, pb);
+      if (w[k] >= shift && w[k] - shift < q_len) memcpy(host.data() + k * pb, src + (w[k] - shift) * pb, pb);
       else memset(host.data() + k * pb, 0, pb);
     }
     OG_HIP(hipMemcpyAsync(stage, host.data(), w.size() * pb, hipMemcpyHostToDevice, ctx->stream));
     OG_TRY(bases_create(ctx, q.is_g2, stage, w.size(), (int)msm_pick_query_c(w.size()), 1, q.dst));
   }
-  for (size_t k = 0; k < nh; k++) {
+  const size_t h_pts = pk->h_form ? pk->d : nh;
+  if (pk->h_form) memcpy(host.data(), hf.e.data(), h_pts * 64);
+  for (size_t k = 0; k < nh && !pk->h_form; k++) {
     size_t r = 0;
     for (uint64_t bit = 0; bit < pk->log_d; bit++) r |= ((k >> bit) & 1) << (pk->log_d - 1 - bit);
     memcpy(host.data() + k * 64, v.query[4] + r * 64, 64);
   }
-  OG_HIP(hipMemcpyAsync(stage, host.data(), nh * 64, hipMemcpyHostToDevice, ctx->stream));
+  OG_HIP(hipMemcpyAsync(stage, host.data(), h_pts * 64, hipMemcpyHostToDevice, ctx->stream));
   const int cl = pk->l->c;
-  const bool h_takes_cl = cl == ch || (cl == 17 && (double)nh * 15 < (double)(1u << 23) && nh >= 512) || (cl == 16 && nh >= 512);
+  const bool h_takes_cl = cl == ch || (cl == 17 && (double)h_pts * 15 < (double)(1u << 23) && nh >= 512) || (cl == 16 && nh >= 512);
   if (OG_HOOK_INT("OG_MERGE_LH", 1) && h_takes_cl && (cl == 16 || cl == 17 || cl == ch)) {
     ch = cl;
     pk->merge_lh = true;
   }
-  OG_TRY(bases_create(ctx, 0, stage, nh, ch, 1, &pk->h));
+  OG_TRY(bases_create(ctx, 0, stage, h_pts, ch, 1, &pk->h));
+  if (pk->h_form) OG_TRY(h_form_check(ctx, pk, v, stage, who));
   return OG_OK;
 }
 
@@ -459,7 +636,7 @@
   const og_bases* q[5] = {pk->a, pk->b1, pk->b2, pk->l, pk->h};
   const int mapk[5] = {0, 1, 1, 2, -1};
   for (int k = 0; k < 5; k++) {
-    out[4 * k + 0] = mapk[k] >= 0 && pk->row[mapk[k]] ? 1 : 0;
+    out[4 * k + 0] = mapk[k] >= 0 && pk->row[mapk[k]] ? 1 : k >= 3 && pk->h_form ? 2 : 0;
     out[4 * k + 1] = q[k]->n;
     out[4 * k + 2] = (uint64_t)q[k]->c;
     int first = k;
@@ -775,7 +952,7 @@
                                 1, c.sh ? c.sh->rank : 0, c.sh ? c.sh->world : 1, out);
 }
 static int sub_sort_h(const ProveCall& c, const SubBatch& s, DigitSort* out) {
-  return msm_digit_sort_windows(c.ctx, 2, s.h, c.pk->d * 32, c.pk->d - 1, nullptr, s.sb, c.pk->h->c, 1, c.sh ? c.sh->rank : 0,
+  return msm_digit_sort_windows(c.ctx, 2, s.h, c.pk->d * 32, c.pk->h_form ? c.pk->d : c.pk->d - 1, nullptr, s.sb, c.pk->h->c, 1, c.sh ? c.sh->rank : 0,
                                 c.sh ? c.sh->world : 1, out);
 }
 
@@ -888,7 +1065,7 @@
 
 static int sub_quotient(const ProveCall& c, const SubBatch& s) {
   ProfScope ps(c.ctx, PROF_HPOLY, (double)c.pk->d * s.sb);
-  OG_TRY(h_poly_device(c.ctx, s.ev[0], s.ev[1], s.ev[2], s.tmp, s.h, (int)c.pk->log_d, s.sb));
+  OG_TRY(h_poly_device(c.ctx, s.ev[0], s.ev[1], s.ev[2], s.tmp, s.h, (int)c.pk->log_d, s.sb, c.pk->h_form ? 1 : 0));
   OG_STEP(c.ctx, "g16.hpoly");
   return OG_OK;
 }
diff --git a/owshen_amd/csrc/ntt.hip b/owshen_amd/csrc/ntt.hip
--- a/owshen_amd/csrc/ntt.hip
+++ b/owshen_amd/csrc/ntt.hip
@@ -141,6 +141,7 @@
   const uint8_t* pw_b;
   const uint8_t* consts;
   int to_mont, from_mont;
+  int pw_mul;
 };
 
 constexpr int NTT_LIMBS = 9;
@@ -222,12 +223,14 @@
   }
   const uint8_t* pa = a.pw_a ? a.pw_a + (size_t)g * a.stride : nullptr;
   const uint8_t* pb = a.pw_b ? a.pw_b + (size_t)g * a.stride : nullptr;
+  const bool pw_mul = a.pw_mul != 0;
   for (int e = threadIdx.x; e < tile; e += 256) {
     const int m = e >> lo_t_log, t = e & (lo_t - 1);
     const size_t p = gbase + ((size_t)m << s0) + t;
     Fr v = lds_get(&lds[e * NTT_LIMBS]);
     if (a.mid && !a.tw_dit) v = fe_mul(v, fe_load<FrParams>(a.mid + p * 32));
-    if (pa) v = fe_mul(fe_sub(fe_mul(fe_load<FrParams>(pa + p * 32), fe_load<FrParams>(pb + p * 32)), v), fe_load<FrParams>(a.consts + 5 * 32));
+    if (pa && pw_mul) v = fe_mul(fe_load<FrParams>(pa + p * 32), v);
+    else if (pa) v = fe_mul(fe_sub(fe_mul(fe_load<FrParams>(pa + p * 32), fe_load<FrParams>(pb + p * 32)), v), fe_load<FrParams>(a.consts + 5 * 32));
     if (a.from_mont) v = fe_from_mont(v);
     fe_store(dst + p * 32, v);
   }
@@ -427,12 +430,15 @@
   const uint8_t* pa = a.pw_a ? a.pw_a + (size_t)g * a.stride : nullptr;
   const uint8_t* pb = a.pw_b ? a.pw_b + (size_t)g * a.stride : nullptr;
   const bool lazy = a.tw_dit != nullptr;
+  const bool pw_mul = a.pw_mul != 0;
   for (int e = threadIdx.x; e < tile; e += 256) {
     const int m = e >> lo_t_log, t = e & (lo_t - 1);
     const size_t p = gbase + ((size_t)m << s0) + t;
     Fr v = lds_get(&lds[e * NTT_LIMBS]);
     if (a.mid && !a.tw_dit) v = fe_mul(v, fe_load<FrParams>(a.mid + p * 32));
-    if (pa) {
+    if (pa && pw_mul) {
+      v = fe_mul(fe_load<FrParams>(pa + p * 32), lazy ? nt_reduce_64n(v) : v);
+    } else if (pa) {
       const Fr ab = fe_mul(fe_load<FrParams>(pa + p * 32), fe_load<FrParams>(pb + p * 32));
       v = fe_mul(lazy ? nt_sub<40>(ab, v) : nt_sub<4>(ab, v), fe_load<FrParams>(a.consts + 5 * 32));
     } else if (lazy) {
@@ -536,7 +542,7 @@
   return OG_OK;
 }
 
-int h_poly_device(og_ctx* ctx, uint8_t* a, uint8_t* b, uint8_t* c, uint8_t* tmp, uint8_t* h_out, int log_d, int batch) {
+int h_poly_device(og_ctx* ctx, uint8_t* a, uint8_t* b, uint8_t* c, uint8_t* tmp, uint8_t* h_out, int log_d, int batch, int coset_form) {
   (void)tmp;
   NttPlan p;
   OG_TRY(ntt_plan(ctx, log_d, &p));
@@ -563,10 +569,27 @@
     NttBlock x;
     x.in = data; x.out = data; x.stride = stride; x.log_n = log_d; x.s0 = bs[k]; x.ns = bn[k];
     x.tw_dif = nullptr; x.mid = nullptr; x.tw_dit = nullptr; x.pw_a = nullptr; x.pw_b = nullptr; x.consts = p.consts;
-    x.to_mont = 0; x.from_mont = 0;
+    x.to_mont = 0; x.from_mont = 0; x.pw_mul = 0;
     return x;
   };
   uint8_t* arr[3] = {a, b, c};
+  if (coset_form) {
+    for (int k = 0; k < 2; k++) {
+      for (int j = nb - 1; j >= 1; j--) {
+        NttBlock x = block(arr[k], j);
+        x.tw_dif = p.tw_inv;
+        OG_TRY(launch(x));
+      }
+      for (int j = 0; j < nb; j++) {
+        NttBlock x = block(arr[k], j);
+        if (j == 0) { x.tw_dif = p.tw_inv; x.mid = p.cs_fwd_ninv_br; }
+        x.tw_dit = p.tw_fwd;
+        if (k == 1 && j == nb - 1) { x.pw_a = a; x.pw_mul = 1; x.from_mont = 1; x.out = h_out; }
+        OG_TRY(launch(x));
+      }
+    }
+    return OG_OK;
+  }
   for (int k = 0; k < 3; k++) {
     for (int j = nb - 1; j >= 1; j--) {
       NttBlock x = block(arr[k], j);
@@ -612,7 +635,12 @@
     hipLaunchKernelGGL(k_to_mont_copy, dim3(grid_for(tot, 256)), dim3(256), 0, ctx->stream, src[k], buf[k], tot);
     OG_HIP(hipGetLastError());
   }
-  OG_TRY(h_poly_device(ctx, buf[0], buf[1], buf[2], buf[3], buf[3], log_d, batch));
+  if (OG_HOOK_INT("OG_H_POLY_COSET", 0)) {
+    OG_TRY(h_poly_device(ctx, buf[0], buf[1], buf[2], buf[3], buf[3], log_d, batch, 1));
+    OG_HIP(hipMemcpyAsync(h_out, buf[3], tot * 32, hipMemcpyDeviceToDevice, ctx->stream));
+    return OG_OK;
+  }
+  OG_TRY(h_poly_device(ctx, buf[0], buf[1], buf[2], buf[3], buf[3], log_d, batch, 0));
   hipLaunchKernelGGL(k_bitrev_copy, dim3(grid_for(d, 256), batch), dim3(256), 0, ctx->stream, buf[3], h_out, d * 32, log_d);
   OG_HIP(hipGetLastError());
   return OG_OK;
diff --git a/owshen_amd/csrc/point_spmv.hip.h b/owshen_amd/csrc/point_spmv.hip.h
--- /dev/null
+++ b/owshen_amd/csrc/point_spmv.hip.h
@@ -0,0 +1,105 @@
+#pragma once
+#include "snarkfile.hip.h"
+#include <algorithm>
+
+namespace og {
+
+static const uint32_t FR_ORDER_WORDS[8] = {0xf0000001u, 0x43e1f593u, 0x79b97091u, 0x2833e848u, 0x8181585du, 0xb85045b6u, 0xe131a029u, 0x30644e72u};
+static K256 fr_order_k256(uint32_t minus) {
+  K256 k;
+  memcpy(k.l, FR_ORDER_WORDS, 32);
+  k.l[0] -= minus;
+  return k;
+}
+
+template <class T>
+__global__ void __launch_bounds__(64) k_spmv_terms(const uint8_t* __restrict__ lag, const uint32_t* __restrict__ idx, const uint8_t* __restrict__ val,
+                                                  size_t nnz, K256 m1, uint8_t* __restrict__ terms) {
+  const size_t e = (size_t)blockIdx.x * blockDim.x + threadIdx.x;
+  if (e >= nnz) return;
+  XYZZ<T> p = XYZZ<T>::from_affine(Affine<T>::load(lag + (size_t)idx[e] * Affine<T>::BYTES));
+  const K256 k = k256_load(val + e * 32);
+  uint32_t hi = 0, dm = 0;
+  int top = -1;
+#pragma unroll
+  for (int w = 0; w < 8; w++) {
+    if (w) hi |= k.l[w];
+    dm |= k.l[w] ^ m1.l[w];
+    if (k.l[w]) top = 32 * w + 31 - __clz((int)k.l[w]);
+  }
+  if (dm == 0)
+    p = xyzz_neg(p);
+  else if (!(hi == 0 && k.l[0] == 1))
+    p = ecntt_smul(p, k, top);
+  p.store(terms + e * XYZZ<T>::BYTES);
+}
+
+template <class T>
+__global__ void __launch_bounds__(64) k_seg_sum(const uint8_t* __restrict__ in, const uint32_t* __restrict__ ptr, size_t n, uint8_t* __restrict__ out,
+                                               int affine) {
+  const size_t c = (size_t)blockIdx.x * blockDim.x + threadIdx.x;
+  if (c >= n) return;
+  const uint32_t b = ptr[c], e = ptr[c + 1];
+  XYZZ<T> acc = XYZZ<T>::inf();
+#pragma unroll 1
+  for (uint32_t i = b; i < e; i++) acc = xyzz_add(acc, XYZZ<T>::load(in + (size_t)i * XYZZ<T>::BYTES));
+  if (!affine) {
+    acc.store(out + c * XYZZ<T>::BYTES);
+    return;
+  }
+  Affine<T> a = xyzz_to_affine(acc);
+  a.x = FieldIO<T>::from_mont(a.x);
+  a.y = FieldIO<T>::from_mont(a.y);
+  a.store(out + c * Affine<T>::BYTES);
+}
+
+constexpr uint32_t SPMV_SEG = 32;
+
+template <class T>
+static int point_spmv(og_ctx* ctx, const uint8_t* lag_d, const std::vector<uint32_t>& tptr, const std::vector<uint32_t>& tidx,
+                      const std::vector<uint8_t>& tval, size_t m, uint8_t* out_d) {
+  const size_t nnz = tidx.size();
+  ZDev dev;
+  uint8_t *idx_d, *val_d, *cur_d;
+  OG_TRY(dev.get(nnz * 4, &idx_d));
+  OG_TRY(dev.get(nnz * 32, &val_d));
+  OG_TRY(dev.get(nnz * XYZZ<T>::BYTES, &cur_d));
+  if (nnz) {
+    OG_HIP(hipMemcpyAsync(idx_d, tidx.data(), nnz * 4, hipMemcpyHostToDevice, ctx->stream));
+    OG_HIP(hipMemcpyAsync(val_d, tval.data(), nnz * 32, hipMemcpyHostToDevice, ctx->stream));
+    hipLaunchKernelGGL(k_spmv_terms<T>, dim3(grid_for(nnz, 64)), dim3(64), 0, ctx->stream, lag_d, (const uint32_t*)idx_d, val_d, nnz, fr_order_k256(1), cur_d);
+    OG_HIP(hipGetLastError());
+  }
+  std::vector<std::vector<uint32_t>> keep;
+  std::vector<uint32_t> cp = tptr;
+  for (;;) {
+    uint32_t longest = 0;
+    for (size_t i = 0; i < m; i++) longest = std::max(longest, cp[i + 1] - cp[i]);
+    if (longest <= SPMV_SEG) break;
+    std::vector<uint32_t> chunk, next(m + 1, 0);
+    for (size_t i = 0; i < m; i++) {
+      for (uint32_t s = cp[i]; s < cp[i + 1]; s += SPMV_SEG) chunk.push_back(s);
+      next[i + 1] = (uint32_t)chunk.size();
+    }
+    const size_t n_chunks = chunk.size();
+    chunk.push_back(cp[m]);
+    uint8_t *p_d, *nxt_d;
+    OG_TRY(dev.get((n_chunks + 1) * 4, &p_d));
+    OG_TRY(dev.get(n_chunks * XYZZ<T>::BYTES, &nxt_d));
+    keep.push_back(std::move(chunk));
+    OG_HIP(hipMemcpyAsync(p_d, keep.back().data(), (n_chunks + 1) * 4, hipMemcpyHostToDevice, ctx->stream));
+    hipLaunchKernelGGL(k_seg_sum<T>, dim3(grid_for(n_chunks, 64)), dim3(64), 0, ctx->stream, cur_d, (const uint32_t*)p_d, n_chunks, nxt_d, 0);
+    OG_HIP(hipGetLastError());
+    cur_d = nxt_d;
+    cp.swap(next);
+  }
+  uint8_t* p_d;
+  OG_TRY(dev.get((m + 1) * 4, &p_d));
+  OG_HIP(hipMemcpyAsync(p_d, cp.data(), (m + 1) * 4, hipMemcpyHostToDevice, ctx->stream));
+  hipLaunchKernelGGL(k_seg_sum<T>, dim3(grid_for(m, 64)), dim3(64), 0, ctx->stream, cur_d, (const uint32_t*)p_d, m, out_d, 1);
+  OG_HIP(hipGetLastError());
+  OG_HIP(hipStreamSynchronize(ctx->stream));
+  return OG_OK;
+}
+
+}
diff --git a/owshen_amd/csrc/prover.h b/owshen_amd/csrc/prover.h
--- a/owshen_amd/csrc/prover.h
+++ b/owshen_amd/csrc/prover.h
@@ -5,7 +5,7 @@
 
 int ntt_domain_consts(og_ctx* ctx, int log_n, uint8_t** consts_d);
 int ntt_canonical(og_ctx* ctx, const uint8_t* in_d, uint8_t* out_d, int log_n, int batch, int inverse, int coset);
-int h_poly_device(og_ctx* ctx, uint8_t* a, uint8_t* b, uint8_t* c, uint8_t* tmp, uint8_t* h_out, int log_d, int batch);
+int h_poly_device(og_ctx* ctx, uint8_t* a, uint8_t* b, uint8_t* c, uint8_t* tmp, uint8_t* h_out, int log_d, int batch, int coset_form);
 int h_poly_canonical(og_ctx* ctx, const uint8_t* a, const uint8_t* b, const uint8_t* c, int log_d, int batch, uint8_t* h_out);
 
 int spmv_canonical(og_ctx* ctx, const uint32_t* ptr_d, const uint32_t* col_d, const uint8_t* val_d, size_t n_rows,
diff --git a/owshen_amd/csrc/ptau.hip b/owshen_amd/csrc/ptau.hip
--- a/owshen_amd/csrc/ptau.hip
+++ b/owshen_amd/csrc/ptau.hip
@@ -2,6 +2,7 @@
 #include "field.hip.h"
 #include "ec.hip.h"
 #include "snarkfile.hip.h"
+#include "point_spmv.hip.h"
 #include "keygen.h"
 #include "key_blob.h"
 #include "mimc7.hip.h"
@@ -21,47 +22,6 @@
   const G2XYZZ p = G2XYZZ::from_affine(G2Affine::load(aff + i * 128));
   const G2XYZZ q = ecntt_smul(p, order);
   if (!q.is_inf()) atomicOr(flags, 4u);
-}
-
-template <class T>
-__global__ void __launch_bounds__(64) k_spmv_terms(const uint8_t* __restrict__ lag, const uint32_t* __restrict__ idx, const uint8_t* __restrict__ val,
-                                                  size_t nnz, K256 m1, uint8_t* __restrict__ terms) {
-  const size_t e = (size_t)blockIdx.x * blockDim.x + threadIdx.x;
-  if (e >= nnz) return;
-  XYZZ<T> p = XYZZ<T>::from_affine(Affine<T>::load(lag + (size_t)idx[e] * Affine<T>::BYTES));
-  const K256 k = k256_load(val + e * 32);
-  uint32_t hi = 0, dm = 0;
-  int top = -1;
-#pragma unroll
-  for (int w = 0; w < 8; w++) {
-    if (w) hi |= k.l[w];
-    dm |= k.l[w] ^ m1.l[w];
-    if (k.l[w]) top = 32 * w + 31 - __clz((int)k.l[w]);
-  }
-  if (dm == 0)
-    p = xyzz_neg(p);
-  else if (!(hi == 0 && k.l[0] == 1))
-    p = ecntt_smul(p, k, top);
-  p.store(terms + e * XYZZ<T>::BYTES);
-}
-
-template <class T>
-__global__ void __launch_bounds__(64) k_seg_sum(const uint8_t* __restrict__ in, const uint32_t* __restrict__ ptr, size_t n, uint8_t* __restrict__ out,
-                                               int affine) {
-  const size_t c = (size_t)blockIdx.x * blockDim.x + threadIdx.x;
-  if (c >= n) return;
-  const uint32_t b = ptr[c], e = ptr[c + 1];
-  XYZZ<T> acc = XYZZ<T>::inf();
-#pragma unroll 1
-  for (uint32_t i = b; i < e; i++) acc = xyzz_add(acc, XYZZ<T>::load(in + (size_t)i * XYZZ<T>::BYTES));
-  if (!affine) {
-    acc.store(out + c * XYZZ<T>::BYTES);
-    return;
-  }
-  Affine<T> a = xyzz_to_affine(acc);
-  a.x = FieldIO<T>::from_mont(a.x);
-  a.y = FieldIO<T>::from_mont(a.y);
-  a.store(out + c * Affine<T>::BYTES);
 }
 
 __global__ void __launch_bounds__(64) k_ptau_h(const uint8_t* __restrict__ tau, size_t d, uint8_t* __restrict__ out) {
@@ -131,14 +91,6 @@
   m.store(out_mont + i * Affine<T>::BYTES);
 }
 
-static const uint32_t FR_WORDS[8] = {0xf0000001u, 0x43e1f593u, 0x79b97091u, 0x2833e848u, 0x8181585du, 0xb85045b6u, 0xe131a029u, 0x30644e72u};
-static K256 fr_order(uint32_t minus) {
-  K256 k;
-  memcpy(k.l, FR_WORDS, 32);
-  k.l[0] -= minus;
-  return k;
-}
-
 static const char* const PTAU_SEC[7] = {"", "section 1 (header)", "section 2 (tauG1)", "section 3 (tauG2)", "section 4 (alphaTauG1)", "section 5 (betaTauG1)",
                                         "section 6 (betaG2)"};
 
@@ -173,7 +125,7 @@
   uint8_t* f_d;
   OG_TRY(dev.get(4, &f_d));
   OG_HIP(hipMemsetAsync(f_d, 0, 4, ctx->stream));
-  hipLaunchKernelGGL(k_g2_subgroup, dim3(grid_for(n, 64)), dim3(64), 0, ctx->stream, mont_d, n, fr_order(0), (uint32_t*)f_d);
+  hipLaunchKernelGGL(k_g2_subgroup, dim3(grid_for(n, 64)), dim3(64), 0, ctx->stream, mont_d, n, fr_order_k256(0), (uint32_t*)f_d);
   OG_HIP(hipGetLastError());
   uint32_t flags = 0;
   OG_HIP(hipMemcpyAsync(&flags, f_d, 4, hipMemcpyDeviceToHost, ctx->stream));
@@ -186,55 +138,6 @@
   bool outside = false;
   OG_TRY(g2_subgroup_flags(ctx, dev, mont_d, n, &outside));
   OG_REQUIRE(!outside, who_sec + ": a point is not in the order-r subgroup");
-  return OG_OK;
-}
-
-constexpr uint32_t SEG = 32;
-
-template <class T>
-static int point_spmv(og_ctx* ctx, const uint8_t* lag_d, const std::vector<uint32_t>& tptr, const std::vector<uint32_t>& tidx,
-                      const std::vector<uint8_t>& tval, size_t m, uint8_t* out_d) {
-  const size_t nnz = tidx.size();
-  ZDev dev;
-  uint8_t *idx_d, *val_d, *cur_d;
-  OG_TRY(dev.get(nnz * 4, &idx_d));
-  OG_TRY(dev.get(nnz * 32, &val_d));
-  OG_TRY(dev.get(nnz * XYZZ<T>::BYTES, &cur_d));
-  if (nnz) {
-    OG_HIP(hipMemcpyAsync(idx_d, tidx.data(), nnz * 4, hipMemcpyHostToDevice, ctx->stream));
-    OG_HIP(hipMemcpyAsync(val_d, tval.data(), nnz * 32, hipMemcpyHostToDevice, ctx->stream));
-    hipLaunchKernelGGL(k_spmv_terms<T>, dim3(grid_for(nnz, 64)), dim3(64), 0, ctx->stream, lag_d, (const uint32_t*)idx_d, val_d, nnz, fr_order(1), cur_d);
-    OG_HIP(hipGetLastError());
-  }
-  std::vector<std::vector<uint32_t>> keep;
-  std::vector<uint32_t> cp = tptr;
-  for (;;) {
-    uint32_t longest = 0;
-    for (size_t i = 0; i < m; i++) longest = std::max(longest, cp[i + 1] - cp[i]);
-    if (longest <= SEG) break;
-    std::vector<uint32_t> chunk, next(m + 1, 0);
-    for (size_t i = 0; i < m; i++) {
-      for (uint32_t s = cp[i]; s < cp[i + 1]; s += SEG) chunk.push_back(s);
-      next[i + 1] = (uint32_t)chunk.size();
-    }
-    const size_t n_chunks = chunk.size();
-    chunk.push_back(cp[m]);
-    uint8_t *p_d, *nxt_d;
-    OG_TRY(dev.get((n_chunks + 1) * 4, &p_d));
-    OG_TRY(dev.get(n_chunks * XYZZ<T>::BYTES, &nxt_d));
-    keep.push_back(std::move(chunk));
-    OG_HIP(hipMemcpyAsync(p_d, keep.back().data(), (n_chunks + 1) * 4, hipMemcpyHostToDevice, ctx->stream));
-    hipLaunchKernelGGL(k_seg_sum<T>, dim3(grid_for(n_chunks, 64)), dim3(64), 0, ctx->stream, cur_d, (const uint32_t*)p_d, n_chunks, nxt_d, 0);
-    OG_HIP(hipGetLastError());
-    cur_d = nxt_d;
-    cp.swap(next);
-  }
-  uint8_t* p_d;
-  OG_TRY(dev.get((m + 1) * 4, &p_d));
-  OG_HIP(hipMemcpyAsync(p_d, cp.data(), (m + 1) * 4, hipMemcpyHostToDevice, ctx->stream));
-  hipLaunchKernelGGL(k_seg_sum<T>, dim3(grid_for(m, 64)), dim3(64), 0, ctx->stream, cur_d, (const uint32_t*)p_d, m, out_d, 1);
-  OG_HIP(hipGetLastError());
-  OG_HIP(hipStreamSynchronize(ctx->stream));
   return OG_OK;
 }
 
diff --git a/owshen_amd/groth16.py b/owshen_amd/groth16.py
--- a/owshen_amd/groth16.py
+++ b/owshen_amd/groth16.py
@@ -3,7 +3,7 @@
 
 import numpy as np
 
-from . import api
+from . import _abi, api
 from .api import FR, FR_MODULUS as R
 
 G1_GEN = (1, 2)
@@ -201,7 +201,7 @@
         d = (C.c_uint64 * 20)()
         self.ctx._check(self.ctx._lib.og_pk_query_form(self._h, d))
         names = ("a", "b1", "b2", "l", "h")
-        return {q: {"form": "row" if d[4 * k] else "wire", "points": int(d[4 * k + 1]), "bits": int(d[4 * k + 2]), "table": names[int(d[4 * k + 3])]}
+        return {q: {"form": "row" if d[4 * k] == 1 else "wire", "eval": _abi.QUERY_FORMS[int(d[4 * k])] == "eval", "points": int(d[4 * k + 1]), "bits": int(d[4 * k + 2]), "table": names[int(d[4 * k + 3])]}
                 for k, q in enumerate(names)}
 
     @staticmethod
```

Result: faster. 882.3 (median of 6 runs) (+1.9%).
